# kongzhecn/OMG

Measured on AMD Instinct MI355X. Metric: images/sec @ SDXL 1024^2 50-step, 2-concept mask fusion, higher is better.
Workload: dtype fp16 (storage and MFMA operands; fp32 accumulate; = the reference's own torch_dtype, inference_lora.py:153-159).  Measured tolerance per UNet forward at full size vs the fp32 oracle: rms 1.09e-3, max 4.9e-3 of O(1) outputs — the reference's own fp16 eager execution, emulated op by op in the oracle

## Files before the change

include/omg_hip.h:

```cpp
#ifndef OMG_HIP_H
#define OMG_HIP_H

#include <stdint.h>

#ifdef __cplusplus
extern "C" {
#endif

#define OMG_ABI_VERSION 6

enum { OMG_F16 = 0, OMG_BF16 = 1, OMG_F32 = 2  };

enum {
  OMG_OK = 0,
  OMG_EINVAL = -1,
  OMG_EDTYPE = -2,
  OMG_ELAUNCH = -3
};

enum {
  OMG_ACT_NONE = 0,
  OMG_ACT_SILU = 1,
  OMG_ACT_GEGLU = 2
};

int omg_abi_version(void);
const char* omg_last_error(void);

typedef struct {
  int32_t dtype;
  int32_t M, N, K;
  const void* A;  int64_t lda;
  const void* W;  int64_t ldw;
  const void* A2; int64_t lda2;
  const void* W2; int64_t ldw2;
  int32_t K2;
  int32_t a2_col_block;
  int32_t groups;
  int32_t rows_per_group;
  const int32_t* group_adapter;
  int64_t w_adapter_stride;
  int64_t w2_adapter_stride;
  const void* bias;
  const void* group_bias; int64_t ldgb;
  const void* residual; int64_t ldr;
  int32_t act;
  float out_scale;
  void* C; int64_t ldc;
} omg_gemm_args;

int omg_gemm(const omg_gemm_args* a, void* stream);

int omg_quant_mx8(int32_t dtype, const void* x, int64_t ldx, int32_t M, int32_t K,
                  void* q, int64_t ldq, void* scales, int32_t s_ld, void* stream);

typedef struct {
  int32_t dtype;
  int32_t M, N, K;
  const void* A; int64_t lda;
  const void* a_scale; int32_t sa_ld;
  const void* W; int64_t ldw;
  const void* w_scale; int32_t sw_ld;
  int32_t groups, rows_per_group;
  const int32_t* group_adapter;
  int64_t w_adapter_stride;
  int64_t sw_adapter_stride;
  const void* bias;
  const void* residual; int64_t ldr;
  int32_t act;
  float out_scale;
  void* C; int64_t ldc;
  void* c_scale; int32_t sc_ld;
} omg_gemm_mx8_args;

int omg_gemm_mx8(const omg_gemm_mx8_args* a, void* stream);

typedef struct {
  int32_t dtype;
  int32_t B, H, W, Cin, Cout;
  const void* X; const void* x_scale;
  const void* Wq; const void* w_scale;
  int32_t sw_ld, act;
  const void* bias;
  const void* group_bias; int64_t ldgb;
  const void* residual;
  float out_scale;
  void* Y;
} omg_conv2d_mx8_args;
int omg_conv2d_mx8(const omg_conv2d_mx8_args* a, void* stream);

typedef struct {
  int32_t dtype;
  int32_t B, Hin, Win;
  int32_t C1, C2;
  int32_t Hout, Wout, Cout;
  int32_t ksize;
  int32_t stride;
  int32_t upsample;
  const void* X1; const void* X2;
  const void* W;
  const void* bias;
  const void* group_bias; int64_t ldgb;
  const void* residual;
  float out_scale;
  void* Y;
  int32_t act;
} omg_conv2d_args;

int omg_conv2d(const omg_conv2d_args* a, void* stream);

typedef struct {
  omg_conv2d_args conv;
  const int32_t* group_adapter;
  int64_t w_slot_stride;
  const void* A2; int64_t lda2;
  const void* W2; int64_t ldw2;
  int64_t w2_slot_stride;
  int32_t K2;
} omg_conv2d_slots_args;

int omg_conv2d_slots(const omg_conv2d_slots_args* a, void* stream);

typedef struct {
  int32_t dtype;
  int32_t B, heads, Nq, Nkv;
  const void* Q; int64_t ldq; int64_t q_bstride;
  const void* K; int64_t ldk; int64_t k_bstride;
  const void* Vt;
  int32_t Nkv_pad;
  const int32_t* qk_src;
  float scale;
  int32_t accumulate;
  float out_scale;
  void* O; int64_t ldo; int64_t o_bstride;
  const void* V; int64_t ldv; int64_t v_bstride;
} omg_attn_args;

int omg_attn_fwd(const omg_attn_args* a, void* stream);

int omg_attn_fwd_causal(const omg_attn_args* a, void* stream);

int omg_transpose_v(int dtype, const void* V, int64_t ldv, int64_t v_bstride,
                    int B, int heads, int Nkv, int Nkv_pad, void* Vt, int mfma_key_order, void* stream);

typedef struct {
  int32_t dtype;
  int32_t B, heads, Nkv, Nkv_pad;
  const void* V; int64_t ldv; int64_t v_bstride;
  const int32_t* edit_of;
  int32_t E, steps;
  const float* mapper; int64_t ld_mapper; int64_t mapper_estride;
  const float* alpha; int64_t alpha_step_stride; int64_t alpha_estride;
  const int32_t* step_idx;
  void* Vt_mapped; void* Vt_own;
} omg_vmap_args;

int omg_transpose_v_mapped(const omg_vmap_args* a, void* stream);

int64_t omg_groupnorm_ws_floats(int B, int groups, int HW);
int omg_groupnorm(int dtype, const void* X1, int C1, const void* X2, int C2,
                  int B, int HW, int groups, float eps,
                  const void* gamma, const void* beta, int silu,
                  float* workspace, void* Y, void* stream);
int omg_layernorm(int dtype, const void* X, int64_t ldx, int M, int C, float eps,
                  const void* gamma, const void* beta, void* Y, int64_t ldy, void* stream);
int omg_layernorm_mx8(int dtype, const void* X, int64_t ldx, int M, int C, float eps,
                      const void* gamma, const void* beta, void* Q, int64_t ldq,
                      void* scales, int s_ld, void* stream);

int omg_groupnorm_mx8(int dtype, const void* X1, int C1, const void* X2, int C2,
                      int B, int HW, int groups, float eps,
                      const void* gamma, const void* beta, int silu,
                      float* workspace, void* Q, void* scales, void* stream);

typedef struct {
  int32_t B, Hin, Win, Cin;
  int32_t Hout, Wout, Cout;
  int32_t ksize, upsample;
  const void* X; const void* W; const void* bias; const void* residual;
  void* Y;
} omg_conv2d_f32_args;

int omg_conv2d_f32(const omg_conv2d_f32_args* a, void* stream);

typedef struct {
  int32_t B, Hin, Win, Cin;
  int32_t Hout, Wout, Cout;
  int32_t upsample;
  const void* X; const void* U; const void* bias; const void* residual;
  void* Y;
} omg_conv2d_f32_wino_args;

int64_t omg_conv2d_f32_wino_weight_floats(int Cout, int Cin);
int omg_conv2d_f32_wino(const omg_conv2d_f32_wino_args* a, void* stream);
int omg_cast_f32(int dtype, const void* X, float* Y, int64_t n, void* stream);

int omg_conv_in(int dtype, const void* X_nchw, int x_is_f32, int B, int Cin, int H, int W,
                const void* Wt , const void* bias, int Cout,
                void* workspace ,
                void* Y_nhwc, void* stream);
int omg_conv_out(int dtype, const void* X_nhwc, int B, int H, int W, int Cin,
// ... 62 lines not shown
```

omg_amd/_lib.py:

```python
from __future__ import annotations

import ctypes as C
import os

_HERE = os.path.dirname(os.path.abspath(__file__))
LIB_PATH = os.environ.get("OMG_HIP_LIB") or os.path.join(_HERE, "csrc", "libomg_hip.so")

OMG_F16, OMG_BF16, OMG_F32 = 0, 1, 2
ACT_NONE, ACT_SILU, ACT_GEGLU = 0, 1, 2
MAX_CONCEPTS = 8

c_i32, c_i64, c_f32, c_vp = C.c_int32, C.c_int64, C.c_float, C.c_void_p


class GemmArgs(C.Structure):
    _fields_ = [
        ("dtype", c_i32), ("M", c_i32), ("N", c_i32), ("K", c_i32),
        ("A", c_vp), ("lda", c_i64), ("W", c_vp), ("ldw", c_i64),
        ("A2", c_vp), ("lda2", c_i64), ("W2", c_vp), ("ldw2", c_i64),
        ("K2", c_i32), ("a2_col_block", c_i32),
        ("groups", c_i32), ("rows_per_group", c_i32),
        ("group_adapter", c_vp), ("w_adapter_stride", c_i64), ("w2_adapter_stride", c_i64),
        ("bias", c_vp), ("group_bias", c_vp), ("ldgb", c_i64),
        ("residual", c_vp), ("ldr", c_i64),
        ("act", c_i32), ("out_scale", c_f32),
        ("C", c_vp), ("ldc", c_i64),
    ]


class GemmMx8Args(C.Structure):
    _fields_ = [
        ("dtype", c_i32), ("M", c_i32), ("N", c_i32), ("K", c_i32),
        ("A", c_vp), ("lda", c_i64), ("a_scale", c_vp), ("sa_ld", c_i32),
        ("W", c_vp), ("ldw", c_i64), ("w_scale", c_vp), ("sw_ld", c_i32),
        ("groups", c_i32), ("rows_per_group", c_i32), ("group_adapter", c_vp),
        ("w_adapter_stride", c_i64), ("sw_adapter_stride", c_i64),
        ("bias", c_vp), ("residual", c_vp), ("ldr", c_i64),
        ("act", c_i32), ("out_scale", c_f32),
        ("C", c_vp), ("ldc", c_i64),
        ("c_scale", c_vp), ("sc_ld", c_i32),
    ]


class Conv2dMx8Args(C.Structure):
    _fields_ = [
        ("dtype", c_i32), ("B", c_i32), ("H", c_i32), ("W", c_i32), ("Cin", c_i32), ("Cout", c_i32),
        ("X", c_vp), ("x_scale", c_vp), ("Wq", c_vp), ("w_scale", c_vp),
        ("sw_ld", c_i32), ("act", c_i32),
        ("bias", c_vp), ("group_bias", c_vp), ("ldgb", c_i64), ("residual", c_vp),
        ("out_scale", c_f32), ("Y", c_vp),
    ]


class Conv2dArgs(C.Structure):
    _fields_ = [
        ("dtype", c_i32), ("B", c_i32), ("Hin", c_i32), ("Win", c_i32),
        ("C1", c_i32), ("C2", c_i32), ("Hout", c_i32), ("Wout", c_i32), ("Cout", c_i32),
        ("ksize", c_i32), ("stride", c_i32), ("upsample", c_i32),
        ("X1", c_vp), ("X2", c_vp), ("W", c_vp), ("bias", c_vp),
        ("group_bias", c_vp), ("ldgb", c_i64), ("residual", c_vp),
        ("out_scale", c_f32), ("Y", c_vp), ("act", c_i32),
    ]


class Conv2dSlotsArgs(C.Structure):
    _fields_ = [
        ("conv", Conv2dArgs), ("group_adapter", c_vp), ("w_slot_stride", c_i64),
        ("A2", c_vp), ("lda2", c_i64), ("W2", c_vp), ("ldw2", c_i64),
        ("w2_slot_stride", c_i64), ("K2", c_i32),
    ]


class Conv2dF32Args(C.Structure):
    _fields_ = [
        ("B", c_i32), ("Hin", c_i32), ("Win", c_i32), ("Cin", c_i32),
        ("Hout", c_i32), ("Wout", c_i32), ("Cout", c_i32), ("ksize", c_i32), ("upsample", c_i32),
        ("X", c_vp), ("W", c_vp), ("bias", c_vp), ("residual", c_vp), ("Y", c_vp),
    ]


class Conv2dF32WinoArgs(C.Structure):
    _fields_ = [
        ("B", c_i32), ("Hin", c_i32), ("Win", c_i32), ("Cin", c_i32),
        ("Hout", c_i32), ("Wout", c_i32), ("Cout", c_i32), ("upsample", c_i32),
        ("X", c_vp), ("U", c_vp), ("bias", c_vp), ("residual", c_vp), ("Y", c_vp),
    ]


class AttnArgs(C.Structure):
    _fields_ = [
        ("dtype", c_i32), ("B", c_i32), ("heads", c_i32), ("Nq", c_i32), ("Nkv", c_i32),
        ("Q", c_vp), ("ldq", c_i64), ("q_bstride", c_i64),
        ("K", c_vp), ("ldk", c_i64), ("k_bstride", c_i64),
        ("Vt", c_vp), ("Nkv_pad", c_i32),
        ("qk_src", c_vp), ("scale", c_f32), ("accumulate", c_i32), ("out_scale", c_f32),
        ("O", c_vp), ("ldo", c_i64), ("o_bstride", c_i64),
        ("V", c_vp), ("ldv", c_i64), ("v_bstride", c_i64),
    ]


class VMapArgs(C.Structure):
    _fields_ = [
        ("dtype", c_i32), ("B", c_i32), ("heads", c_i32), ("Nkv", c_i32), ("Nkv_pad", c_i32),
        ("V", c_vp), ("ldv", c_i64), ("v_bstride", c_i64),
        ("edit_of", c_vp), ("E", c_i32), ("steps", c_i32),
        ("mapper", c_vp), ("ld_mapper", c_i64), ("mapper_estride", c_i64),
        ("alpha", c_vp), ("alpha_step_stride", c_i64), ("alpha_estride", c_i64),
        ("step_idx", c_vp), ("Vt_mapped", c_vp), ("Vt_own", c_vp),
    ]


class StepArgs(C.Structure):
    _fields_ = [
        ("C", c_i32), ("H", c_i32), ("W", c_i32), ("Hm", c_i32), ("Wm", c_i32),
        ("n_concepts", c_i32), ("fuse", c_i32), ("guidance_scale", c_f32),
        ("noise_pred", c_vp), ("region_pred", c_vp * MAX_CONCEPTS), ("masks", c_vp * MAX_CONCEPTS),
        ("coef", c_vp), ("step_idx", c_vp), ("advance", c_i32),
        ("latents", c_vp), ("out_dtype", c_i32), ("model_input_next", c_vp), ("fused_noise_out", c_vp),
    ]


SYMBOLS = {
    "omg_abi_version": (c_i32, []),
    "omg_last_error": (C.c_char_p, []),
    "omg_gemm": (c_i32, [C.POINTER(GemmArgs), c_vp]),
    "omg_quant_mx8": (c_i32, [c_i32, c_vp, c_i64, c_i32, c_i32, c_vp, c_i64, c_vp, c_i32, c_vp]),
    "omg_gemm_mx8": (c_i32, [C.POINTER(GemmMx8Args), c_vp]),
    "omg_conv2d_mx8": (c_i32, [C.POINTER(Conv2dMx8Args), c_vp]),
    "omg_groupnorm_mx8": (c_i32, [c_i32, c_vp, c_i32, c_vp, c_i32, c_i32, c_i32, c_i32, c_f32, c_vp, c_vp, c_i32, c_vp, c_vp, c_vp, c_vp]),
    "omg_conv2d": (c_i32, [C.POINTER(Conv2dArgs), c_vp]),
    "omg_conv2d_slots": (c_i32, [C.POINTER(Conv2dSlotsArgs), c_vp]),
    "omg_conv2d_f32": (c_i32, [C.POINTER(Conv2dF32Args), c_vp]),
    "omg_conv2d_f32_wino_weight_floats": (c_i64, [c_i32, c_i32]),
    "omg_conv2d_f32_wino": (c_i32, [C.POINTER(Conv2dF32WinoArgs), c_vp]),
    "omg_cast_f32": (c_i32, [c_i32, c_vp, c_vp, c_i64, c_vp]),
    "omg_attn_fwd": (c_i32, [C.POINTER(AttnArgs), c_vp]),
    "omg_attn_fwd_causal": (c_i32, [C.POINTER(AttnArgs), c_vp]),
    "omg_transpose_v": (c_i32, [c_i32, c_vp, c_i64, c_i64, c_i32, c_i32, c_i32, c_i32, c_vp, c_i32, c_vp]),
    "omg_transpose_v_mapped": (c_i32, [C.POINTER(VMapArgs), c_vp]),
    "omg_groupnorm_ws_floats": (c_i64, [c_i32, c_i32, c_i32]),
    "omg_groupnorm": (c_i32, [c_i32, c_vp, c_i32, c_vp, c_i32, c_i32, c_i32, c_i32, c_f32, c_vp, c_vp, c_i32, c_vp, c_vp, c_vp]),
    "omg_layernorm": (c_i32, [c_i32, c_vp, c_i64, c_i32, c_i32, c_f32, c_vp, c_vp, c_vp, c_i64, c_vp]),
    "omg_layernorm_mx8": (c_i32, [c_i32, c_vp, c_i64, c_i32, c_i32, c_f32, c_vp, c_vp, c_vp, c_i64, c_vp, c_i32, c_vp]),
    "omg_conv_in": (c_i32, [c_i32, c_vp, c_i32, c_i32, c_i32, c_i32, c_i32, c_vp, c_vp, c_i32, c_vp, c_vp, c_vp]),
    "omg_conv_out": (c_i32, [c_i32, c_vp, c_i32, c_i32, c_i32, c_i32, c_vp, c_vp, c_i32, c_vp, c_vp]),
    "omg_timestep_embedding": (c_i32, [c_i32, c_vp, c_i32, c_i32, c_vp, c_i64, c_vp]),
    "omg_silu": (c_i32, [c_i32, c_vp, c_vp, c_i64, c_vp]),
    "omg_softmax_rows": (c_i32, [c_i32, c_vp, c_i64, c_i64, c_i64, C.c_float, c_vp]),
    "omg_channel_mix": (c_i32, [c_vp, c_vp, c_vp, c_i32, c_i32, c_i32, c_i64, c_vp, c_vp]),
    "omg_add_inplace": (c_i32, [c_i32, c_vp, c_vp, c_i64, c_vp]),
    "omg_copy2d": (c_i32, [c_i32, c_vp, c_i64, c_vp, c_i64, c_i64, c_i64, c_vp]),
    "omg_fuse_cfg_step": (c_i32, [C.POINTER(StepArgs), c_vp]),
    "omg_fuse_cfg_step_ms": (c_i32, [C.POINTER(StepArgs), c_vp, c_vp, c_vp]),
    "omg_fuse_cfg_step_noise": (c_i32, [C.POINTER(StepArgs), c_vp, c_i64, c_vp]),
    "omg_scale_model_input": (c_i32, [c_i32, c_vp, c_vp, c_i32, c_vp, c_vp]),
    "omg_gather_step": (c_i32, [c_i32, c_vp, c_vp, c_vp, c_i64, c_vp]),
    "omg_attn_probs": (c_i32, [C.POINTER(AttnArgs), c_vp, c_vp]),
    "omg_attn_apply_probs": (c_i32, [c_i32, c_vp, c_vp, c_i64, c_i64, c_i32, c_i32, c_i32, c_i32, c_vp, c_i64, c_i64, c_vp]),
    "omg_dwconv2d": (c_i32, [c_i32, c_vp, c_i64, c_i32, c_i32, c_i32, c_i32, c_i32, c_vp, c_vp, c_vp, c_i64, c_vp]),
    "omg_relu_linear_att_ws_floats": (c_i64, [c_i32, c_i32, c_i32, c_i32]),
    "omg_relu_linear_att": (c_i32, [c_i32, c_vp, c_i64, c_i32, c_i32, c_i32, c_i32, c_f32, c_vp, c_vp, c_i64, c_vp]),
    "omg_conv3x3_nhwc_act": (c_i32, [c_i32, c_vp, c_i32, c_i32, c_i32, c_i32, c_i32, c_i32, c_vp, c_vp, c_i32, c_vp, c_vp, c_vp]),
    "omg_dwconv3x3_act": (c_i32, [c_i32, c_vp, c_i64, c_i32, c_i32, c_i32, c_i32, c_i32, c_vp, c_vp, c_i32, c_vp, c_i64, c_vp]),
    "omg_upsample_add_nhwc": (c_i32, [c_i32, c_vp, c_i32, c_i32, c_i32, c_i32, c_i32, c_i32, c_i32, c_vp, c_vp]),
    "omg_debug_set_glds": (None, [c_i32]),
    "omg_debug_set_gemm_variant": (None, [c_i32]),
    "omg_debug_choose_variant": (c_i32, [c_i32, c_i32, c_i32, c_i32]),
    "omg_debug_set_mx8_split": (None, [c_i32]),
    "omg_debug_set_attn_variant": (None, [c_i32]),
}

_lib = None


class OmgHipError(RuntimeError):
    pass


def lib() -> C.CDLL:
# ... 36 lines not shown
```

omg_amd/attention.py:

```python
from __future__ import annotations

from typing import Optional

import torch
from torch import nn

from . import _lib as L
from . import ops
from .modules import Dropout, Linear, LoraState, bump_pointer_epoch, pointer_epoch


class Attention(nn.Module):

    def __init__(self, query_dim: int, cross_attention_dim: Optional[int], heads: int, dim_head: int = 64,
                 dtype=torch.float16, device=None):
        super().__init__()
        if dim_head != 64:
            raise L.OmgHipError("the gfx950 attention kernel is specialised for head_dim 64 (all SDXL layers)")
        inner = heads * dim_head
        self.heads, self.scale, self.inner_dim = heads, dim_head ** -0.5, inner
        self.is_cross = cross_attention_dim is not None
        kv_dim = cross_attention_dim if self.is_cross else query_dim
        self.to_q = Linear(query_dim, inner, bias=False, dtype=dtype, device=device)
        self.to_k = Linear(kv_dim, inner, bias=False, dtype=dtype, device=device)
        self.to_v = Linear(kv_dim, inner, bias=False, dtype=dtype, device=device)
        self.to_out = nn.ModuleList([Linear(inner, query_dim, bias=True, dtype=dtype, device=device), Dropout()])
        self.spatial_norm = None
        self.group_norm = None
        self.norm_cross = None
        self.residual_connection = False
        self.rescale_output_factor = 1.0
        self.processor = FusedAttnProcessor()
        self._qkv = None
        self._kv = None
        self._qkv_slots = None
        self._kv_slots = None
        self._kv_cache = {}
        self.ip_kv_weight: Optional[torch.Tensor] = None
        self.ip_scale, self.ip_tokens = 1.0, 16
        self._ip_cache = None
        self._mx8 = {}

    def set_processor(self, processor) -> None:
        self.processor = processor

    def get_processor(self):
        return self.processor

    def forward(self, hidden_states, encoder_hidden_states=None, attention_mask=None, **cross_attention_kwargs):
        return self.processor(self, hidden_states, encoder_hidden_states=encoder_hidden_states,
                              attention_mask=attention_mask, **cross_attention_kwargs)

    def prepare_attention_mask(self, attention_mask, target_length, batch_size, out_dim=3):
        if attention_mask is not None:
            raise L.OmgHipError("attention masks are not used on OMG's path (always None) and are not supported")
        return None

    def head_to_batch_dim(self, t: torch.Tensor) -> torch.Tensor:
        B, N, _ = t.shape
        return t.reshape(B, N, self.heads, 64).permute(0, 2, 1, 3).reshape(B * self.heads, N, 64)

    def batch_to_head_dim(self, t: torch.Tensor) -> torch.Tensor:
        BH, N, d = t.shape
        return t.reshape(BH // self.heads, self.heads, N, d).permute(0, 2, 1, 3).reshape(BH // self.heads, N, self.heads * d)

    def get_attention_scores(self, query: torch.Tensor, key: torch.Tensor, attention_mask=None) -> torch.Tensor:
        if attention_mask is not None:
            raise L.OmgHipError("attention masks are not supported")
        q, k = query.contiguous(), key.contiguous()
        return ops.attn_probs(q, k, 1, self.scale)

    def _apply(self, fn, *a, **k):
        self.invalidate_packed()
        return super()._apply(fn, *a, **k)

    def invalidate_packed(self):
        self._qkv = self._kv = self._qkv_slots = self._kv_slots = None
        self._kv_cache = {}
        self._mx8 = {}
        self._ip_cache = None
        bump_pointer_epoch()

    def qkv_weight(self) -> torch.Tensor:
        if self._qkv is None:
            self._qkv = torch.cat([self.to_q.weight.data, self.to_k.weight.data, self.to_v.weight.data], dim=0).contiguous()
        return self._qkv

    def kv_weight(self) -> torch.Tensor:
        if self._kv is None:
            self._kv = torch.cat([self.to_k.weight.data, self.to_v.weight.data], dim=0).contiguous()
        return self._kv

    def _has_lora(self) -> bool:
        st = self.to_q.lora_state
        return st is not None and not st.merged and any(l.lora_down is not None for l in (self.to_q, self.to_k, self.to_v))

    def _merged(self) -> Optional[LoraState]:
        st = self.to_q.lora_state
        if st is None or not st.merged:
            return None
        have = [l.w_slots is not None for l in (self.to_q, self.to_k, self.to_v)]
        if any(have) and not all(have):
            raise L.OmgHipError("merged LoRA slots cover only part of to_q/to_k/to_v; rebuild the LoraBank")
        return st if all(have) else None

    def qkv_slots(self) -> torch.Tensor:
        if self._qkv_slots is None:
            self._qkv_slots = torch.cat([self.to_q.w_slots, self.to_k.w_slots, self.to_v.w_slots], dim=1).contiguous()
        return self._qkv_slots

    def kv_slots(self) -> torch.Tensor:
        if self._kv_slots is None:
            self._kv_slots = torch.cat([self.to_k.w_slots, self.to_v.w_slots], dim=1).contiguous()
        return self._kv_slots

    def project_self(self, x):
        B, N, C = x.shape
        inner = self.inner_dim
        if isinstance(x, ops.Mx8Tensor) or (self.to_q.mx8 and C % 128 == 0 and not self._has_lora()):
            if self._has_lora():
                raise L.OmgHipError("MX-fp8 activations cannot feed a segment-mode LoRA projection")
            xq = x if isinstance(x, ops.Mx8Tensor) else ops.quant_mx8(x)
            st = self._merged()
            if st is not None:
                if "qkv_slots" not in self._mx8:
                    self._mx8["qkv_slots"] = ops.quant_mx8(self.qkv_slots().reshape(-1, C))
                qkv = ops.gemm_mx8(xq, self._mx8["qkv_slots"], out_dtype=self.to_q.weight.dtype, groups=st.groups,
                                   w_group_adapter=st.group_adapter, n_per_adapter=3 * inner)
            else:
                if "qkv" not in self._mx8:
                    self._mx8["qkv"] = ops.quant_mx8(self.qkv_weight())
                qkv = ops.gemm_mx8(xq, self._mx8["qkv"], out_dtype=self.to_q.weight.dtype)
            qkv = qkv.view(B, N, 3 * inner)
            return qkv[:, :, :inner], qkv[:, :, inner:2 * inner], ops.value_operand(qkv[:, :, 2 * inner:], self.heads)
        if self._has_lora():
            q = self.to_q(x); k = self.to_k(x); v = self.to_v(x)
        else:
            st = self._merged()
            if st is not None:
                qkv = ops.gemm(x.reshape(B * N, C), self.qkv_slots(), groups=st.groups, w_group_adapter=st.group_adapter)
            else:
                qkv = ops.gemm(x.reshape(B * N, C), self.qkv_weight())
            qkv = qkv.view(B, N, 3 * inner)
            q, k, v = qkv[:, :, :inner], qkv[:, :, inner:2 * inner], qkv[:, :, 2 * inner:]
        return q, k, ops.value_operand(v, self.heads)

    def project_cross(self, ctx: torch.Tensor, with_v: bool = False):
        st = self.to_k.lora_state
        skey = (tuple(ctx.shape), None if st is None else (st.group_adapter.data_ptr(), st.merged))
        stamp = (ctx.data_ptr(), ctx._version)
        hit = self._kv_cache.get(skey)
        if hit is not None:
            self._kv_cache[skey] = self._kv_cache.pop(skey)
        if hit is not None and hit[0] == stamp:
            return (hit[1], hit[2], hit[5], hit[6]) if with_v else (hit[1], hit[2])
        B, Nk, Cx = ctx.shape
        inner = self.inner_dim
        kv_out = hit[4] if hit is not None else None
        vt_out = hit[2] if hit is not None else None
        if self._has_lora():
            k = self.to_k(ctx); v = self.to_v(ctx)
            kv_out = None
        else:
            ms = self._merged()
            x2 = ctx.reshape(B * Nk, Cx)
            if ms is not None:
                kv = ops.gemm(x2, self.kv_slots(), groups=ms.groups, w_group_adapter=ms.group_adapter, out=kv_out)
            else:
                kv = ops.gemm(x2, self.kv_weight(), out=kv_out)
            kv_out = kv
            kv = kv.view(B, Nk, 2 * inner)
            k, v = kv[:, :, :inner], kv[:, :, inner:]
        vt = ops.transpose_v(v, self.heads, out=vt_out)
        if hit is None and len(self._kv_cache) >= 4:
            self._kv_cache.pop(next(iter(self._kv_cache)))
            bump_pointer_epoch()
        images = hit[6] if hit is not None else [None, None]
        self._kv_cache[skey] = (stamp, k, vt, ctx, kv_out, v, images)
        return (k, vt, v, images) if with_v else (k, vt)


def _ip_kv(attn: Attention, ip_ctx: torch.Tensor):
    shape = tuple(ip_ctx.shape)
    stamp = (ip_ctx.data_ptr(), ip_ctx._version)
    cache = attn._ip_cache
    if cache is None:
        cache = attn._ip_cache = {}
    c = cache.get(shape)
    if c is not None:
        cache[shape] = cache.pop(shape)
    if c is None or c[0] != stamp:
        Bc, Ni, Cx = shape
        kv_out = c[3] if c is not None else None
        vt_out = c[2] if c is not None else None
        kv = ops.gemm(ip_ctx.reshape(Bc * Ni, Cx), attn.ip_kv_weight, out=kv_out)
        kv3 = kv.view(Bc, Ni, 2 * attn.inner_dim)
        vt = ops.transpose_v(kv3[:, :, attn.inner_dim:], attn.heads, out=vt_out)
        if c is None and len(cache) >= 4:
            cache.pop(next(iter(cache)))
            bump_pointer_epoch()
        c = (stamp, kv3[:, :, :attn.inner_dim], vt, kv, shape, ip_ctx)
        cache[shape] = c
    return c


def _ip_branch(attn: Attention, q: torch.Tensor, o: torch.Tensor, ip_ctx: torch.Tensor, row0: int) -> None:
    c = _ip_kv(attn, ip_ctx)
    ops.attention(q[row0:], c[1], c[2], attn.heads, attn.scale, out=o[row0:], accumulate=True, out_scale=attn.ip_scale)


def _to_tokens(attn, hidden_states):
    if isinstance(hidden_states, ops.Mx8Tensor):
        return hidden_states
    if hidden_states.dim() == 4:
        raise L.OmgHipError("4-D (NCHW) hidden_states are not produced by the SDXL transformer blocks; pass (B, N, C)")
    return hidden_states


class FusedAttnProcessor:

    supports_fused_residual = True

    def _qk_src(self, attn, is_cross: bool, n_tokens: int, batch: int, device, main_batch=None, images=1):
        return None

    def _skip_layer(self) -> None:
        return None

    def __call__(self, attn: Attention, hidden_states, encoder_hidden_states=None, attention_mask=None, temb=None,
                 scale: float = 1.0, residual: Optional[torch.Tensor] = None, **cross_attention_kwargs):
        if attention_mask is not None:
            raise L.OmgHipError("attention_mask is not supported")
        x = _to_tokens(attn, hidden_states)
        B, N, _ = x.shape
        is_cross = encoder_hidden_states is not None
        if is_cross:
            q = attn.to_q(x)
            k, vt = attn.project_cross(encoder_hidden_states)
        else:
            q, k, vt = attn.project_self(x)
        bypass = cross_attention_kwargs.pop("omg_bypass_controller", False)
        main_b = cross_attention_kwargs.pop("omg_main_batch", None)
        n_img = cross_attention_kwargs.pop("omg_images", 1)
        twin = cross_attention_kwargs.pop("omg_twin", False)
        if twin and not bypass:
            self._skip_layer()
        src = None if (bypass or twin) else self._qk_src(attn, is_cross, N, B, x.device, main_b, n_img)
        ip_ctx = cross_attention_kwargs.pop("omg_ip_tokens", None)
        ip_row0 = cross_attention_kwargs.pop("omg_ip_rows", 0)
        o = ops.attention(q, k, vt, attn.heads, attn.scale, qk_src=src)
        if is_cross and ip_ctx is not None and attn.ip_kv_weight is not None:
            _ip_branch(attn, q, o, ip_ctx, ip_row0)
        out = attn.to_out[0](o, residual=residual)
        return out


class RegionControlNet_AttnProcessor(FusedAttnProcessor):

    force_protocol = False

    def __init__(self, attention_op=None, controller=None, place_in_unet=None):
        self.attention_op = attention_op
        self.controller = controller
        self.place_in_unet = place_in_unet

    def _fusable(self) -> bool:
        return self.controller is None or getattr(self.controller, "is_pure_replacement", False)

    def _general(self) -> bool:
        c = self.controller
        return hasattr(c, "fused_edit") and hasattr(c, "edit_tables") and getattr(c, "local_blend", None) is None

    def _general_call(self, attn: Attention, hidden_states, encoder_hidden_states, residual, kw):
        ctl = self.controller
        x = _to_tokens(attn, hidden_states)
        B, N, _ = x.shape
        is_cross = encoder_hidden_states is not None
        main_b = kw.pop("omg_main_batch", None)
        n_img = kw.pop("omg_images", 1)
        if kw.pop("omg_twin", False):
            raise L.OmgHipError("omg_twin (dedup) needs a pure-replacement controller")
        ip_ctx = kw.pop("omg_ip_tokens", None)
        ip_row0 = kw.pop("omg_ip_rows", 0)
        v = images = None
        if is_cross:
            q = attn.to_q(x)
            if ctl.cross_kind() == "mixed":
                k, vt, v, images = attn.project_cross(encoder_hidden_states, with_v=True)
            else:
                k, vt = attn.project_cross(encoder_hidden_states)
        else:
            q, k, vt = attn.project_self(x)
        kind, src, edit_of = ctl.fused_edit(is_cross, N, main_b or B, self.place_in_unet, device=x.device, total_batch=B, images=n_img)
        if kind == "mixed":
            mapper, alpha, step = ctl.edit_tables(x.device)
            if images[0] is None:
                images[0], images[1] = torch.empty_like(vt), torch.empty_like(vt)
            vm, vo = ops.transpose_v_mapped(v, attn.heads, edit_of, mapper, alpha, step, nkv_pad=vt.shape[3], out=(images[0], images[1]))
            o = ops.attention(q, k, vm, attn.heads, attn.scale, qk_src=src)
            ops.attention(q, k, vo, attn.heads, attn.scale, out=o, accumulate=True)
        else:
            o = ops.attention(q, k, vt, attn.heads, attn.scale, qk_src=src)
        if is_cross and ip_ctx is not None and attn.ip_kv_weight is not None:
            _ip_branch(attn, q, o, ip_ctx, ip_row0)
        return attn.to_out[0](o, residual=residual)

    def _qk_src(self, attn, is_cross, n_tokens, batch, device, main_batch=None, images=1):
        if self.controller is None:
            return None
        return self.controller.fused_qk_src(is_cross, n_tokens, main_batch or batch, self.place_in_unet, device=device,
                                            total_batch=batch, images=images)

    def _skip_layer(self) -> None:
        if self.controller is not None:
            self.controller.skip_layer()

    def __call__(self, attn: Attention, hidden_states, encoder_hidden_states=None, attention_mask=None, temb=None,
                 scale: float = 1.0, residual: Optional[torch.Tensor] = None, **cross_attention_kwargs):
        bypass = cross_attention_kwargs.get("omg_bypass_controller", False)
        if bypass or self.controller is None or (self._fusable() and not self.force_protocol):
            return super().__call__(attn, hidden_states, encoder_hidden_states, attention_mask, temb, scale,
                                    residual=residual, **cross_attention_kwargs)
        if self._general() and not self.force_protocol:
            if attention_mask is not None:
                raise L.OmgHipError("attention_mask is not supported")
            return self._general_call(attn, hidden_states, encoder_hidden_states, residual, cross_attention_kwargs)
        if cross_attention_kwargs.get("omg_images", 1) != 1:
            raise L.OmgHipError("protocol mode (non-identity mapper) runs one request at a time")
        x = _to_tokens(attn, hidden_states)
        is_cross = encoder_hidden_states is not None
        src = encoder_hidden_states if is_cross else x
        query = attn.head_to_batch_dim(attn.to_q(x))
        key = attn.head_to_batch_dim(attn.to_k(src))
        value = attn.to_v(src)
        probs = attn.get_attention_scores(query, key, None)
        probs = self.controller(probs, is_cross, self.place_in_unet)
        o = ops.attn_apply_probs(probs.contiguous(), value, attn.heads)
        return attn.to_out[0](o, residual=residual)


class IPAttnProcessor2_0(nn.Module):

    supports_fused_residual = True

    def __init__(self, hidden_size: int, cross_attention_dim: Optional[int] = None, scale: float = 1.0, num_tokens: int = 4,
                 dtype=torch.float16, device=None):
        super().__init__()
        self.hidden_size, self.cross_attention_dim, self.scale, self.num_tokens = hidden_size, cross_attention_dim, scale, num_tokens
        self.to_k_ip = Linear(cross_attention_dim or hidden_size, hidden_size, bias=False, dtype=dtype, device=device)
        self.to_v_ip = Linear(cross_attention_dim or hidden_size, hidden_size, bias=False, dtype=dtype, device=device)

    def __call__(self, attn: Attention, hidden_states, encoder_hidden_states=None, attention_mask=None, temb=None,
                 residual: Optional[torch.Tensor] = None, **kw):
        if attention_mask is not None:
            raise L.OmgHipError("attention_mask is not supported")
        x = _to_tokens(attn, hidden_states)
        if encoder_hidden_states is None:
            q, k, vt = attn.project_self(x)
            o = ops.attention(q, k, vt, attn.heads, attn.scale)
            return attn.to_out[0](o, residual=residual)
        end = encoder_hidden_states.shape[1] - self.num_tokens
        text, ip = encoder_hidden_states[:, :end], encoder_hidden_states[:, end:]
        q = attn.to_q(x)
        B, Nt, Cx = text.shape
        k = attn.to_k(text.reshape(B * Nt, Cx)).view(B, Nt, -1)
        v = attn.to_v(text.reshape(B * Nt, Cx)).view(B, Nt, -1)
        o = ops.attention(q, k, ops.transpose_v(v, attn.heads), attn.heads, attn.scale)
        Ni = ip.shape[1]
        ipc = ip.reshape(B * Ni, Cx)
        k_ip = self.to_k_ip(ipc).view(B, Ni, -1)
        v_ip = self.to_v_ip(ipc).view(B, Ni, -1)
        ops.attention(q, k_ip, ops.transpose_v(v_ip, attn.heads), attn.heads, attn.scale, out=o, accumulate=True,
                      out_scale=self.scale)
        return attn.to_out[0](o, residual=residual)
```

omg_amd/controller.py:

```python
from __future__ import annotations

from typing import Dict, List, Optional, Sequence, Tuple

import numpy as np
import torch

MAX_NUM_WORDS = 77


def _word_of_token(text: str, tokenizer) -> Tuple[List[str], np.ndarray]:
    words = text.split(" ")
    pieces = [tokenizer.decode([tok]).strip("#") for tok in tokenizer.encode(text)][1:-1]
    cum = np.cumsum([len(pc_) for pc_ in pieces], dtype=np.int64) if pieces else np.zeros(0, np.int64)
    owner = np.full(len(pieces), len(words), dtype=np.int64)
    first, base = 0, 0
    for k, word in enumerate(words):
        if first >= len(pieces):
            break
        last = int(np.searchsorted(cum, base + len(word), side="left"))
        last = max(last, first)
        last = min(last, len(pieces) - 1)
        owner[first:last + 1] = k
        first, base = last + 1, int(cum[last])
    return words, owner


def get_word_inds(text: str, word_place, tokenizer) -> np.ndarray:
    words = text.split(" ")
    if isinstance(word_place, str):
        wanted = [i for i, w in enumerate(words) if w == word_place]
    elif isinstance(word_place, int):
        wanted = [word_place]
    else:
        wanted = list(word_place)
    if not wanted:
        return np.array([])
    _, owner = _word_of_token(text, tokenizer)
    return np.flatnonzero(np.isin(owner, wanted)) + 1


def _alignment_matrix(src_spans: Sequence[np.ndarray], tgt_spans: Sequence[np.ndarray], max_len: int) -> np.ndarray:
    m = np.zeros((max_len, max_len))
    i = j = 0
    for s, t in zip(src_spans, tgt_spans):
        s, t = np.asarray(s, dtype=np.int64), np.asarray(t, dtype=np.int64)
        run = min(int(s[0]) - i, max_len - i, max_len - j)
        if run < int(s[0]) - i:
            r = np.arange(max(run, 0))
            m[i + r, j + r] = 1
            return m
        r = np.arange(run)
        m[i + r, j + r] = 1
        i, j = i + run, j + run
        if i >= max_len or j >= max_len:
            return m
        if len(s) == len(t):
            m[s, t] = 1
        else:
            m[np.ix_(s, t)] = 1.0 / len(t)
        i, j = i + len(s), j + len(t)
    tail = np.arange(max(0, min(max_len - i, max_len - j)))
    if src_spans:
        m[j + tail, j + tail] = 1
    else:
        m[i + tail, j + tail] = 1
    return m


def get_replacement_mapper(prompts: Sequence[str], tokenizer, max_len: int = MAX_NUM_WORDS) -> torch.Tensor:
    out = []
    words0 = prompts[0].split(" ")
    for other in prompts[1:]:
        words = other.split(" ")
        if len(words0) != len(words):
            raise ValueError("attention replacement edit can only be applied on prompts with the same length"
                             f" but prompt A has {len(words0)} words and prompt B has {len(words)} words.")
        changed = [k for k, (a, b) in enumerate(zip(words0, words)) if a != b]
        if not changed:
            out.append(torch.eye(max_len, dtype=torch.float32))
            continue
        if tokenizer is None:
            raise ValueError("a tokenizer is required to align prompts that differ")
        _, own0 = _word_of_token(prompts[0], tokenizer)
        _, own1 = _word_of_token(other, tokenizer)
        src = [np.flatnonzero(own0 == k) + 1 for k in changed]
        tgt = [np.flatnonzero(own1 == k) + 1 for k in changed]
        out.append(torch.from_numpy(_alignment_matrix(src, tgt, max_len)).float())
    return torch.stack(out)


def get_time_words_attention_alpha(prompts, num_steps, cross_replace_steps, tokenizer, max_num_words=MAX_NUM_WORDS):
    spec = dict(cross_replace_steps) if isinstance(cross_replace_steps, dict) else {"default_": cross_replace_steps}
    spec.setdefault("default_", (0.0, 1.0))
    if isinstance(cross_replace_steps, dict):
        cross_replace_steps.setdefault("default_", (0.0, 1.0))
    n_rows, n_edit = num_steps + 1, len(prompts) - 1
    steps = torch.arange(n_rows).view(n_rows, 1)

    def inside(bounds) -> torch.Tensor:
        lo, hi = (0, bounds) if isinstance(bounds, float) else bounds
        return ((steps >= int(lo * n_rows)) & (steps < int(hi * n_rows))).to(torch.float32)

    alpha = inside(spec["default_"]).view(n_rows, 1, 1).repeat(1, n_edit, max_num_words)
    for word, bounds in spec.items():
        if word == "default_":
            continue
        col = inside(bounds)
        for k in range(n_edit):
            pos = get_word_inds(prompts[k + 1], word, tokenizer)
            if len(pos) > 0:
                alpha[:, k, torch.as_tensor(pos, dtype=torch.long)] = col
    return alpha.reshape(n_rows, n_edit, 1, 1, max_num_words)


class AttentionReplace:
    def __init__(self, prompts, num_steps: int, cross_replace_steps, self_replace_steps, width, height,
                 local_blend=None, tokenizer=None, device=None, dtype=None):
        self.low_resource = False
        self.width, self.height = width, height
        self.batch_size = len(prompts)
        self.local_blend = local_blend
        self.device, self.dtype = device, dtype
        alpha = get_time_words_attention_alpha(prompts, num_steps, cross_replace_steps, tokenizer)
        self.cross_replace_alpha = alpha.to(device)
        if isinstance(self_replace_steps, float):
            self_replace_steps = (0, self_replace_steps)
        self.num_self_replace = (int(num_steps * self_replace_steps[0]), int(num_steps * self_replace_steps[1]))
        mapper = get_replacement_mapper(prompts, tokenizer)
        self._alpha_host = alpha.reshape(alpha.shape[0], alpha.shape[1], MAX_NUM_WORDS).float().contiguous()
        self._mapper_host = mapper.float().contiguous()
        self._tables: Dict[str, Tuple[torch.Tensor, torch.Tensor]] = {}
        self._edit_cache: Dict[Tuple, torch.Tensor] = {}
        self._step_dev: Dict[str, torch.Tensor] = {}
        self._step_dev_val: Dict[str, int] = {}
        self._bound_step: Optional[Tuple[torch.Tensor, int]] = None
        self.mapper = mapper.to(dtype=dtype, device=device)
        self.num_att_layers = -1
        self.cur_step = 0
        self.cur_att_layer = 0
        eye = torch.eye(MAX_NUM_WORDS)
        self._identity_mapper = all(torch.equal(m.float().cpu(), eye) for m in self.mapper)
        self.is_pure_replacement = bool(local_blend is None and self._identity_mapper and bool((self.cross_replace_alpha == 1).all()))
        self._src_cache: Dict[Tuple, torch.Tensor] = {}
        ident = bool(all(torch.equal(m, eye) for m in self._mapper_host))
        self._cross_kinds = ["borrow" if ident and bool((a == 1).all()) else "own" if bool((a == 0).all()) else "mixed"
                             for a in self._alpha_host]

    @property
    def num_uncond_att_layers(self):
        return 0

    def reset(self):
        self.cur_step = 0
        self.cur_att_layer = 0

    def between_steps(self):
        return

    def step_callback(self, x_t):
        return x_t

    def _tick(self):
        self.cur_att_layer += 1
        if self.cur_att_layer == self.num_att_layers + self.num_uncond_att_layers:
            self.cur_att_layer = 0
            self.cur_step += 1
            self.between_steps()

    def _self_window(self) -> bool:
        return self.num_self_replace[0] <= self.cur_step < self.num_self_replace[1]

    def forward(self, attn, is_cross: bool, place_in_unet: str):
        if not (is_cross or self._self_window()):
            return attn
        v = attn.reshape(self.batch_size, attn.shape[0] // self.batch_size, *attn.shape[1:])
        base, edits = v[0], v[1:]
        if is_cross:
            a = self.cross_replace_alpha[self.cur_step].to(device=v.device, dtype=v.dtype)
            mapped = base.unsqueeze(0).expand(edits.shape[0], *base.shape) if self._identity_mapper \
                else torch.matmul(base.unsqueeze(0), self.mapper.to(device=v.device, dtype=v.dtype).unsqueeze(1))
            edits.copy_(mapped * a + (1 - a) * edits)
        elif edits.shape[2] <= self.width * self.height:
            edits.copy_(base.unsqueeze(0).expand_as(edits))
        return v.reshape(attn.shape)

    def __call__(self, attn, is_cross: bool, place_in_unet: str):
        cond = attn[attn.shape[0] // 2:]
        out = self.forward(cond, is_cross, place_in_unet)
        if out.data_ptr() != cond.data_ptr():
            cond.copy_(out)
        self._tick()
        return attn

    def replaces(self, is_cross: bool, n_tokens: int) -> bool:
        if is_cross:
            return True
        return self._self_window() and n_tokens <= self.width * self.height

    def qk_src_vector(self, batch: int, device, total_batch: Optional[int] = None, images: int = 1) -> torch.Tensor:
        total = total_batch or batch * images
        key = (batch, total, images, str(device))
        t = self._src_cache.get(key)
        if t is None:
            n = batch // 2
            v = []
            for j in range(images):
                v += [j * batch + i for i in range(n)] + [j * batch + n] * (batch - n)
            v += list(range(batch * images, total))
            t = torch.tensor(v, dtype=torch.int32, device=device)
            self._src_cache[key] = t
        return t

    def cross_kind(self, step: Optional[int] = None) -> str:
        step = self.cur_step if step is None else step
        return self._cross_kinds[min(max(step, 0), len(self._cross_kinds) - 1)]

    def edit_of_vector(self, batch: int, device, total_batch: Optional[int] = None, images: int = 1) -> torch.Tensor:
        total = total_batch or batch * images
        key = (batch, total, images, str(device))
        t = self._edit_cache.get(key)
        if t is None:
            n = batch // 2
            t = torch.tensor(([-1] * (n + 1) + list(range(batch - n - 1))) * images + [-1] * (total - batch * images),
                             dtype=torch.int32, device=device)
            self._edit_cache[key] = t
        return t

    def bind_step_counter(self, step_idx: Optional[torch.Tensor], offset: int = 0) -> None:
        self._bound_step = None if step_idx is None else (step_idx, int(offset))

    def _own_step_counter(self, device, refresh: bool = True) -> torch.Tensor:
        key = str(device)
        t = self._step_dev.get(key)
        if t is None:
            t = self._step_dev[key] = torch.zeros(1, dtype=torch.int32, device=device)
            self._step_dev_val[key] = 0
        if refresh and self._step_dev_val[key] != self.cur_step:
            if torch.cuda.is_current_stream_capturing():
                raise RuntimeError("a captured step needs a device step counter: bind_step_counter(step_idx) before capturing")
            t.fill_(self.cur_step)
            self._step_dev_val[key] = self.cur_step
        return t

    def edit_tables(self, device=None) -> Tuple[torch.Tensor, torch.Tensor, torch.Tensor]:
        device = torch.device(device or self.device or "cuda")
        key = str(device)
        tabs = self._tables.get(key)
        if tabs is None:
            tabs = self._tables[key] = (self._mapper_host.to(device), self._alpha_host.to(device))
        mapper, alpha = tabs
        if self._bound_step is not None:
            step, off = self._bound_step
            if not 0 <= off < alpha.shape[0]:
                raise RuntimeError(f"step counter offset {off} outside the {alpha.shape[0]}-row alpha table")
            return mapper, alpha[off:], step
        return mapper, alpha, self._own_step_counter(device, refresh=False)

    def fused_edit(self, is_cross: bool, n_tokens: int, batch: int, place_in_unet: str = "", device=None,
                   total_batch: Optional[int] = None, images: int = 1):
        if self.local_blend is not None:
            raise RuntimeError("fused_edit does not cover local_blend")
        n2 = 2 * self.batch_size
        if batch != n2 and not (batch == n2 - 1 and self.is_pure_replacement):
            raise ValueError(f"controller built for {self.batch_size} prompts expects a batch of {n2} ([unc..., cond...]), got {batch}")
        dev = device or self.device or "cuda"
        kind = self.cross_kind() if is_cross else ("borrow" if self.replaces(False, n_tokens) else "own")
        src = edit_of = None
        if kind != "own":
            src = self.qk_src_vector(batch, dev, total_batch, images)
        if kind == "mixed":
            edit_of = self.edit_of_vector(batch, dev, total_batch, images)
            if self._bound_step is None:
                self._own_step_counter(torch.device(dev))
        self._tick()
        return kind, src, edit_of

    def skip_layer(self) -> None:
        if not self.is_pure_replacement:
            raise RuntimeError("skip_layer needs a pure-replacement controller")
        self._tick()

    def fused_qk_src(self, is_cross: bool, n_tokens: int, batch: int, place_in_unet: str = "",
                     device=None, total_batch: Optional[int] = None, images: int = 1) -> Optional[torch.Tensor]:
        if not self.is_pure_replacement:
            raise RuntimeError("fused_qk_src needs a pure-replacement controller (identity mapper, alpha == 1)")
        if batch not in (2 * self.batch_size, 2 * self.batch_size - 1):
            raise ValueError(f"controller built for {self.batch_size} prompts expects a batch of {2 * self.batch_size} "
                             f"([unc..., cond...]), got {batch}")
        src = self.qk_src_vector(batch, device or self.device or "cuda", total_batch, images) if self.replaces(is_cross, n_tokens) else None
        self._tick()
        return src
```

omg_amd/csrc/gemm.hip:

```cpp
#include "common.h"
#include "gemm_epilogue.h"

__device__ __attribute__((aligned(256))) unsigned char omg_zero_page[256];

__device__ long long omg_dbg_ts[8192][6];

namespace {

constexpr int BM = 128, BN = 128, BK = 64;
constexpr int TILE_BYTES = BM * BK * 2;
constexpr int STAGE_LD = 68;
constexpr int LDS_BYTES_MAIN = 4 * TILE_BYTES;
constexpr int LDS_BYTES_EPI = 4 * 64 * STAGE_LD * 4;
constexpr int LDS_BYTES = LDS_BYTES_EPI > LDS_BYTES_MAIN ? LDS_BYTES_EPI : LDS_BYTES_MAIN;


template <bool GLDS>
OMG_DEV void stage16(const char* src, char* lds_wave_base, int lane, u32x4& hold) {
  if constexpr (GLDS) {
    __builtin_amdgcn_global_load_lds((gbl_ptr_t)src, (lds_ptr_t)lds_wave_base, 16, 0, 0);
  } else {
    hold = *(const u32x4*)src;
  }
}

template <typename T, int MT, int NT>
OMG_DEV void acc_init_cols(const GemmP& p, f32x16 (&acc)[MT][NT], int l31, int col0, int m0) {
  const bool fold = fold_group_bias(p);
  const long grow = fold ? (long)(m0 / p.rows_per_group) * p.ldgb : 0;
#pragma unroll
  for (int j = 0; j < NT; ++j) {
    const int c = col0 + j * 32 + l31;
    float b = 0.f;
    if (c < p.N) {
      float g = 0.f;
      if (p.bias) b = (float)((const T*)p.bias)[c];
      if (fold) g = (float)((const T*)p.group_bias)[grow + c];
      b = b + g;
    }
#pragma unroll
    for (int i = 0; i < MT; ++i)
#pragma unroll
      for (int r = 0; r < 16; ++r) acc[i][j][r] = b;
  }
}

template <typename T>
OMG_DEV void gemm_epilogue(const GemmP& p, f32x16 (&acc)[2][2], char* smem, int w, int lane, int m0, int n0, int m_end) {
  const int hi = lane >> 5, l31 = lane & 31;
  const int wm = w >> 1, wn = w & 1;
  __syncthreads();
  float* stage = (float*)smem + w * (64 * STAGE_LD);
#pragma unroll
  for (int i = 0; i < 2; ++i)
#pragma unroll
    for (int j = 0; j < 2; ++j)
#pragma unroll
      for (int r = 0; r < 16; ++r) {
        const int row = i * 32 + (r & 3) + 8 * (r >> 2) + 4 * hi;
        stage[row * STAGE_LD + j * 32 + l31] = acc[i][j][r];
      }
  __syncthreads();

  const int wm0 = m0 + wm * 64;
  const int wn0 = n0 + wn * 64;
  if (p.act == OMG_ACT_GEGLU) {
    const int ocol0 = (wn0 >> 1);
    const int sub = lane & 3, rsub = lane >> 2;
#pragma unroll
    for (int it = 0; it < 4; ++it) {
      const int row = it * 16 + rsub;
      const int gm = wm0 + row;
      const int gc = wn0 + sub * 8;
      if (gm < m_end && gc < p.N) {
        float v[8], g[8];
        const float* sp = stage + row * STAGE_LD + sub * 8;
#pragma unroll
        for (int e = 0; e < 8; ++e) { v[e] = sp[e]; g[e] = sp[32 + e]; }
        float o[8];
#pragma unroll
        for (int e = 0; e < 8; ++e) o[e] = v[e] * gelu_f(g[e]) * p.out_scale;
        *(u32x4*)(p.C + ((long)gm * p.ldc + ocol0 + sub * 8) * 2) = pack8<T>(o);
      }
    }
    return;
  }
  {
    const int sub = lane & 7, rsub = lane >> 3;
    const int gc = wn0 + sub * 8;
    const bool gb_rows = p.group_bias != nullptr && !fold_group_bias(p);
#pragma unroll
    for (int it = 0; it < 8; ++it) {
      const int row = it * 8 + rsub;
      const int gm = wm0 + row;
      if (gm < m_end && gc < p.N) {
        float v[8];
        const float* sp = stage + row * STAGE_LD + sub * 8;
#pragma unroll
        for (int e = 0; e < 8; ++e) v[e] = sp[e];
        if (gb_rows) {
          float gb[8];
          const int g = gm / p.rows_per_group;
          unpack8<T>(*(const u32x4*)(p.group_bias + ((long)g * p.ldgb + gc) * 2), gb);
#pragma unroll
          for (int e = 0; e < 8; ++e) v[e] += gb[e];
        }
        if (p.act == OMG_ACT_SILU) {
#pragma unroll
          for (int e = 0; e < 8; ++e) v[e] = silu_fast(v[e]);
        }
        if (p.residual) {
          float rv[8];
          unpack8<T>(*(const u32x4*)(p.residual + ((long)gm * p.ldr + gc) * 2), rv);
#pragma unroll
          for (int e = 0; e < 8; ++e) v[e] = __builtin_fmaf(v[e], p.out_scale, rv[e]);
        } else {
#pragma unroll
          for (int e = 0; e < 8; ++e) v[e] *= p.out_scale;
        }
        *(u32x4*)(p.C + ((long)gm * p.ldc + gc) * 2) = pack8<T>(v);
      }
    }
  }
}

template <typename T, bool CONV, bool GLDS, bool CSEG = false>
__global__ __launch_bounds__(256, 2) void gemm_kernel(GemmP p) {
  static_assert(CONV || !CSEG, "CSEG is the segment of the CONV form; the plain form always has it");
  extern __shared__ __attribute__((aligned(16))) char smem[];
  const int tid = threadIdx.x;
  const int lane = tid & 63;
  const int w = __builtin_amdgcn_readfirstlane(tid >> 6);
  const int hi = lane >> 5;
  const int l31 = lane & 31;

  const int nwg = gridDim.x;
  int bid = blockIdx.x;
  {
    const int q = nwg >> 3, r = nwg & 7, xcd = bid & 7, idx = bid >> 3;
    bid = (xcd < r ? xcd * (q + 1) : r * (q + 1) + (xcd - r) * q) + idx;
  }
  const int tiles_per_group = p.tiles_m * p.tiles_n;
  const int grp = bid / tiles_per_group;
  const int t_in = bid - grp * tiles_per_group;
  int tm, tn;
  {
    const int per_group = 8 * p.tiles_n;
    const int gid = t_in / per_group;
    const int first_m = gid * 8;
    const int gsz = (p.tiles_m - first_m) < 8 ? (p.tiles_m - first_m) : 8;
    const int r = t_in - gid * per_group;
    tm = first_m + (r % gsz);
    tn = r / gsz;
  }
  const int m_base = (p.tile_groups > 1) ? grp * p.rows_per_group : 0;
  const int m_end = (p.tile_groups > 1) ? m_base + p.rows_per_group : p.M;
  const int m0 = m_base + tm * BM;
  const int n0 = tn * BN;

  int adapter = 0;
  if (p.group_adapter != nullptr) adapter = p.group_adapter[grp];
  const bool seg2 = (p.K2 > 0) && (adapter >= 0);
  if (p.w_adapter_stride != 0 && adapter < 0) return;
  const char* Wp = p.W + (p.w_adapter_stride != 0 ? (long)adapter * p.w_adapter_stride * 2 : 0);
  const char* W2p = p.W2 + (seg2 ? (long)adapter * p.w2_adapter_stride * 2 : 0);
  const int a2off = (p.a2_col_block > 0) ? (n0 / p.a2_col_block) * p.K2 : 0;

  const int nk1 = (p.K + BK - 1) / BK;
  const int nk2 = seg2 ? (p.K2 + BK - 1) / BK : 0;
  const int nk = nk1 + nk2;

  const int prow = lane >> 3;
  const int ppos = lane & 7;
  int arow[4];
  int wrow[4];
  int cb[4], cy[4], cx[4];
#pragma unroll
  for (int i = 0; i < 4; ++i) {
    const int r = w * 32 + i * 8 + prow;
    int gm = m0 + r; if (gm > m_end - 1) gm = m_end - 1;
    int gn = n0 + r; if (gn > p.N - 1) gn = p.N - 1;
    arow[i] = gm; wrow[i] = gn;
    if constexpr (CONV) {
      const int hw = p.Hout * p.Wout;
      const int b = gm / hw; const int rem = gm - b * hw;
      cb[i] = b; cy[i] = rem / p.Wout; cx[i] = rem - cy[i] * p.Wout;
    }
  }
  const int Ctot = p.C1 + p.C2;
  const int cpt = CONV ? Ctot / BK : 1;
  const int pad = CONV ? (p.ksize == 3 ? 1 : 0) : 0;
  const char* zero = (const char*)omg_zero_page;

  u32x4 hold[8];
  char* ldsA = smem;
  char* ldsB = smem + 2 * TILE_BYTES;

  auto issue = [&](int kt, int buf) {
    const bool s2 = kt >= nk1;
    const int k0 = (s2 ? kt - nk1 : kt) * BK;
    const int Kseg = s2 ? p.K2 : p.K;
    int dy = 0, dx = 0, c0 = k0;
    const char* xsrc = p.A; int xC = p.C1;
    if constexpr (CONV) {
      const int ktc = (CSEG && s2) ? 0 : kt;
      const int tap = ktc / cpt; const int cc = ktc - tap * cpt;
      dy = tap / p.ksize; dx = tap - dy * p.ksize;
      c0 = cc * BK;
      if (c0 >= p.C1) { xsrc = p.X2; xC = p.C2; c0 -= p.C1; }
    }
#pragma unroll
    for (int i = 0; i < 4; ++i) {
      const int r = w * 32 + i * 8 + prow;
      const int c = ppos ^ ((r >> 1) & 7);
      const bool kvalid = (k0 + c * 8) < Kseg;
      const char* asrc;
      if constexpr (CONV) {
        int iy = cy[i] * p.stride + dy - pad;
        int ix = cx[i] * p.stride + dx - pad;
        const int Hl = p.upsample ? p.Hin * 2 : p.Hin;
        const int Wl = p.upsample ? p.Win * 2 : p.Win;
        const bool ok = (iy >= 0) && (iy < Hl) && (ix >= 0) && (ix < Wl);
        if (p.upsample) { iy >>= 1; ix >>= 1; }
        const long pix = ((long)cb[i] * p.Hin + iy) * p.Win + ix;
        asrc = ok ? xsrc + (pix * xC + c0 + c * 8) * 2 : zero;
        if constexpr (CSEG) {
          if (s2) asrc = kvalid ? p.A2 + ((long)arow[i] * p.lda2 + k0 + c * 8) * 2 : zero;
        }
      } else {
        if (!s2) asrc = kvalid ? p.A + ((long)arow[i] * p.lda + k0 + c * 8) * 2 : zero;
        else     asrc = kvalid ? p.A2 + ((long)arow[i] * p.lda2 + a2off + k0 + c * 8) * 2 : zero;
      }
      stage16<GLDS>(asrc, ldsA + buf * TILE_BYTES + (w * 32 + i * 8) * 128, lane, hold[i]);
      const char* wsrc;
      if (!s2) wsrc = kvalid ? Wp + ((long)wrow[i] * p.ldw + (CONV ? kt * BK : k0) + c * 8) * 2 : zero;
      else     wsrc = kvalid ? W2p + ((long)wrow[i] * p.ldw2 + k0 + c * 8) * 2 : zero;
      stage16<GLDS>(wsrc, ldsB + buf * TILE_BYTES + (w * 32 + i * 8) * 128, lane, hold[4 + i]);
    }
  };
  auto commit = [&](int buf) {
    if constexpr (!GLDS) {
#pragma unroll
      for (int i = 0; i < 4; ++i) {
        const int off = (w * 32 + i * 8) * 128 + lane * 16;
        *(u32x4*)(ldsA + buf * TILE_BYTES + off) = hold[i];
        *(u32x4*)(ldsB + buf * TILE_BYTES + off) = hold[4 + i];
      }
    }
  };

  const int wm = w >> 1, wn = w & 1;
  f32x16 acc[2][2];
  acc_init_cols<T, 2, 2>(p, acc, lane & 31, n0 + wn * 64, m0);

  using V8 = typename Vec<T>::v8;

  issue(0, 0);
  commit(0);
  for (int kt = 0; kt < nk; ++kt) {
    const int buf = kt & 1;
    asm volatile("s_waitcnt vmcnt(0)" ::: "memory");
    __syncthreads();
    if (kt + 1 < nk) issue(kt + 1, buf ^ 1);
    const char* a_base = ldsA + buf * TILE_BYTES;
    const char* b_base = ldsB + buf * TILE_BYTES;
#pragma unroll
    for (int ks = 0; ks < 4; ++ks) {
      V8 af[2], bf[2];
      const int kc = ks * 2 + hi;
#pragma unroll
      for (int i = 0; i < 2; ++i) {
        const int ra = wm * 64 + i * 32 + l31;
        af[i] = *(const V8*)(a_base + ra * 128 + ((kc ^ ((ra >> 1) & 7)) << 4));
        const int rb = wn * 64 + i * 32 + l31;
        bf[i] = *(const V8*)(b_base + rb * 128 + ((kc ^ ((rb >> 1) & 7)) << 4));
      }
#pragma unroll
      for (int i = 0; i < 2; ++i)
#pragma unroll
        for (int j = 0; j < 2; ++j) acc[i][j] = Vec<T>::mfma32(af[i], bf[j], acc[i][j]);
    }
    if constexpr (!GLDS) { if (kt + 1 < nk) commit(buf ^ 1); }
  }

  gemm_epilogue<T>(p, acc, smem, w, lane, m0, n0, m_end);
}


OMG_DEV int conv_voff(int b, int oy, int ox, int ch_bytes, int stride, int dy, int dx, int Hl, int Wl, int ups, int Hin, int Win,
                      int pix_bytes, int c0_bytes) {
  int iy = oy * stride + dy, ix = ox * stride + dx;
  const bool ok = ((unsigned)iy < (unsigned)Hl) & ((unsigned)ix < (unsigned)Wl);
  iy >>= ups; ix >>= ups;
  const int pix = (b * Hin + iy) * Win + ix;
  const int off = pix * pix_bytes + c0_bytes + ch_bytes;
  return ok ? off : 0x7ffffff0;
}

template <typename T, bool CONV, int MT>
__global__ __launch_bounds__(512, 2) void gemm_kernel_v6(GemmP p) {
  constexpr int BM_ = 256, BN_ = MT == 4 ? 256 : 128, BKc = 64, NW = 8, NT = 2;
  constexpr int WN_ = MT == 4 ? 4 : 2;
  constexpr int BI = BN_ / 8 / NW;
  constexpr int ND = 4 + BI;
  constexpr int HB = ND / 2;
  constexpr int A_BYTES = BM_ * BKc * 2;
  constexpr int STAGE_BYTES = (BM_ + BN_) * BKc * 2;

  extern __shared__ __attribute__((aligned(16))) char smem[];
  const int tid = threadIdx.x;
  const int lane = tid & 63;
  const int w = __builtin_amdgcn_readfirstlane(tid >> 6);
  const int hi = lane >> 5;
  const int l31 = lane & 31;

  const int nwg = gridDim.x;
  int bid = blockIdx.x;
  {
    const int q = nwg >> 3, r = nwg & 7, xcd = bid & 7, idx = bid >> 3;
    bid = (xcd < r ? xcd * (q + 1) : r * (q + 1) + (xcd - r) * q) + idx;
  }
  const int tiles_per_group = p.tiles_m * p.tiles_n;
  const int grp = bid / tiles_per_group;
  const int t_in = bid - grp * tiles_per_group;
  int tm, tn;
  {
    const int per_group = 8 * p.tiles_n;
    const int gid = t_in / per_group;
    const int first_m = gid * 8;
    const int gsz = (p.tiles_m - first_m) < 8 ? (p.tiles_m - first_m) : 8;
    const int r = t_in - gid * per_group;
    tm = first_m + (r % gsz);
    tn = r / gsz;
  }
  const int m_base = (p.tile_groups > 1) ? grp * p.rows_per_group : 0;
  const int m_end = (p.tile_groups > 1) ? m_base + p.rows_per_group : p.M;
  const int m0 = m_base + tm * BM_;
  const int n0 = tn * BN_;
  int adapter = 0;
  if (p.group_adapter != nullptr) adapter = p.group_adapter[grp];
  if (p.w_adapter_stride != 0 && adapter < 0) return;
  const char* Wp = p.W + (p.w_adapter_stride != 0 ? (long)adapter * p.w_adapter_stride * 2 : 0);
  const int nk = (p.K + BKc - 1) / BKc;

  const int Ctot = p.C1 + p.C2;
  const long a_bytes = CONV ? (long)p.M / (p.Hout * p.Wout) * p.Hin * p.Win * p.C1 * 2 : ((long)(p.M - 1) * p.lda + p.K) * 2;
  const __amdgpu_buffer_rsrc_t rsA = __builtin_amdgcn_make_buffer_rsrc((void*)p.A, 0, (int)(a_bytes < 0x7fffff00 ? a_bytes : 0x7fffff00), 0x00020000);
  const __amdgpu_buffer_rsrc_t rsA2 = __builtin_amdgcn_make_buffer_rsrc((void*)(CONV && p.X2 ? p.X2 : p.A), 0,
      CONV ? (int)((long)p.M / (p.Hout * p.Wout) * p.Hin * p.Win * p.C2 * 2) : 0, 0x00020000);
  const long w_bytes = ((long)(p.N - 1) * p.ldw + p.K) * 2;
  const __amdgpu_buffer_rsrc_t rsW = __builtin_amdgcn_make_buffer_rsrc((void*)Wp, 0, (int)w_bytes, 0x00020000);

  const int prow = lane >> 3, ppos = lane & 7;
  int voffA[4], voffW[BI], ldoA[4], ldoW[BI];
  int cb[4], cy[4], cx[4], cch[4];
#pragma unroll
  for (int i = 0; i < 4; ++i) {
    const int r = (w + i * NW) * 8 + prow;
    const int c = ppos ^ ((r >> 1) & 7);
    int gm = m0 + r; if (gm > m_end - 1) gm = m_end - 1;
    ldoA[i] = (w + i * NW) * 1024;
    if constexpr (CONV) {
      const int hw = p.Hout * p.Wout;
      const int b = gm / hw; const int rem = gm - b * hw;
      cb[i] = b; cy[i] = rem / p.Wout; cx[i] = rem - cy[i] * p.Wout; cch[i] = c * 16;
      voffA[i] = 0;
    } else {
      voffA[i] = (int)(((long)gm * p.lda + c * 8) * 2);
    }
  }
#pragma unroll
  for (int i = 0; i < BI; ++i) {
    const int r = (w + i * NW) * 8 + prow;
    const int c = ppos ^ ((r >> 1) & 7);
    int gn = n0 + r; if (gn > p.N - 1) gn = p.N - 1;
    voffW[i] = (int)(((long)gn * p.ldw + c * 8) * 2);
    ldoW[i] = A_BYTES + (w + i * NW) * 1024;
  }

  const int wm = w / WN_, wn = w % WN_;
  f32x16 acc[MT][NT];
  const bool gb_epi = acc_init_bias<T, MT, NT>(p, acc, lane, m0, n0 + wn * 64);
  using V8 = typename Vec<T>::v8;
  int aro[MT][4], bro[NT][4];
#pragma unroll
  for (int ks = 0; ks < 4; ++ks) {
    const int kc = ks * 2 + hi;
#pragma unroll
    for (int i = 0; i < MT; ++i) {
      const int ra = wm * (MT * 32) + i * 32 + l31;
      aro[i][ks] = ra * 128 + ((kc ^ ((ra >> 1) & 7)) << 4);
    }
#pragma unroll
    for (int j = 0; j < NT; ++j) {
      const int rb = wn * 64 + j * 32 + l31;
      bro[j][ks] = A_BYTES + rb * 128 + ((kc ^ ((rb >> 1) & 7)) << 4);
    }
  }

  int koff = 0;
  int tap_dy = 0, tap_dx = 0, c0b = 0, xCb = 0;
  bool x2 = false;
  const int cpt = CONV ? Ctot / BKc : 1;
  const int pad = CONV ? (p.ksize == 3 ? 1 : 0) : 0;
  const int Hl = CONV ? (p.upsample ? p.Hin * 2 : p.Hin) : 0;
  const int Wl = CONV ? (p.upsample ? p.Win * 2 : p.Win) : 0;
#define OMG_PREP(kt_)                                                                                      \
  do {                                                                                                     \
    koff = (kt_) * (BKc * 2);                                                                              \
    if constexpr (CONV) {                                                                                  \
      const int tap = (kt_) / cpt; const int cc = (kt_) - tap * cpt;                                       \
      tap_dy = tap / p.ksize - pad; tap_dx = tap - (tap / p.ksize) * p.ksize - pad;                        \
      int c0 = cc * BKc;                                                                                   \
      x2 = c0 >= p.C1;                                                                                     \
      if (x2) c0 -= p.C1;                                                                                  \
      c0b = c0 * 2; xCb = (x2 ? p.C2 : p.C1) * 2;                                                          \
    }                                                                                                      \
  } while (0)
#define OMG_AVO(i_) (CONV ? conv_voff(cb[i_], cy[i_], cx[i_], cch[i_], p.stride, tap_dy, tap_dx, Hl, Wl, p.upsample, p.Hin, p.Win, xCb, c0b) : voffA[i_])

  const bool late = w >= 4;
  V8 af[2][MT], bf[2][NT];
#define OMG_ISA(d_) ((d_) < 4)
#define OMG_AI(d_) ((d_) < 4 ? (d_) : 0)
#define OMG_WI(d_) ((d_) >= 4 ? (d_) - 4 : 0)
#define OMG_VO(d_) (OMG_ISA(d_) ? OMG_AVO(OMG_AI(d_)) : voffW[OMG_WI(d_)])
#define OMG_LO(d_) (OMG_ISA(d_) ? ldoA[OMG_AI(d_)] : ldoW[OMG_WI(d_)])
#define OMG_RS(d_) (OMG_ISA(d_) ? ((CONV && x2) ? rsA2 : rsA) : rsW)
#define OMG_SO(d_) ((OMG_ISA(d_) && CONV) ? 0 : koff)
#define OMG_DMA(d_, nb_)                                                                                     \
  dma16(OMG_RS(d_), (nb_) + OMG_LO(d_), OMG_VO(d_), OMG_SO(d_))
#define OMG_DMA2(q_, nb_)                                                                                    \
  dma16(late ? OMG_RS(HB + (q_)) : OMG_RS(q_), (nb_) + (late ? OMG_LO(HB + (q_)) : OMG_LO(q_)),              \
        late ? OMG_VO(HB + (q_)) : OMG_VO(q_), late ? OMG_SO(HB + (q_)) : OMG_SO(q_))
#define OMG_Q(q_)                                                                                            \
  do {                                                                                                       \
    if constexpr (MT == 4) {                                                                                 \
      _Pragma("unroll") for (int i = ((q_) & 1) * 2; i < ((q_) & 1) * 2 + 2; ++i)                            \
        _Pragma("unroll") for (int j = 0; j < NT; ++j)                                                       \
          acc[i][j] = Vec<T>::mfma32(bf[(q_) >> 1][j], af[(q_) >> 1][i], acc[i][j]);                         \
    } else {                                                                                                 \
      _Pragma("unroll") for (int j = 0; j < NT; ++j)                                                         \
        acc[(q_) & 1][j] = Vec<T>::mfma32(bf[(q_) >> 1][j], af[(q_) >> 1][(q_) & 1], acc[(q_) & 1][j]);      \
    }                                                                                                        \
  } while (0)
#define OMG_RD(sb_, half_)                                                                                   \
  do {                                                                                                       \
    _Pragma("unroll") for (int ks = 0; ks < 2; ++ks) {                                                       \
      _Pragma("unroll") for (int j = 0; j < NT; ++j) bf[ks][j] = *(const V8*)((sb_) + bro[j][(half_) * 2 + ks]); \
      _Pragma("unroll") for (int i = 0; i < MT; ++i) af[ks][i] = *(const V8*)((sb_) + aro[i][(half_) * 2 + ks]); \
    }                                                                                                        \
  } while (0)

  OMG_PREP(0);
  OMG_DMA(0, smem); OMG_DMA(1, smem); OMG_DMA(2, smem); OMG_DMA(3, smem);
  OMG_DMA(4, smem); OMG_DMA(5, smem);
  if constexpr (ND == 8) { OMG_DMA(6, smem); OMG_DMA(7, smem); }

  for (int kt = 0; kt < nk; ++kt) {
    wait_vmcnt<0>();
    __builtin_amdgcn_s_barrier();
    const char* sb = smem + (kt & 1) * STAGE_BYTES;
    char* nb = smem + ((kt + 1) & 1) * STAGE_BYTES;
    const bool nxt = kt + 1 < nk;
    OMG_PREP(kt + 1);
    if (late) {
      if (kt > 0) {
        OMG_Q(0); if (nxt) OMG_DMA(0, nb);
        OMG_Q(1); if (nxt) OMG_DMA(1, nb);
        OMG_Q(2); if (nxt) OMG_DMA(2, nb);
        OMG_Q(3); if constexpr (HB == 4) { if (nxt) OMG_DMA(3, nb); }
      } else if (nxt) {
        OMG_DMA(0, nb); OMG_DMA(1, nb); OMG_DMA(2, nb);
        if constexpr (HB == 4) OMG_DMA(3, nb);
      }
    }
    OMG_RD(sb, 0);
    OMG_Q(0); if (nxt) OMG_DMA2(0, nb);
    OMG_Q(1); if (nxt) OMG_DMA2(1, nb);
    OMG_Q(2); if (nxt) OMG_DMA2(2, nb);
    OMG_Q(3); if constexpr (HB == 4) { if (nxt) OMG_DMA2(3, nb); }
    OMG_RD(sb, 1);
    if (!late) {
      OMG_Q(0); if (nxt) OMG_DMA(HB + 0, nb);
      OMG_Q(1); if (nxt) OMG_DMA(HB + 1, nb);
      OMG_Q(2); if (nxt) OMG_DMA(HB + 2, nb);
      OMG_Q(3); if constexpr (HB == 4) { if (nxt) OMG_DMA(HB + 3, nb); }
    }
  }
  if (late) { OMG_Q(0); OMG_Q(1); OMG_Q(2); OMG_Q(3); }
#undef OMG_DMA
#undef OMG_DMA2
#undef OMG_Q
#undef OMG_RD
#undef OMG_ISA
#undef OMG_AI
#undef OMG_WI
#undef OMG_VO
#undef OMG_LO
#undef OMG_RS
#undef OMG_SO
#undef OMG_PREP
#undef OMG_AVO
  if (p.dbg & 32) {
    float sacc = 0.f;
#pragma unroll
    for (int i = 0; i < MT; ++i)
#pragma unroll
      for (int j = 0; j < NT; ++j)
#pragma unroll
        for (int r = 0; r < 16; ++r) sacc += acc[i][j][r];
    if (sacc == 1.2345e-30f) p.C[0] = 1;
    return;
  }
  epilogue_direct<T, MT, NT>(p, acc, lane, m0 + wm * (MT * 32), n0 + wn * 64, m_end, gb_epi);
}

template <typename T, bool CONV, int ABL = 0, int MT = 4, int NT = 4, bool XE = false, int EF = 0>
__global__ __launch_bounds__(256, 1) void gemm_kernel_v7(GemmP p) {
  constexpr int BM_ = MT * 64, BN_ = NT * 64, BKc = 64;
  constexpr int AB = MT * 2, WB = NT * 2;
  constexpr int NMM = MT * NT;
  constexpr int SLOTS = NMM / 2;
  constexpr int NRD = MT + NT;
  static_assert(NMM % 2 == 0, "even number of MFMAs per k-step");
  constexpr int A_BYTES = BM_ * BKc * 2;
  constexpr int STAGE_BYTES = (BM_ + BN_) * BKc * 2;

  const bool ts_on = (p.dbg & 16) && blockIdx.x < 8192 && threadIdx.x == 0;
  long long ts0 = 0, ts1 = 0, ts2 = 0;
  if (((p.dbg >> 16) & 0xff) != 0 && blockIdx.x < 256) {
    const long long wait = (long long)((blockIdx.x * 97) & 255) * ((p.dbg >> 16) & 0xff) * 25 / 256;
    const long long t_end = __builtin_amdgcn_s_memrealtime() + wait;
    while (__builtin_amdgcn_s_memrealtime() < t_end) __builtin_amdgcn_s_sleep(2);
  }
  if (p.dbg & 16) ts0 = __builtin_amdgcn_s_memrealtime();
  extern __shared__ __attribute__((aligned(16))) char smem[];
  const int tid = threadIdx.x;
  const int lane = tid & 63;
  const int w = __builtin_amdgcn_readfirstlane(tid >> 6);
  const int hi = lane >> 5;
  const int l31 = lane & 31;

  const int nwg = gridDim.x;
  int bid = blockIdx.x;
  {
    const int q = nwg >> 3, r = nwg & 7, xcd = bid & 7, idx = bid >> 3;
    bid = (xcd < r ? xcd * (q + 1) : r * (q + 1) + (xcd - r) * q) + idx;
  }
  const int tiles_per_group = p.tiles_m * p.tiles_n;
  const int grp = bid / tiles_per_group;
  const int t_in = bid - grp * tiles_per_group;
  int tm, tn;
  {
    const int per_group = 8 * p.tiles_n;
    const int gid = t_in / per_group;
    const int first_m = gid * 8;
    const int gsz = (p.tiles_m - first_m) < 8 ? (p.tiles_m - first_m) : 8;
    const int r = t_in - gid * per_group;
    tm = first_m + (r % gsz);
    tn = r / gsz;
  }
  const int m_base = (p.tile_groups > 1) ? grp * p.rows_per_group : 0;
  const int m_end = (p.tile_groups > 1) ? m_base + p.rows_per_group : p.M;
  const int m0 = m_base + tm * BM_;
  const int n0 = tn * BN_;
  int adapter = 0;
  if (p.group_adapter != nullptr) adapter = p.group_adapter[grp];
  if (p.w_adapter_stride != 0 && adapter < 0) return;
  const char* Wp = p.W + (p.w_adapter_stride != 0 ? (long)adapter * p.w_adapter_stride * 2 : 0);
  const int nk = (p.K + BKc - 1) / BKc;

  const int Ctot = p.C1 + p.C2;
  const long a_bytes = CONV ? (long)p.M / (p.Hout * p.Wout) * p.Hin * p.Win * p.C1 * 2 : ((long)(p.M - 1) * p.lda + p.K) * 2;
  const __amdgpu_buffer_rsrc_t rsA = __builtin_amdgcn_make_buffer_rsrc((void*)p.A, 0, (int)(a_bytes < 0x7fffff00 ? a_bytes : 0x7fffff00), 0x00020000);
  const __amdgpu_buffer_rsrc_t rsA2 = __builtin_amdgcn_make_buffer_rsrc((void*)(CONV && p.X2 ? p.X2 : p.A), 0,
      CONV ? (int)((long)p.M / (p.Hout * p.Wout) * p.Hin * p.Win * p.C2 * 2) : 0, 0x00020000);
  const long w_bytes = ((long)(p.N - 1) * p.ldw + p.K) * 2;
  const __amdgpu_buffer_rsrc_t rsW = __builtin_amdgcn_make_buffer_rsrc((void*)Wp, 0, (int)w_bytes, 0x00020000);

  const int prow = lane >> 3, ppos = lane & 7;
  int voffA[AB], voffW[WB];
  int cb[AB], cy[AB], cx[AB];
  const int dchunk = (ppos ^ ((w & 1) * 4 + (prow >> 1))) * 16;
#pragma unroll
  for (int i = 0; i < AB; ++i) {
    const int r = (w + i * 4) * 8 + prow;
    int gm = m0 + r; if (gm > m_end - 1) gm = m_end - 1;
    if constexpr (CONV) {
      const int hw = p.Hout * p.Wout;
      const int b = gm / hw; const int rem = gm - b * hw;
      cb[i] = b; cy[i] = rem / p.Wout; cx[i] = rem - cy[i] * p.Wout;
      voffA[i] = 0;
    } else {
      cb[i] = cy[i] = cx[i] = 0;
      voffA[i] = (int)((long)gm * p.lda * 2) + dchunk;
    }
  }
#pragma unroll
  for (int i = 0; i < WB; ++i) {
    const int r = (w + i * 4) * 8 + prow;
    int gn = n0 + r; if (gn > p.N - 1) gn = p.N - 1;
    voffW[i] = (int)((long)gn * p.ldw * 2) + dchunk;
  }
  const int ldo = w * 1024;

  const int wm = w >> 1, wn = w & 1;
  f32x16 acc[MT][NT];
  using V8 = typename Vec<T>::v8;
  int aoff[4], boff[4];
#pragma unroll
  for (int ks = 0; ks < 4; ++ks) {
    const int sw = ((ks * 2 + hi) ^ ((l31 >> 1) & 7)) << 4;
    aoff[ks] = (wm * (MT * 32) + l31) * 128 + sw;
    boff[ks] = A_BYTES + (wn * (NT * 32) + l31) * 128 + sw;
  }

  int koff = 0;
  int tap_dy = 0, tap_dx = 0, c0b = 0, xCb = 0;
  bool x2 = false;
  const int cpt = CONV ? Ctot / BKc : 1;
  const int pad = CONV ? (p.ksize == 3 ? 1 : 0) : 0;
  const int Hl = CONV ? (p.upsample ? p.Hin * 2 : p.Hin) : 0;
  const int Wl = CONV ? (p.upsample ? p.Win * 2 : p.Win) : 0;
#define OMG_PREP(kt_)                                                                                      \
  do {                                                                                                     \
    koff = (kt_) * (BKc * 2);                                                                              \
    if constexpr (CONV) {                                                                                  \
      const int tap = (kt_) / cpt; const int cc = (kt_) - tap * cpt;                                       \
      tap_dy = tap / p.ksize - pad; tap_dx = tap - (tap / p.ksize) * p.ksize - pad;                        \
      int c0 = cc * BKc;                                                                                   \
      x2 = c0 >= p.C1;                                                                                     \
      if (x2) c0 -= p.C1;                                                                                  \
      c0b = c0 * 2; xCb = (x2 ? p.C2 : p.C1) * 2;                                                          \
    }                                                                                                      \
  } while (0)
#define OMG_DMA(d_, nb_)                                                                                   \
  do {                                                                                                     \
    if ((d_) < AB) {                                                                                       \
      const int i_ = (d_) < AB ? (d_) : 0;                                                                 \
      if (CONV) dma16(x2 ? rsA2 : rsA, (nb_) + ldo + i_ * 4096,                                            \
                      conv_voff(cb[i_], cy[i_], cx[i_], dchunk, p.stride, tap_dy, tap_dx, Hl, Wl, p.upsample, p.Hin, p.Win, xCb, c0b), 0); \
      else dma16(rsA, (nb_) + ldo + i_ * 4096, voffA[i_], koff);                                           \
    } else {                                                                                               \
      const int i_ = (d_) - AB < WB ? (d_) - AB : 0;                                                       \
      dma16(rsW, (nb_) + A_BYTES + ldo + i_ * 4096, voffW[i_], koff);                                      \
    }                                                                                                      \
  } while (0)
#define OMG_DMAN(first_, n_, nb_)                                                                          \
  do { _Pragma("unroll") for (int d_ = 0; d_ < (n_); ++d_) OMG_DMA((first_) + d_, nb_); } while (0)
#define OMG_RD(f_, sb_, ks_)                                                                               \
  do {                                                                                                     \
    _Pragma("unroll") for (int j = 0; j < NT; ++j) bf[f_][j] = *(const V8*)((sb_) + boff[ks_] + j * 4096); \
    _Pragma("unroll") for (int i = 0; i < MT; ++i) af[f_][i] = *(const V8*)((sb_) + aoff[ks_] + i * 4096); \
  } while (0)
#define OMG_MM(f_)                                                                                         \
  do {                                                                                                     \
    _Pragma("unroll") for (int i = 0; i < MT; ++i)                                                         \
      _Pragma("unroll") for (int j = 0; j < NT; ++j)                                                       \
        acc[i][j] = Vec<T>::mfma32(af[f_][i], bf[f_][j], acc[i][j]);                                       \
  } while (0)
#define OMG_RD1(f_, sb_, ks_, r_)                                                                          \
  do {                                                                                                     \
     \
    const bool isA_ = (r_) == 1 || (r_) > NT;                                                              \
    const int idx_ = (r_) <= 1 ? 0 : (r_) <= NT ? (r_) - 1 : (r_) - NT;                                    \
    if (!isA_) bf[f_][idx_] = *(const V8*)((sb_) + boff[ks_] + idx_ * 4096);                               \
    else af[f_][idx_] = *(const V8*)((sb_) + aoff[ks_] + idx_ * 4096);                                     \
  } while (0)
#define OMG_MM1(f_, n_) acc[(n_) / NT][(n_) % NT] = Vec<T>::mfma32(bf[f_][(n_) % NT], af[f_][(n_) / NT], acc[(n_) / NT][(n_) % NT])
#define OMG_KSTEP(f_, RD_, rb_, rks_, DMA_, d0_, dn_, db_)                                                 \
  do {                                                                                                     \
    constexpr int RPS_ = (RD_) == 2 ? 2 : (NRD + SLOTS - 1) / SLOTS;                                       \
    constexpr int DPS_ = ((dn_) + SLOTS - 1) / SLOTS;                                                      \
    _Pragma("unroll") for (int s_ = 0; s_ < SLOTS; ++s_) {                                                 \
      OMG_MM1(f_, 2 * s_);                                                                                 \
      __builtin_amdgcn_sched_barrier(0);                                                                   \
      if ((RD_) != 0 && !(ABL & 2)) {                                                                      \
        _Pragma("unroll") for (int q_ = 0; q_ < RPS_; ++q_)                                                \
          if (s_ * RPS_ + q_ < NRD) OMG_RD1(1 - (f_), rb_, rks_, s_ * RPS_ + q_);                          \
      }                                                                                                    \
      __builtin_amdgcn_sched_barrier(0);                                                                   \
      OMG_MM1(f_, 2 * s_ + 1);                                                                             \
      __builtin_amdgcn_sched_barrier(0);                                                                   \
      if ((DMA_) && !(ABL & 1)) {                                                                          \
        _Pragma("unroll") for (int q_ = 0; q_ < DPS_; ++q_)                                                \
          if (s_ * DPS_ + q_ < (dn_)) OMG_DMA((d0_) + s_ * DPS_ + q_, db_);                                \
      }                                                                                                    \
      __builtin_amdgcn_sched_barrier(0);                                                                   \
    }                                                                                                      \
  } while (0)

  V8 af[2][MT], bf[2][NT];
  OMG_PREP(0);
  OMG_DMAN(0, AB + WB, smem);
  const bool gb_epi = acc_init_bias<T, MT, NT>(p, acc, lane, m0, n0 + wn * (NT * 32));
  wait_vmcnt<0>();
  __builtin_amdgcn_s_barrier();
  if (p.dbg & 16) ts1 = __builtin_amdgcn_s_memrealtime();
  OMG_PREP(1);
  if (nk > 1) OMG_DMAN(0, AB, smem + STAGE_BYTES);
  OMG_RD(0, smem, 0);

#define OMG_STAGE(HAS1_, HAS2_)                                                                            \
  do {                                                                                                     \
    const char* cur = smem + (kt & 1) * STAGE_BYTES;                                                       \
    char* nxt = smem + ((kt + 1) & 1) * STAGE_BYTES;                                                       \
                                                  \
    OMG_KSTEP(0, 1, cur, 1, HAS1_, AB, WB, nxt);                                                            \
    OMG_KSTEP(1, 1, cur, 2, false, 0, 0, nxt);                                                             \
    OMG_KSTEP(0, 1, cur, 3, false, 0, 0, nxt);                                                             \
     \
    if (!(ABL & 4)) { asm volatile("s_waitcnt vmcnt(0) lgkmcnt(0)" ::: "memory"); __builtin_amdgcn_s_barrier(); } \
                                                                                                      \
     \
    if (HAS2_) OMG_PREP(kt + 2);                                                                           \
    OMG_KSTEP(1, (HAS1_) ? 2 : 0, nxt, 0, HAS2_, 0, AB, (char*)cur);                                                     \
  } while (0)
  int kt = 0;
// ... 57 lines not shown
  if (grid <= 0) return OMG_OK;
  OMG_LAUNCH((gemm_kernel_v6<T, CONV, MT>), dim3(grid), dim3(512), lds, s, p);
  return omg_check_launch("gemm_v6");
}

template <typename T, bool CONV, int ABL = 0, int MT = 4, int NT = 4, bool XE = false, int EF = 0>
int launch_v7(GemmP p, hipStream_t s, int mrows) {
  constexpr int BM_ = MT * 64, BN_ = NT * 64;
  constexpr int lds = 2 * (BM_ + BN_) * 64 * 2 + (XE ? 4 * 8192 : 0);
  static bool attr = false;
  if (!attr) {
    attr = true;
    (void)hipFuncSetAttribute((const void*)gemm_kernel_v7<T, CONV, ABL, MT, NT, XE, EF>, hipFuncAttributeMaxDynamicSharedMemorySize, lds);
  }
  p.tiles_m = (mrows + BM_ - 1) / BM_;
  p.tiles_n = (p.N + BN_ - 1) / BN_;
  p.dbg = g_dbg;
  const int grid = p.tile_groups * p.tiles_m * p.tiles_n;
  if (grid <= 0) return OMG_OK;
  OMG_LAUNCH((gemm_kernel_v7<T, CONV, ABL, MT, NT, XE, EF>), dim3(grid), dim3(256), lds, s, p);
  return omg_check_launch("gemm_v7");
}

int num_cus();
#include "gemm_v12.h"
#include "gemm_v13.h"

int num_cus() {
  static int n = 0;
  if (n == 0) {
    int dev = 0;
    (void)hipGetDevice(&dev);
    if (hipDeviceGetAttribute(&n, hipDeviceAttributeMultiprocessorCount, dev) != hipSuccess || n <= 0) n = 256;
  }
  return n;
}

int choose_variant(int mrows, int groups, int N, bool conv, bool geglu = false) {
  if (g_variant != 0) return g_variant;
  const long t256 = (long)groups * ((mrows + 255) / 256) * ((N + 255) / 256);
  const long t256x128 = (long)groups * ((mrows + 255) / 256) * ((N + 127) / 128);
  const long t128x320 = (long)groups * ((mrows + 127) / 128) * ((N + 319) / 320);
  const long t256x320 = (long)groups * ((mrows + 255) / 256) * ((N + 319) / 320);
  const double c256 = (N > 128 && t256 >= 120) ? (double)((t256 + 255) / 256) : 1e30;
  const double c128 = t256x128 >= 120 ? (double)((t256x128 + 255) / 256) * 0.58 * 1.06 : 1e30;
  const double c320 = (conv && !geglu && N % 320 == 0 && t128x320 >= 120) ? (double)((t128x320 + 255) / 256) * 0.70 : 1e30;
  const double c13 = (!geglu && N % 320 == 0 && t256x320 >= 120) ? (double)((t256x320 + 255) / 256) * (conv ? 1.20 : 1.28) : 1e30;
  if (c13 < c256 && c13 < c128 && c13 < c320) return 28;
  if (c320 < c256 && c320 < c128) return 24;
  if (c256 <= c128) return c256 < 1e30 ? 25 : 1;
  return 14;
}

template <typename T, bool CONV>
int launch(const GemmP& p, hipStream_t s) {
  const int mrows = p.tile_groups > 1 ? p.rows_per_group : p.M;
  if (g_use_glds) {
    int v = choose_variant(mrows, p.tile_groups, p.N, CONV, p.act == OMG_ACT_GEGLU);
    const long lim = 0x7fff0000L;
    const long a_sz = CONV ? (long)p.M / (p.Hout * p.Wout) * p.Hin * p.Win * (p.C1 > p.C2 ? p.C1 : p.C2) * 2 : (long)p.M * p.lda * 2;
    const long c_sz = (long)p.M * (p.ldc > p.ldr ? p.ldc : p.ldr) * 2;
    const bool v6ok = p.K2 == 0 && p.A2 == nullptr && p.K % 64 == 0 && a_sz < lim && (long)p.N * p.ldw * 2 < lim && c_sz < lim &&
                      (p.group_bias == nullptr || (long)(p.M / (p.rows_per_group > 0 ? p.rows_per_group : 1) + 1) * p.ldgb * 2 < lim);
    if ((v == 24 || v == 28) && p.act == OMG_ACT_GEGLU) v = 25;
    if (v == 24 && v6ok) return launch_v7<T, CONV, 0, 2, 5>(p, s, mrows);
    if (v == 15 && v6ok) return launch_v7<T, CONV>(p, s, mrows);
    if (v == 25 && v6ok) return launch_v12_form<T, CONV>(p, s, mrows);
    if (v == 28 && v6ok) return launch_v13_form<T, CONV>(p, s, mrows);
#ifdef OMG_ABLATION_BUILDS
    if constexpr (!CONV && sizeof(T) == 2 && Vec<T>::is_f16) {
      if (v >= 17 && v <= 23 && v6ok) {
        switch (v - 16) {
          case 1: return launch_v7<T, CONV, 1>(p, s, mrows);
          case 2: return launch_v7<T, CONV, 2>(p, s, mrows);
          case 3: return launch_v7<T, CONV, 3>(p, s, mrows);
          case 4: return launch_v7<T, CONV, 4>(p, s, mrows);
          case 5: return launch_v7<T, CONV, 5>(p, s, mrows);
          case 6: return launch_v7<T, CONV, 6>(p, s, mrows);
          default: return launch_v7<T, CONV, 7>(p, s, mrows);
        }
      }
    }
#endif
    if ((v == 13 || v == 14) && v6ok) return v == 13 ? launch_v6<T, CONV, 4>(p, s, mrows) : launch_v6<T, CONV, 2>(p, s, mrows);
  }
  const int grid = p.tile_groups * p.tiles_m * p.tiles_n;
  if (grid <= 0) return OMG_OK;
  if constexpr (CONV) {
    if (p.K2 > 0) {
      if (g_use_glds) {
        OMG_LAUNCH((gemm_kernel<T, true, true, true>), dim3(grid), dim3(256), LDS_BYTES, s, p);
      } else {
        OMG_LAUNCH((gemm_kernel<T, true, false, true>), dim3(grid), dim3(256), LDS_BYTES, s, p);
      }
      return omg_check_launch("gemm");
    }
  }
  if (g_use_glds) {
    OMG_LAUNCH((gemm_kernel<T, CONV, true>), dim3(grid), dim3(256), LDS_BYTES, s, p);
  } else {
    OMG_LAUNCH((gemm_kernel<T, CONV, false>), dim3(grid), dim3(256), LDS_BYTES, s, p);
  }
  return omg_check_launch("gemm");
}

bool g_attr_set = false;
void ensure_attrs() {
  if (g_attr_set) return;
  g_attr_set = true;
  (void)hipFuncSetAttribute((const void*)gemm_kernel<f16, false, true>, hipFuncAttributeMaxDynamicSharedMemorySize, LDS_BYTES);
  (void)hipFuncSetAttribute((const void*)gemm_kernel<f16, false, false>, hipFuncAttributeMaxDynamicSharedMemorySize, LDS_BYTES);
  (void)hipFuncSetAttribute((const void*)gemm_kernel<f16, true, true>, hipFuncAttributeMaxDynamicSharedMemorySize, LDS_BYTES);
  (void)hipFuncSetAttribute((const void*)gemm_kernel<f16, true, false>, hipFuncAttributeMaxDynamicSharedMemorySize, LDS_BYTES);
  (void)hipFuncSetAttribute((const void*)gemm_kernel<f16, true, true, true>, hipFuncAttributeMaxDynamicSharedMemorySize, LDS_BYTES);
  (void)hipFuncSetAttribute((const void*)gemm_kernel<f16, true, false, true>, hipFuncAttributeMaxDynamicSharedMemorySize, LDS_BYTES);
#ifndef OMG_DEV_F16_ONLY
  (void)hipFuncSetAttribute((const void*)gemm_kernel<bf16, false, true>, hipFuncAttributeMaxDynamicSharedMemorySize, LDS_BYTES);
  (void)hipFuncSetAttribute((const void*)gemm_kernel<bf16, false, false>, hipFuncAttributeMaxDynamicSharedMemorySize, LDS_BYTES);
  (void)hipFuncSetAttribute((const void*)gemm_kernel<bf16, true, true>, hipFuncAttributeMaxDynamicSharedMemorySize, LDS_BYTES);
  (void)hipFuncSetAttribute((const void*)gemm_kernel<bf16, true, false>, hipFuncAttributeMaxDynamicSharedMemorySize, LDS_BYTES);
  (void)hipFuncSetAttribute((const void*)gemm_kernel<bf16, true, true, true>, hipFuncAttributeMaxDynamicSharedMemorySize, LDS_BYTES);
  (void)hipFuncSetAttribute((const void*)gemm_kernel<bf16, true, false, true>, hipFuncAttributeMaxDynamicSharedMemorySize, LDS_BYTES);
#endif
}

}

extern "C" int omg_debug_read_ts(long long* out, int blocks) {
  return (int)hipMemcpyFromSymbol(out, HIP_SYMBOL(omg_dbg_ts), sizeof(long long) * 6 * (blocks < 8192 ? blocks : 8192));
}
extern "C" void omg_debug_set_glds(int on) { g_use_glds = on != 0; }
extern "C" void omg_debug_set_gemm_variant(int v) { g_variant = v & 0xff; g_dbg = v >> 8; }
extern "C" int omg_debug_choose_variant(int mrows, int groups, int N, int conv) {
  const int saved = g_variant;
  g_variant = 0;
  const int v = choose_variant(mrows, groups, N, (conv & 1) != 0, (conv & 2) != 0);
  g_variant = saved;
  return v;
}

extern "C" int omg_gemm(const omg_gemm_args* a, void* stream) {
  OMG_REQUIRE(a != nullptr, "omg_gemm: null args");
  OMG_REQUIRE(a->dtype == OMG_F16 || a->dtype == OMG_BF16, "omg_gemm: dtype");
  OMG_REQUIRE(a->M >= 0 && a->N > 0 && a->K > 0, "omg_gemm: shape");
  if (a->M == 0) return OMG_OK;
  OMG_REQUIRE(a->K % 8 == 0 && a->N % 8 == 0 && a->K2 % 8 == 0, "omg_gemm: K, K2, N must be multiples of 8");
  OMG_REQUIRE(a->lda % 8 == 0 && a->ldw % 8 == 0 && a->ldc % 8 == 0, "omg_gemm: leading dims must be multiples of 8");
  OMG_REQUIRE(a->A && a->W && a->C, "omg_gemm: null operand");
  OMG_REQUIRE(a->groups >= 1 && (long)a->groups * a->rows_per_group == a->M, "omg_gemm: M != groups*rows_per_group");
  if (a->K2 > 0) OMG_REQUIRE(a->A2 && a->W2 && a->lda2 % 8 == 0 && a->ldw2 % 8 == 0, "omg_gemm: LoRA segment operands");
  if (a->act == OMG_ACT_GEGLU) OMG_REQUIRE(a->N % 64 == 0 && !a->residual && !a->group_bias, "omg_gemm: GEGLU needs N % 64 == 0, no residual");
  if (a->residual) OMG_REQUIRE(a->ldr % 8 == 0, "omg_gemm: ldr");
  if (a->group_bias) OMG_REQUIRE(a->ldgb % 8 == 0, "omg_gemm: ldgb");
  ensure_attrs();
  GemmP p{};
  p.M = a->M; p.N = a->N; p.K = a->K;
  p.A = (const char*)a->A; p.lda = a->lda; p.W = (const char*)a->W; p.ldw = a->ldw;
  p.A2 = (const char*)a->A2; p.lda2 = a->lda2; p.W2 = (const char*)a->W2; p.ldw2 = a->ldw2;
  p.K2 = a->K2; p.a2_col_block = a->a2_col_block;
  const bool per_group = (a->group_adapter != nullptr) && a->groups > 1;
  p.tile_groups = per_group ? a->groups : 1;
  p.rows_per_group = a->rows_per_group;
  p.group_adapter = a->group_adapter;
  p.w_adapter_stride = a->w_adapter_stride; p.w2_adapter_stride = a->w2_adapter_stride;
  p.bias = (const char*)a->bias; p.group_bias = (const char*)a->group_bias; p.ldgb = a->ldgb;
  p.residual = (const char*)a->residual; p.ldr = a->ldr;
  p.act = a->act; p.out_scale = a->out_scale; p.C = (char*)a->C; p.ldc = a->ldc;
  const int mrows = per_group ? a->rows_per_group : a->M;
  p.tiles_m = (mrows + BM - 1) / BM;
  p.tiles_n = (a->N + BN - 1) / BN;
  hipStream_t s = (hipStream_t)stream;
#ifdef OMG_DEV_F16_ONLY
  OMG_REQUIRE(a->dtype == OMG_F16, "omg_gemm: this is a DEV=1 build (fp16 kernels only)");
  return launch<f16, false>(p, s);
#else
  return a->dtype == OMG_F16 ? launch<f16, false>(p, s) : launch<bf16, false>(p, s);
#endif
}

static int conv2d_params(const omg_conv2d_args* a, GemmP& p) {
  OMG_REQUIRE(a->dtype == OMG_F16 || a->dtype == OMG_BF16, "omg_conv2d: dtype");
  OMG_REQUIRE(a->ksize == 1 || a->ksize == 3, "omg_conv2d: ksize must be 1 or 3");
  OMG_REQUIRE(a->stride == 1 || a->stride == 2, "omg_conv2d: stride must be 1 or 2");
  OMG_REQUIRE(a->C1 > 0 && a->C1 % 64 == 0 && a->C2 % 64 == 0 && a->C2 >= 0, "omg_conv2d: channels must be multiples of 64");
  OMG_REQUIRE(a->Cout % 8 == 0, "omg_conv2d: Cout % 8");
  OMG_REQUIRE(a->X1 && a->W && a->Y && (a->C2 == 0 || a->X2), "omg_conv2d: null operand");
  OMG_REQUIRE(!(a->upsample && a->stride != 1), "omg_conv2d: upsample with stride");
  const int Hl = a->upsample ? 2 * a->Hin : a->Hin, Wl = a->upsample ? 2 * a->Win : a->Win;
  const int pad = a->ksize == 3 ? 1 : 0;
  OMG_REQUIRE(a->Hout == (Hl + 2 * pad - a->ksize) / a->stride + 1 && a->Wout == (Wl + 2 * pad - a->ksize) / a->stride + 1,
              "omg_conv2d: output size mismatch");
  ensure_attrs();
  const int Ctot = a->C1 + a->C2;
  p.M = a->B * a->Hout * a->Wout; p.N = a->Cout; p.K = a->ksize * a->ksize * Ctot;
  if (p.M == 0) return OMG_OK;
  p.A = (const char*)a->X1; p.X2 = (const char*)a->X2;
  p.W = (const char*)a->W; p.ldw = p.K;
  p.K2 = 0; p.tile_groups = 1; p.rows_per_group = a->Hout * a->Wout;
  p.bias = (const char*)a->bias; p.group_bias = (const char*)a->group_bias; p.ldgb = a->ldgb;
  p.residual = (const char*)a->residual; p.ldr = a->Cout;
  OMG_REQUIRE(a->act == OMG_ACT_NONE || a->act == OMG_ACT_SILU, "omg_conv2d: act");
  p.act = a->act; p.out_scale = a->out_scale; p.C = (char*)a->Y; p.ldc = a->Cout;
  p.Hin = a->Hin; p.Win = a->Win; p.C1 = a->C1; p.C2 = a->C2; p.Hout = a->Hout; p.Wout = a->Wout;
  p.ksize = a->ksize; p.stride = a->stride; p.upsample = a->upsample;
  p.tiles_m = (p.M + BM - 1) / BM; p.tiles_n = (p.N + BN - 1) / BN;
  if (a->group_bias) OMG_REQUIRE(a->ldgb % 8 == 0, "omg_conv2d: ldgb");
#ifdef OMG_DEV_F16_ONLY
  OMG_REQUIRE(a->dtype == OMG_F16, "omg_conv2d: this is a DEV=1 build (fp16 kernels only)");
#endif
  return OMG_OK;
}

static int conv2d_launch(int dtype, const GemmP& p, hipStream_t s) {
#ifdef OMG_DEV_F16_ONLY
  (void)dtype;
  return launch<f16, true>(p, s);
#else
  return dtype == OMG_F16 ? launch<f16, true>(p, s) : launch<bf16, true>(p, s);
#endif
}

extern "C" int omg_conv2d(const omg_conv2d_args* a, void* stream) {
  OMG_REQUIRE(a != nullptr, "omg_conv2d: null args");
  GemmP p{};
  const int rc = conv2d_params(a, p);
  if (rc != OMG_OK || p.M == 0) return rc;
  return conv2d_launch(a->dtype, p, (hipStream_t)stream);
}

extern "C" int omg_conv2d_slots(const omg_conv2d_slots_args* a, void* stream) {
  OMG_REQUIRE(a != nullptr, "omg_conv2d_slots: null args");
  OMG_REQUIRE(a->K2 >= 0 && a->K2 % 8 == 0, "omg_conv2d_slots: K2 must be a non-negative multiple of 8");
  OMG_REQUIRE(a->w_slot_stride >= 0 && a->w_slot_stride % 8 == 0, "omg_conv2d_slots: w_slot_stride must be a non-negative multiple of 8");
  if (a->K2 > 0) {
    OMG_REQUIRE(a->A2 && a->W2, "omg_conv2d_slots: LoRA segment operands");
    OMG_REQUIRE(a->lda2 >= a->K2 && a->lda2 % 8 == 0 && a->ldw2 >= a->K2 && a->ldw2 % 8 == 0,
                "omg_conv2d_slots: lda2 / ldw2 must be multiples of 8 and at least K2");
    OMG_REQUIRE(a->w2_slot_stride >= 0 && a->w2_slot_stride % 8 == 0, "omg_conv2d_slots: w2_slot_stride must be a non-negative multiple of 8");
  }
  GemmP p{};
  const int rc = conv2d_params(&a->conv, p);
  if (rc != OMG_OK) return rc;
  OMG_REQUIRE(a->w_slot_stride == 0 || a->w_slot_stride >= (int64_t)p.N * p.K, "omg_conv2d_slots: w_slot_stride smaller than one weight");
  if (p.M == 0) return OMG_OK;
  const bool per_sample = a->group_adapter != nullptr && a->conv.B > 1;
  if (per_sample) {
    p.tile_groups = a->conv.B;
    p.tiles_m = (p.rows_per_group + BM - 1) / BM;
  }
  p.group_adapter = a->group_adapter;
  p.w_adapter_stride = a->w_slot_stride;
  p.A2 = (const char*)a->A2; p.lda2 = a->lda2; p.W2 = (const char*)a->W2; p.ldw2 = a->ldw2;
  p.K2 = a->K2; p.w2_adapter_stride = a->w2_slot_stride;
  if (p.K2 == 0) { p.A2 = nullptr; p.W2 = nullptr; }
  return conv2d_launch(a->conv.dtype, p, (hipStream_t)stream);
}
```

omg_amd/csrc/gemm_epilogue.h:

```cpp
#pragma once
#include "common.h"

namespace {

struct GemmP {
  int M, N, K;
  const char* A; long lda;
  const char* W; long ldw;
  const char* A2; long lda2;
  const char* W2; long ldw2;
  int K2, a2_col_block;
  int tile_groups, rows_per_group;
  const int* group_adapter;
  long w_adapter_stride, w2_adapter_stride;
  const char* bias;
  const char* group_bias; long ldgb;
  const char* residual; long ldr;
  int act; float out_scale;
  char* C; long ldc;
  int Hin, Win, C1, C2, Hout, Wout, ksize, stride, upsample;
  const char* X2;
  int tiles_m, tiles_n;
  int dbg;
  const char* SA; const char* SW;
  int sa_ld, sw_ld;
  long sw_adapter_stride;
  char* QS; int qs_ld;
};

typedef __attribute__((address_space(3))) void* lds_ptr_t;
typedef const __attribute__((address_space(1))) void* gbl_ptr_t;
OMG_DEV bool fold_group_bias(const GemmP& p) { return p.group_bias != nullptr && p.rows_per_group % 256 == 0; }

template <int N> OMG_DEV void wait_vmcnt() {
  static_assert(N >= 0 && N <= 63, "vmcnt range");
  asm volatile("s_waitcnt vmcnt(%0)" ::"n"(N) : "memory");
}


template <typename T>
OMG_DEV void swap_runs(unsigned (&q)[4]) {
  asm volatile("s_nop 4\n\tv_permlane32_swap_b32 %0, %2\n\tv_permlane32_swap_b32 %1, %3\n\ts_nop 4"
               : "+v"(q[0]), "+v"(q[1]), "+v"(q[2]), "+v"(q[3]));
}
constexpr int EPI_OOB = 0x7f000000;
OMG_DEV __amdgpu_buffer_rsrc_t epi_rsrc(const char* base, long bytes) {
  const unsigned long long a = (unsigned long long)base;
  const unsigned lo = __builtin_amdgcn_readfirstlane((unsigned)a), hi = __builtin_amdgcn_readfirstlane((unsigned)(a >> 32));
  const int n = __builtin_amdgcn_readfirstlane(base != nullptr ? (int)(bytes < 0x7effff00L ? bytes : 0x7effff00L) : 0);
  return __builtin_amdgcn_make_buffer_rsrc((void*)(((unsigned long long)hi << 32) | lo), 0, n, 0x00020000);
}
template <typename T>
OMG_DEV void decode_runs(const u32x4 raw, float (&f)[8]) {
  unsigned q[4] = {raw[0], raw[1], raw[2], raw[3]};
  swap_runs<T>(q);
  u32x4 sw = {q[0], q[1], q[2], q[3]};
  unpack8<T>(sw, f);
}
template <typename T>
OMG_DEV void load_runs(__amdgpu_buffer_rsrc_t rs, int off, int soff, float (&f)[8]) {
  decode_runs<T>(__builtin_amdgcn_raw_buffer_load_b128(rs, off, soff, 0), f);
}
template <typename T>
OMG_DEV void store_runs(__amdgpu_buffer_rsrc_t rs, int off, int soff, const float (&f)[8]) {
  u32x4 pk = pack8<T>(f);
  unsigned q[4] = {pk[0], pk[1], pk[2], pk[3]};
  swap_runs<T>(q);
  u32x4 sw = {q[0], q[1], q[2], q[3]};
  __builtin_amdgcn_raw_buffer_store_b128(sw, rs, off + soff, 0, 0);
}
template <typename T>
OMG_DEV void store_runs_dbg(__amdgpu_buffer_rsrc_t rs, int off, const float (&f)[8], bool nt, int pol) {
  u32x4 pk = pack8<T>(f);
  switch (pol) {
    case 1: __builtin_amdgcn_raw_buffer_store_b128(pk, rs, off, 0, 1); break;
    case 2: __builtin_amdgcn_raw_buffer_store_b128(pk, rs, off, 0, 16); break;
    case 3: __builtin_amdgcn_raw_buffer_store_b128(pk, rs, off, 0, 17); break;
    case 4: __builtin_amdgcn_raw_buffer_store_b128(pk, rs, off, 0, 3); break;
    case 5: __builtin_amdgcn_raw_buffer_store_b128(pk, rs, off, 0, 18); break;
    case 6: __builtin_amdgcn_raw_buffer_store_b128(pk, rs, off, 0, 19); break;
    default:
      if (nt) __builtin_amdgcn_raw_buffer_store_b128(pk, rs, off, 0, 2);
      else __builtin_amdgcn_raw_buffer_store_b128(pk, rs, off, 0, 0);
  }
}

template <typename T, int MT, int NT>
OMG_DEV bool acc_init_bias(const GemmP& p, f32x16 (&acc)[MT][NT], int lane, int m0, int wn0) {
  const int hi = lane >> 5;
  const bool fold_gb = fold_group_bias(p);
  const __amdgpu_buffer_rsrc_t rsB = epi_rsrc(p.bias, (long)p.N * 2);
  const __amdgpu_buffer_rsrc_t rsG = epi_rsrc(fold_gb ? p.group_bias + (long)(m0 / p.rows_per_group) * p.ldgb * 2 : nullptr, (long)p.N * 2);
  u32x4 rb[NT][2], rg[NT][2];
#pragma unroll
  for (int j = 0; j < NT; ++j)
#pragma unroll
    for (int pr = 0; pr < 2; ++pr) {
      const int c = wn0 + j * 32 + pr * 16 + hi * 8;
      rb[j][pr] = __builtin_amdgcn_raw_buffer_load_b128(rsB, c * 2, 0, 0);
      rg[j][pr] = __builtin_amdgcn_raw_buffer_load_b128(rsG, c * 2, 0, 0);
    }
#pragma unroll
  for (int j = 0; j < NT; ++j)
#pragma unroll
    for (int pr = 0; pr < 2; ++pr) {
      float f[8], g[8];
      decode_runs<T>(rb[j][pr], f);
      decode_runs<T>(rg[j][pr], g);
#pragma unroll
      for (int i = 0; i < MT; ++i)
#pragma unroll
        for (int e = 0; e < 8; ++e) acc[i][j][pr * 8 + e] = f[e] + g[e];
    }
  return p.group_bias != nullptr && !fold_gb;
}

template <int NT>
struct EpiCtx {
  __amdgpu_buffer_rsrc_t rsC, rsR, rsG;
  int hi, l31, wm0, m_end;
  int lane_col;
  int wn0, n_out;
  char* xl;
  const char* rl;
  int voob[NT][2];
};


template <typename T, int ROWB>
OMG_DEV void xe_put(const EpiCtx<4>& cx, int piece, const float (&v)[8]) {
  const u32x4 pk = pack8<T>(v);
  const int sw = ROWB == 256 ? (cx.l31 & 15) : ((cx.l31 >> 1) & 7);
  char* b = cx.xl + cx.l31 * ROWB + ((cx.hi ^ (cx.l31 >> 4)) << 3);
  const int c0 = piece ^ sw;
  const u32x2 r0 = {pk[0], pk[1]}, r1 = {pk[2], pk[3]};
  *(u32x2*)(b + (c0 << 4)) = r0;
  *(u32x2*)(b + ((c0 ^ 1) << 4)) = r1;
}
template <typename T, int ROWB>
OMG_DEV void xe_flush(const GemmP& p, const EpiCtx<4>& cx, int i, int col0) {
  constexpr int LPR = ROWB / 16;
  constexpr int RPI = 64 / LPR;
  constexpr int NU = 32 / RPI;
  asm volatile("s_waitcnt lgkmcnt(0)" ::: "memory");
  const int lane = cx.hi * 32 + cx.l31;
  const int rq = lane / LPR, c = lane % LPR;
  const bool col_ok = col0 + 8 * c < cx.n_out && !(p.dbg & 1024);
  const int colb = (col0 + 8 * c) * 2;
  u32x4 d[NU];
#pragma unroll
  for (int u = 0; u < NU; ++u) {
    const int rr = u * RPI + rq;
    const int sw = ROWB == 256 ? (rr & 15) : ((rr >> 1) & 7);
    const u32x4 x = *(const u32x4*)(cx.xl + rr * ROWB + ((c ^ sw) << 4));
    if (u * RPI >= 16) d[u] = u32x4{x[2], x[3], x[0], x[1]}; else d[u] = x;
  }
  if constexpr (ROWB == 128) {
    if (p.QS != nullptr) {
      const __amdgpu_buffer_rsrc_t rsQ = epi_rsrc(p.QS, (long)(cx.n_out >> 7) * p.qs_ld * 4);
      const int sbase = ((col0 >> 7) * p.qs_ld) * 4 + ((col0 >> 5) & 3);
#pragma unroll
      for (int u = 0; u < NU; ++u) {
        const int gm = cx.wm0 + i * 32 + u * RPI + rq;
        float f[8];
        unpack8<T>(d[u], f);
        float amax = 0.f;
#pragma unroll
        for (int e = 0; e < 8; ++e) amax = __builtin_fmaxf(amax, __builtin_fabsf(f[e]));
        amax = __builtin_fmaxf(amax, __shfl_xor(amax, 1));
        amax = __builtin_fmaxf(amax, __shfl_xor(amax, 2));
        const unsigned be = mx8_scale_exp(amax);
        const float inv = mx8_inv_scale(be);
        const u32x2 o = {mx8_pack4(f[0] * inv, f[1] * inv, f[2] * inv, f[3] * inv), mx8_pack4(f[4] * inv, f[5] * inv, f[6] * inv, f[7] * inv)};
        const bool ok = gm < cx.m_end && col_ok;
        __builtin_amdgcn_raw_buffer_store_b64(o, cx.rsC, ok ? gm * (int)p.ldc + col0 + 8 * c : EPI_OOB, 0, 0);
        const unsigned both = be | (__shfl_down(be, 4) << 8);
        __builtin_amdgcn_raw_buffer_store_b16((unsigned short)both, rsQ, (ok && c == 0) ? sbase + gm * 4 : EPI_OOB, 0, 0);
      }
      asm volatile("" ::: "memory");
      return;
    }
  }
#pragma unroll
  for (int u = 0; u < NU; ++u) {
    const int gm = cx.wm0 + i * 32 + u * RPI + rq;
// ... 167 lines not shown
```

omg_amd/csrc/gemm_v12.h:

```cpp
#include "gemm_v12_sched.inc"

template <typename T, int NT>
OMG_DEV void bias_issue(const GemmP& p, int lane, int m0, int wn0, u32x4 (&rb)[NT][2], u32x4 (&rg)[NT][2]) {
  const int hi = lane >> 5;
  const bool fold_gb = fold_group_bias(p);
  const __amdgpu_buffer_rsrc_t rsB = epi_rsrc(p.bias, (long)p.N * 2);
  const __amdgpu_buffer_rsrc_t rsG = epi_rsrc(fold_gb ? p.group_bias + (long)(m0 / p.rows_per_group) * p.ldgb * 2 : nullptr, (long)p.N * 2);
#pragma unroll
  for (int j = 0; j < NT; ++j)
#pragma unroll
    for (int pr = 0; pr < 2; ++pr) {
      const int c = wn0 + j * 32 + pr * 16 + hi * 8;
      rb[j][pr] = __builtin_amdgcn_raw_buffer_load_b128(rsB, c * 2, 0, 0);
      rg[j][pr] = __builtin_amdgcn_raw_buffer_load_b128(rsG, c * 2, 0, 0);
    }
}
template <typename T, int MT, int NT>
OMG_DEV void bias_apply(const u32x4 (&rb)[NT][2], const u32x4 (&rg)[NT][2], f32x16 (&acc)[MT][NT]) {
#pragma unroll
  for (int j = 0; j < NT; ++j)
#pragma unroll
    for (int pr = 0; pr < 2; ++pr) {
      float f[8], g[8];
      decode_runs<T>(rb[j][pr], f);
      decode_runs<T>(rg[j][pr], g);
#pragma unroll
      for (int i = 0; i < MT; ++i)
#pragma unroll
        for (int e = 0; e < 8; ++e) acc[i][j][pr * 8 + e] = f[e] + g[e];
    }
}

constexpr bool omg_is_next(unsigned tag) { return tag == 1u; }
OMG_DEV int fresh_lane() {
  int l = (int)__builtin_amdgcn_mbcnt_hi(~0u, __builtin_amdgcn_mbcnt_lo(~0u, 0u));
  asm volatile("" : "+v"(l));
  return l;
}
struct TileV12 { int m0, n0, m_end, grp; };
OMG_DEV TileV12 decode_tile_v12(const GemmP& p, int vb, int ntiles) {
  int bid = vb;
  {
    const int q = ntiles >> 3, r = ntiles & 7, xcd = bid & 7, idx = bid >> 3;
    bid = (xcd < r ? xcd * (q + 1) : r * (q + 1) + (xcd - r) * q) + idx;
  }
  const int tiles_per_group = p.tiles_m * p.tiles_n;
  const int grp = bid / tiles_per_group;
  const int t_in = bid - grp * tiles_per_group;
  constexpr int G = 8;
  const int per_group = G * p.tiles_n;
  const int gid = t_in / per_group;
  const int first_m = gid * G;
  const int gsz = (p.tiles_m - first_m) < G ? (p.tiles_m - first_m) : G;
  const int r = t_in - gid * per_group;
  const int tm = first_m + (r % gsz);
  const int tn = r / gsz;
  const int m_base = (p.tile_groups > 1) ? grp * p.rows_per_group : 0;
  TileV12 t;
  t.m_end = (p.tile_groups > 1) ? m_base + p.rows_per_group : p.M;
  t.m0 = m_base + tm * 256;
  t.n0 = tn * 256;
  t.grp = grp;
  return t;
}
OMG_DEV int next_tile_v12(const GemmP& p, int vb, int step, int ntiles) {
  if (p.w_adapter_stride == 0 || p.group_adapter == nullptr) return vb;
  while (vb < ntiles) {
    const TileV12 t = decode_tile_v12(p, vb, ntiles);
    if (p.group_adapter[t.grp] >= 0) break;
    vb += step;
  }
  return vb;
}

template <typename T, bool CONV, int EF>
__global__ __launch_bounds__(256, 1) void gemm_kernel_v12(GemmP p) {
  constexpr int MT = 4, NT = 4;
  constexpr bool XE = true;
  constexpr int BM_ = MT * 64, BN_ = NT * 64, BKc = 64;
  constexpr int AB = MT * 2, WB = NT * 2;
  constexpr int A_BYTES = BM_ * BKc * 2;
  constexpr int STAGE_BYTES = (BM_ + BN_) * BKc * 2;
  constexpr int HALF = 32768;
  static_assert(A_BYTES == HALF && STAGE_BYTES == 2 * HALF, "the ring's canonical roles are the two-stage layout");
  constexpr bool EARLY_RES = EF == 2;
  constexpr bool PERSIST = EF != 2;
  constexpr bool PREFETCH = PERSIST;
  static_assert(OMG_KS_LAST_TAILS >= 32, "32 prefetch DMAs / 32 residual DMAs");

  extern __shared__ __attribute__((aligned(16))) char smem[];
  const int tid = threadIdx.x;
  const int lane = tid & 63;
  const int w = __builtin_amdgcn_readfirstlane(tid >> 6);
  const int ntiles = p.tile_groups * p.tiles_m * p.tiles_n;
  const int step = PERSIST ? (int)gridDim.x : ntiles;
  const int nk = (p.K + BKc - 1) / BKc;

  const int Ctot = p.C1 + p.C2;
  const long a_bytes = CONV ? (long)p.M / (p.Hout * p.Wout) * p.Hin * p.Win * p.C1 * 2 : ((long)(p.M - 1) * p.lda + p.K) * 2;
  const __amdgpu_buffer_rsrc_t rsA = __builtin_amdgcn_make_buffer_rsrc((void*)p.A, 0, (int)(a_bytes < 0x7fffff00 ? a_bytes : 0x7fffff00), 0x00020000);
  const __amdgpu_buffer_rsrc_t rsA2 = __builtin_amdgcn_make_buffer_rsrc((void*)(CONV && p.X2 ? p.X2 : p.A), 0,
      CONV ? (int)((long)p.M / (p.Hout * p.Wout) * p.Hin * p.Win * p.C2 * 2) : 0, 0x00020000);
  const long w_bytes = ((long)(p.N - 1) * p.ldw + p.K) * 2;
  __amdgpu_buffer_rsrc_t rsW;

  const int prow = lane >> 3, ppos = lane & 7;
  int voffA[AB], voffW[WB];
  int cb[AB], cy[AB], cx[AB];
  const int dchunk = (ppos ^ ((w & 1) * 4 + (prow >> 1))) * 16;
  const int ldo = w * 1024;
  const int wm = w >> 1, wn = w & 1;
  f32x16 acc[MT][NT];
  using V8 = typename Vec<T>::v8;

  int vb = next_tile_v12(p, (int)blockIdx.x, step, ntiles);
  if (vb >= ntiles) return;
  int m0, n0, m_end;
#define OMG_TILE_SCALARS(t_)                                                                               \
  do {                                                                                                     \
    m0 = (t_).m0; n0 = (t_).n0; m_end = (t_).m_end;                                                        \
    int adapter_ = 0;                                                                                      \
    if (p.group_adapter != nullptr) adapter_ = p.group_adapter[(t_).grp];                                  \
    const char* Wp_ = p.W + (p.w_adapter_stride != 0 ? (long)adapter_ * p.w_adapter_stride * 2 : 0);       \
    rsW = __builtin_amdgcn_make_buffer_rsrc((void*)Wp_, 0, (int)w_bytes, 0x00020000);                      \
  } while (0)
#define OMG_ADDR_A(i_)                                                                                     \
  do {                                                                                                     \
    const int r_ = (w + (i_) * 4) * 8 + prow;                                                              \
    int gm_ = m0 + r_; if (gm_ > m_end - 1) gm_ = m_end - 1;                                               \
    if constexpr (CONV) {                                                                                  \
      const int hw_ = p.Hout * p.Wout;                                                                     \
      const int b_ = gm_ / hw_; const int rem_ = gm_ - b_ * hw_;                                           \
      cb[i_] = b_; cy[i_] = rem_ / p.Wout; cx[i_] = rem_ - cy[i_] * p.Wout;                                \
      voffA[i_] = 0;                                                                                       \
    } else {                                                                                               \
      cb[i_] = cy[i_] = cx[i_] = 0;                                                                        \
      voffA[i_] = (int)((long)gm_ * p.lda * 2) + dchunk;                                                   \
    }                                                                                                      \
  } while (0)
#define OMG_ADDR_W(i_)                                                                                     \
  do {                                                                                                     \
    const int r_ = (w + (i_) * 4) * 8 + prow;                                                              \
    int gn_ = n0 + r_; if (gn_ > p.N - 1) gn_ = p.N - 1;                                                   \
    voffW[i_] = (int)((long)gn_ * p.ldw * 2) + dchunk;                                                     \
  } while (0)
  {
    const TileV12 t = decode_tile_v12(p, vb, ntiles);
    OMG_TILE_SCALARS(t);
  }
#pragma unroll
  for (int i = 0; i < AB; ++i) OMG_ADDR_A(i);
#pragma unroll
  for (int i = 0; i < WB; ++i) OMG_ADDR_W(i);

  int koff = 0;
  int tap_dy = 0, tap_dx = 0, c0b = 0, xCb = 0;
  bool x2 = false;
  const int cpt = CONV ? Ctot / BKc : 1;
  const int pad = CONV ? (p.ksize == 3 ? 1 : 0) : 0;
  const int Hl = CONV ? (p.upsample ? p.Hin * 2 : p.Hin) : 0;
  const int Wl = CONV ? (p.upsample ? p.Win * 2 : p.Win) : 0;
#define OMG_PREP(kt_)                                                                                      \
  do {                                                                                                     \
    koff = (kt_) * (BKc * 2);                                                                              \
    if constexpr (CONV) {                                                                                  \
      const int tap = (kt_) / cpt; const int cc = (kt_) - tap * cpt;                                       \
      tap_dy = tap / p.ksize - pad; tap_dx = tap - (tap / p.ksize) * p.ksize - pad;                        \
      int c0 = cc * BKc;                                                                                   \
      x2 = c0 >= p.C1;                                                                                     \
      if (x2) c0 -= p.C1;                                                                                  \
      c0b = c0 * 2; xCb = (x2 ? p.C2 : p.C1) * 2;                                                          \
    }                                                                                                      \
  } while (0)
#define OMG_DMA(d_, nb_)                                                                                   \
  do {                                                                                                     \
    if ((d_) < AB) {                                                                                       \
      const int i_ = (d_) < AB ? (d_) : 0;                                                                 \
      if (CONV) dma16(x2 ? rsA2 : rsA, (nb_) + ldo + i_ * 4096,                                            \
                      conv_voff(cb[i_], cy[i_], cx[i_], dchunk, p.stride, tap_dy, tap_dx, Hl, Wl, p.upsample, p.Hin, p.Win, xCb, c0b), 0); \
      else dma16(rsA, (nb_) + ldo + i_ * 4096, voffA[i_], koff);                                           \
    } else {                                                                                               \
      const int i_ = (d_) >= AB ? (d_) - AB : 0;                                                           \
      dma16(rsW, (nb_) + A_BYTES + ldo + i_ * 4096, voffW[i_], koff);                                      \
    }                                                                                                      \
  } while (0)
#define OMG_DMAN(first_, n_, nb_)                                                                          \
  do { _Pragma("unroll") for (int d_ = 0; d_ < (n_); ++d_) OMG_DMA((first_) + d_, nb_); } while (0)
  V8 fw[4][NT], fa[4][MT];
  unsigned la[4], lw[4];
#define OMG_LA_LW(lane_)                                                                                   \
  do {                                                                                                     \
    const unsigned lds0_ = (unsigned)(unsigned long)(lds_ptr_t)smem;                                       \
    const int hi_ = (lane_) >> 5, l31_ = (lane_) & 31;                                                     \
    _Pragma("unroll") for (int ks = 0; ks < 4; ++ks) {                                                     \
      const unsigned sw_ = (unsigned)(((ks * 2 + hi_) ^ ((l31_ >> 1) & 7)) << 4);                          \
      la[ks] = lds0_ + (unsigned)((wm * (MT * 32) + l31_) * 128) + sw_;                                    \
      lw[ks] = lds0_ + (unsigned)((wn * (NT * 32) + l31_) * 128) + sw_;                                    \
    }                                                                                                      \
  } while (0)
  OMG_LA_LW(lane);
  int sa_cur, sw_cur, sa_nxt, sw_nxt, s_sp;
#define OMG_DMAR(d_)                                                                                       \
  do {                                                                                                     \
    if ((d_) < AB) {                                                                                       \
      const int i_ = (d_) < AB ? (d_) : 0;                                                                 \
      if (CONV) dma16(x2 ? rsA2 : rsA, smem + s_sp + ldo + i_ * 4096,                                      \
                      conv_voff(cb[i_], cy[i_], cx[i_], dchunk, p.stride, tap_dy, tap_dx, Hl, Wl, p.upsample, p.Hin, p.Win, xCb, c0b), 0); \
      else dma16(rsA, smem + s_sp + ldo + i_ * 4096, voffA[i_], koff);                                     \
    } else {                                                                                               \
      const int i_ = (d_) >= AB ? (d_) - AB : 0;                                                           \
      dma16(rsW, smem + sw_cur + ldo + i_ * 4096, voffW[i_], koff);                                        \
    }                                                                                                      \
  } while (0)
#define OMG_SB __builtin_amdgcn_sched_barrier(0)
#define OMG_XRD1(ks_, r_, tog_)                                                                            \
  do {                                                                                                     \
    constexpr bool isA_ = (r_) == 1 || (r_) > NT;                                                          \
    constexpr int idx_ = (r_) <= 1 ? 0 : (r_) <= NT ? (r_) - 1 : (r_) - NT;                                \
    const unsigned ad_ = (isA_ ? la[ks_] : lw[ks_]) + (unsigned)(omg_is_next(tog_) ? (isA_ ? sa_nxt : sw_nxt) : (isA_ ? sa_cur : sw_cur)); \
    if constexpr (isA_) asm volatile("ds_read_b128 %0, %1 offset:%2" : "=v"(fa[ks_][idx_]) : "v"(ad_), "n"(idx_ * 4096)); \
    else asm volatile("ds_read_b128 %0, %1 offset:%2" : "=v"(fw[ks_][idx_]) : "v"(ad_), "n"(idx_ * 4096));  \
  } while (0)
#define OMG_XMM1(ks_, n_) acc[(n_) / NT][(n_) % NT] = Vec<T>::mfma32(fw[ks_][(n_) % NT], fa[ks_][(n_) / NT], acc[(n_) / NT][(n_) % NT])
#define OMG_XMML(ks_, n_) do { OMG_XMM1(ks_, n_); asm volatile("" : "+a"(acc[(n_) / NT][(n_) % NT])); } while (0)
#define OMG_XWAIT(ks_, left_)                                                                              \
  asm volatile("s_waitcnt lgkmcnt(" #left_ ")"                                                             \
               : "+v"(fw[ks_][0]), "+v"(fw[ks_][1]), "+v"(fw[ks_][2]), "+v"(fw[ks_][3]),                   \
                 "+v"(fa[ks_][0]), "+v"(fa[ks_][1]), "+v"(fa[ks_][2]), "+v"(fa[ks_][3]))

  int e_m0 = 0, e_n0 = 0, e_mend = 0;
  int vbn = 0;
  int lane_l = 0; (void)lane_l;
  bool has_next = false;
  u32x4 rb[NT][2], rg[NT][2];
#define OMG_HEAD(n_)                                                                                       \
  do {                                                                                                     \
    if constexpr (PREFETCH) {       \
      if constexpr ((n_) == 0) {              \
        const TileV12 t_ = decode_tile_v12(p, has_next ? vbn : vb, ntiles);                                \
        OMG_TILE_SCALARS(t_);                                                                              \
      } else if constexpr ((n_) >= 1 && (n_) <= AB) {                                                      \
        OMG_ADDR_A((n_) >= 1 && (n_) <= AB ? (n_) - 1 : 0);                                                \
      } else if constexpr ((n_) > AB && (n_) <= AB + WB) {                                                 \
        OMG_ADDR_W((n_) > AB && (n_) <= AB + WB ? (n_) - 1 - AB : 0);                                      \
      }                                                                                                    \
    }                                                                                                      \
  } while (0)
#define OMG_TAIL(n_)                                                                                       \
  do {                                                                                                     \
    if constexpr (EARLY_RES) {                                                                             \
      if constexpr ((n_) == 0) lane_l = fresh_lane();                                 \
      if constexpr ((n_) < 32) {                                                      \
        constexpr int i_ = (n_) >> 3, u_ = (n_) & 7;                                                       \
        const int rr_ = u_ * 4 + (lane_l >> 4);                                                            \
        const int gm_ = e_m0 + wm * 128 + i_ * 32 + rr_;                                                   \
        const int col_ = e_n0 + wn * 128 + (((lane_l & 15) ^ (rr_ & 15)) << 3);                            \
        const int off_ = (gm_ < e_mend && col_ < p.N) ? (gm_ * (int)p.ldr + col_) * 2 : EPI_OOB;           \
        __builtin_amdgcn_raw_ptr_buffer_load_lds(rsRes, (lds_ptr_t)(smem + w * 32768 + i_ * 8192 + u_ * 1024), 16, off_, 0, 0, 0); \
      }                                                                                                    \
    }                                                                                                      \
    if constexpr (PREFETCH) {                                                                              \
      if constexpr ((n_) == 0) OMG_PREP(0);                                                                \
      if constexpr ((n_) == AB + WB) OMG_PREP(1);                                                          \
      if constexpr ((n_) < AB + WB) {                                                                      \
        if (has_next) OMG_DMA((n_) < AB + WB ? (n_) : 0, smem);                                            \
      } else if constexpr ((n_) < 2 * (AB + WB)) {                                                         \
        if (has_next && nk > 1) OMG_DMA((n_) >= AB + WB && (n_) < 2 * (AB + WB) ? (n_) - (AB + WB) : 0, smem + STAGE_BYTES); \
      }                                                                                                    \
    }                                                                                                      \
  } while (0)
  const __amdgpu_buffer_rsrc_t rsRes = epi_rsrc(EARLY_RES ? p.residual : nullptr, ((long)(p.M - 1) * p.ldr + p.N) * 2);
  const bool fold_gb = fold_group_bias(p);
  const bool gb_epi = p.group_bias != nullptr && !fold_gb;
  (void)rsRes;

  OMG_PREP(0);
  OMG_DMAN(0, AB + WB, smem);
  bias_issue<T, NT>(p, lane, m0, n0 + wn * (NT * 32), rb, rg);
  bias_apply<T, MT, NT>(rb, rg, acc);
  bool first = true;
  for (;;) {
    wait_vmcnt<0>();
    __builtin_amdgcn_s_barrier();
    if (!PREFETCH || first) {
      OMG_PREP(1);
      if (nk > 1) OMG_DMAN(0, AB + WB, smem + STAGE_BYTES);
    }
    sa_cur = 0; sw_cur = HALF; sa_nxt = 2 * HALF; sw_nxt = 3 * HALF; s_sp = 4 * HALF;
    { const unsigned tnxt = 1u; (void)tnxt; OMG_KS_PROLOGUE_5(); }
    e_m0 = m0; e_n0 = n0; e_mend = m_end;
    if constexpr (PERSIST) { vbn = next_tile_v12(p, vb + step, step, ntiles); has_next = vbn < ntiles; }

    int kt = 0;
#define OMG_KS_VARS const unsigned tcur = 0u; const unsigned tnxt = 1u; (void)tnxt; (void)tcur
#define OMG_KS_ROT do { const int t_ = sa_cur; sa_cur = sa_nxt; sa_nxt = s_sp; s_sp = t_; const int u_ = sw_cur; sw_cur = sw_nxt; sw_nxt = u_; } while (0)
    for (; kt < nk - 2; ++kt) { OMG_KS_VARS; OMG_KS_STAGE_5(true, true); OMG_KS_ROT; }
    if (kt < nk - 1) { OMG_KS_VARS; OMG_KS_STAGE_5(true, false); OMG_KS_ROT; ++kt; }
    { OMG_KS_VARS; OMG_KS_LAST_5(); }

    const int lane_e = PERSIST ? fresh_lane() : lane;
    if constexpr (EF == 2) {
      if constexpr (!EARLY_RES) res_stage_dma(p, smem + w * 32768, lane_e, e_m0 + wm * 128, e_n0 + wn * 128, e_mend);
      epilogue_direct<T, MT, NT, XE, EF>(p, acc, lane_e, e_m0 + wm * (MT * 32), e_n0 + wn * (NT * 32), e_mend, gb_epi, smem + 2 * STAGE_BYTES + w * 8192,
                                         smem + w * 32768);
    } else
    epilogue_direct<T, MT, NT, XE, EF>(p, acc, lane_e, e_m0 + wm * (MT * 32), e_n0 + wn * (NT * 32), e_mend, gb_epi, smem + 2 * STAGE_BYTES + w * 8192);
    if (!PERSIST || !has_next) break;
    vb = vbn;
    first = false;
    { const int lane_n = fresh_lane(); OMG_LA_LW(lane_n); }
    if constexpr (!PREFETCH) {
      const TileV12 t = decode_tile_v12(p, vb, ntiles);
      OMG_TILE_SCALARS(t);
#pragma unroll
      for (int i = 0; i < AB; ++i) OMG_ADDR_A(i);
#pragma unroll
      for (int i = 0; i < WB; ++i) OMG_ADDR_W(i);
      OMG_PREP(0);
      OMG_DMAN(0, AB + WB, smem);
    }
    bias_issue<T, NT>(p, lane, m0, n0 + wn * (NT * 32), rb, rg);
    bias_apply<T, MT, NT>(rb, rg, acc);
  }
#undef OMG_KS_VARS
#undef OMG_KS_ROT
#undef OMG_HEAD
#undef OMG_TAIL
#undef OMG_DMAR
#undef OMG_XWAIT
#undef OMG_XMM1
#undef OMG_XMML
#undef OMG_XRD1
#undef OMG_SB
#undef OMG_PREP
#undef OMG_DMA
#undef OMG_DMAN
#undef OMG_ADDR_A
#undef OMG_LA_LW
#undef OMG_ADDR_W
#undef OMG_TILE_SCALARS
}

template <typename T, bool CONV, int EF>
int launch_v12(GemmP p, hipStream_t s, int mrows) {
  constexpr int lds = 2 * (256 + 256) * 64 * 2 + 4 * 8192;
  static bool attr = false;
  if (!attr) {
    attr = true;
    (void)hipFuncSetAttribute((const void*)gemm_kernel_v12<T, CONV, EF>, hipFuncAttributeMaxDynamicSharedMemorySize, lds);
  }
  p.tiles_m = (mrows + 255) / 256;
  p.tiles_n = (p.N + 255) / 256;
  p.dbg = g_dbg;
  const int ntiles = p.tile_groups * p.tiles_m * p.tiles_n;
  if (ntiles <= 0) return OMG_OK;
  int grid = ntiles;
  if (EF != 2) {
    int cus = num_cus() & ~7;
    if (g_dbg & 0x10000) cus = 8;
    if (grid > cus && cus > 0) grid = cus;
  }
  OMG_LAUNCH((gemm_kernel_v12<T, CONV, EF>), dim3(grid), dim3(256), lds, s, p);
  return omg_check_launch("gemm_v12");
}
template <typename T, bool CONV>
int launch_v12_form(const GemmP& p, hipStream_t s, int mrows) {
  const bool gb_rows = p.group_bias != nullptr && p.rows_per_group % 256 != 0;
  if (p.act == OMG_ACT_GEGLU) return launch_v12<T, CONV, 3>(p, s, mrows);
  if (gb_rows || p.act == OMG_ACT_SILU) return launch_v12<T, CONV, 4>(p, s, mrows);
  if (p.residual != nullptr) return launch_v12<T, CONV, 2>(p, s, mrows);
  return launch_v12<T, CONV, 1>(p, s, mrows);
}
```

omg_amd/csrc/gemm_v13.h:

```cpp

template <typename T> struct MfmaAsm;
template <> struct MfmaAsm<f16> {
  static OMG_DEV void a(f32x16& c, f16x8 x, f16x8 y) { asm volatile("v_mfma_f32_32x32x16_f16 %0, %1, %2, %0" : "+a"(c) : "v"(x), "v"(y)); }
  static OMG_DEV void v(f32x16& c, f16x8 x, f16x8 y) { asm volatile("v_mfma_f32_32x32x16_f16 %0, %1, %2, %0" : "+v"(c) : "v"(x), "v"(y)); }
};
template <> struct MfmaAsm<bf16> {
  static OMG_DEV void a(f32x16& c, bf16x8 x, bf16x8 y) { asm volatile("v_mfma_f32_32x32x16_bf16 %0, %1, %2, %0" : "+a"(c) : "v"(x), "v"(y)); }
  static OMG_DEV void v(f32x16& c, bf16x8 x, bf16x8 y) { asm volatile("v_mfma_f32_32x32x16_bf16 %0, %1, %2, %0" : "+v"(c) : "v"(x), "v"(y)); }
};
OMG_DEV void acc_fence(f32x16 (&acc)[4][5]) {
  asm volatile("s_nop 15\n\ts_nop 15" : "+a"(acc[0][0]), "+a"(acc[0][1]), "+a"(acc[0][2]), "+a"(acc[0][3]), "+v"(acc[0][4]));
  asm volatile("" : "+a"(acc[1][0]), "+a"(acc[1][1]), "+a"(acc[1][2]), "+a"(acc[1][3]), "+v"(acc[1][4]));
  asm volatile("" : "+a"(acc[2][0]), "+a"(acc[2][1]), "+a"(acc[2][2]), "+a"(acc[2][3]), "+v"(acc[2][4]));
  asm volatile("" : "+a"(acc[3][0]), "+a"(acc[3][1]), "+a"(acc[3][2]), "+a"(acc[3][3]), "+v"(acc[3][4]));
}

#define OMG_V13_COL(j_, wn0_, wn4_) ((j_) < 4 ? (wn0_) + (j_) * 32 : (wn4_))

template <typename T>
OMG_DEV bool acc_init_bias13(const GemmP& p, f32x16 (&acc)[4][5], int lane, int m0, int wn0, int wn4) {
  const int hi = lane >> 5;
  const bool fold_gb = fold_group_bias(p);
  const __amdgpu_buffer_rsrc_t rsB = epi_rsrc(p.bias, (long)p.N * 2);
  const __amdgpu_buffer_rsrc_t rsG = epi_rsrc(fold_gb ? p.group_bias + (long)(m0 / p.rows_per_group) * p.ldgb * 2 : nullptr, (long)p.N * 2);
// ... 9 lines not shown
#pragma unroll
  for (int j = 0; j < 5; ++j)
#pragma unroll
    for (int pr = 0; pr < 2; ++pr) {
      float f[8], g[8];
      decode_runs<T>(rb[j][pr], f);
      decode_runs<T>(rg[j][pr], g);
#pragma unroll
      for (int i = 0; i < 4; ++i)
#pragma unroll
        for (int e = 0; e < 8; ++e) acc[i][j][pr * 8 + e] = f[e] + g[e];
    }
  return p.group_bias != nullptr && !fold_gb;
}

template <typename T, bool RS, bool GENERIC>
OMG_DEV void epilogue_rows13(const GemmP& p, f32x16 (&acc)[4][5], const EpiCtx<5>& cx, const EpiCtx<4>& cx4, int lane_col4, bool has_gb) {
  const float osc = p.out_scale;
  const bool has_rs = GENERIC ? p.residual != nullptr : RS;
  u32x4 rraw[2][5][2];
#define OMG_V13_LCOL(j_) ((j_) < 4 ? cx.lane_col : lane_col4)
#define OMG_V13_SOFF(j_, pr_) ((((j_) < 4 ? (j_) * 32 : 0) + (pr_) * 16) * 2)
#define OMG_FETCH_RES13(i_, buf_)                                                                          \
  do {                                                                                                     \
    const int gm_ = cx.wm0 + (i_) * 32 + cx.l31;                                                           \
    const int rrow_ = gm_ < cx.m_end ? gm_ * (int)p.ldr * 2 : EPI_OOB;                                     \
    _Pragma("unroll") for (int j = 0; j < 5; ++j)                                                          \
      _Pragma("unroll") for (int pr = 0; pr < 2; ++pr)                                                     \
        rraw[buf_][j][pr] = __builtin_amdgcn_raw_buffer_load_b128(cx.rsR, (rrow_ + OMG_V13_LCOL(j)) | cx.voob[j][pr], OMG_V13_SOFF(j, pr), 0); \
  } while (0)
  if (has_rs) OMG_FETCH_RES13(0, 0);
#pragma unroll
  for (int i = 0; i < 4; ++i) {
    const int gm = cx.wm0 + i * 32 + cx.l31;
    const bool row_ok = gm < cx.m_end;
    if (has_rs && i + 1 < 4) OMG_FETCH_RES13(i + 1, (i + 1) & 1);
    const int crow = row_ok ? gm * (int)p.ldc * 2 : EPI_OOB;
    const int grow = GENERIC && has_gb && row_ok ? ((gm / p.rows_per_group) * (int)p.ldgb) * 2 : EPI_OOB;
#pragma unroll
    for (int j = 0; j < 5; ++j)
#pragma unroll
      for (int pr = 0; pr < 2; ++pr) {
        float v[8];
#pragma unroll
        for (int e = 0; e < 8; ++e) v[e] = acc[i][j][pr * 8 + e];
        if constexpr (GENERIC) {
          if (has_gb) {
            float f[8];
            load_runs<T>(cx.rsG, (grow + OMG_V13_LCOL(j)) | cx.voob[j][pr], OMG_V13_SOFF(j, pr), f);
#pragma unroll
            for (int e = 0; e < 8; ++e) v[e] += f[e];
          }
          if (p.act == OMG_ACT_SILU) {
#pragma unroll
            for (int e = 0; e < 8; ++e) v[e] = silu_fast(v[e]);
          }
        }
        if (has_rs) {
          const u32x4 rr = rraw[i & 1][j][pr];
          unsigned q[4] = {rr[0], rr[1], rr[2], rr[3]};
          swap_runs<T>(q);
          u32x4 sw = {q[0], q[1], q[2], q[3]};
          float rf[8];
          unpack8<T>(sw, rf);
#pragma unroll
          for (int e = 0; e < 8; ++e) v[e] = __builtin_fmaf(v[e], osc, rf[e]);
        } else {
#pragma unroll
          for (int e = 0; e < 8; ++e) v[e] *= osc;
        }
        if (j < 4) xe_put<T, 256>(cx4, 4 * j + 2 * pr, v);
        else store_runs<T>(cx.rsC, (crow + OMG_V13_LCOL(j)) | cx.voob[j][pr], OMG_V13_SOFF(j, pr), v);
        __builtin_amdgcn_sched_barrier(0);
      }
    xe_flush<T, 256>(p, cx4, i, cx4.wn0);
  }
#undef OMG_FETCH_RES13
#undef OMG_V13_SOFF
#undef OMG_V13_LCOL
}

template <typename T, int EF>
OMG_DEV void epilogue13(const GemmP& p, f32x16 (&acc)[4][5], int lane, int wm0, int wn0, int wn4, int m_end, bool has_gb, char* xl) {
  static_assert(EF == 1 || EF == 4 || EF == 5, "forms of the 256 x 320 tile: bias only, generic, residual");
  EpiCtx<5> cx;
  cx.hi = lane >> 5; cx.l31 = lane & 31; cx.wm0 = wm0; cx.m_end = m_end;
  cx.rsC = epi_rsrc(p.C, ((long)(p.M - 1) * p.ldc + p.N) * 2);
  cx.rsR = epi_rsrc(p.residual, ((long)(p.M - 1) * p.ldr + p.N) * 2);
  cx.rsG = epi_rsrc(has_gb ? p.group_bias : nullptr, 0x7effff00L);
#pragma unroll
  for (int j = 0; j < 5; ++j)
#pragma unroll
    for (int pr = 0; pr < 2; ++pr) cx.voob[j][pr] = (OMG_V13_COL(j, wn0, wn4) + pr * 16 + cx.hi * 8 < p.N && !(p.dbg & 1024)) ? 0 : EPI_OOB;
  cx.lane_col = (wn0 + cx.hi * 8) * 2;
  cx.wn0 = wn0; cx.n_out = p.N; cx.xl = xl; cx.rl = nullptr;
  const int lane_col4 = (wn4 + cx.hi * 8) * 2;
  EpiCtx<4> cx4;
  cx4.rsC = cx.rsC; cx4.rsR = cx.rsR; cx4.rsG = cx.rsG;
  cx4.hi = cx.hi; cx4.l31 = cx.l31; cx4.wm0 = wm0; cx4.m_end = m_end; cx4.lane_col = cx.lane_col; cx4.wn0 = wn0; cx4.n_out = p.N; cx4.xl = xl; cx4.rl = nullptr;
#pragma unroll
  for (int j = 0; j < 4; ++j)
#pragma unroll
    for (int pr = 0; pr < 2; ++pr) cx4.voob[j][pr] = cx.voob[j][pr];
  if constexpr (EF == 1) epilogue_rows13<T, false, false>(p, acc, cx, cx4, lane_col4, false);
  else if constexpr (EF == 5) epilogue_rows13<T, true, false>(p, acc, cx, cx4, lane_col4, false);
  else epilogue_rows13<T, false, true>(p, acc, cx, cx4, lane_col4, has_gb);
}

template <typename T, bool CONV, int EF>
__global__ __launch_bounds__(256, 1) void gemm_kernel_v13(GemmP p) {
  constexpr int MT = 4, NT = 5;
  constexpr int BM_ = MT * 64, BN_ = NT * 64, BKc = 64;
  constexpr int AB = MT * 2, WB = NT * 2;
  constexpr int NMM = MT * NT;
  constexpr int SLOTS = NMM / 2;
  constexpr int NRD = MT + NT;
  constexpr int A_BYTES = BM_ * BKc * 2;
  constexpr int STAGE_BYTES = (BM_ + BN_) * BKc * 2;
  static_assert(2 * STAGE_BYTES <= 160 * 1024, "two stages in LDS");

  const bool ts_on = (p.dbg & 16) && blockIdx.x < 8192 && threadIdx.x == 0;
  long long ts0 = 0, ts1 = 0, ts2 = 0;
  if (p.dbg & 16) ts0 = __builtin_amdgcn_s_memrealtime();
  extern __shared__ __attribute__((aligned(16))) char smem[];
  const int tid = threadIdx.x;
  const int lane = tid & 63;
  const int w = __builtin_amdgcn_readfirstlane(tid >> 6);
  const int hi = lane >> 5;
  const int l31 = lane & 31;

  const int nwg = gridDim.x;
  int bid = blockIdx.x;
  {
    const int q = nwg >> 3, r = nwg & 7, xcd = bid & 7, idx = bid >> 3;
    bid = (xcd < r ? xcd * (q + 1) : r * (q + 1) + (xcd - r) * q) + idx;
  }
  const int tiles_per_group = p.tiles_m * p.tiles_n;
  const int grp = bid / tiles_per_group;
  const int t_in = bid - grp * tiles_per_group;
  int tm, tn;
  {
    const int per_group = 8 * p.tiles_n;
    const int gid = t_in / per_group;
    const int first_m = gid * 8;
    const int gsz = (p.tiles_m - first_m) < 8 ? (p.tiles_m - first_m) : 8;
    const int r = t_in - gid * per_group;
    tm = first_m + (r % gsz);
    tn = r / gsz;
  }
  const int m_base = (p.tile_groups > 1) ? grp * p.rows_per_group : 0;
  const int m_end = (p.tile_groups > 1) ? m_base + p.rows_per_group : p.M;
  const int m0 = m_base + tm * BM_;
  const int n0 = tn * BN_;
  int adapter = 0;
  if (p.group_adapter != nullptr) adapter = p.group_adapter[grp];
  if (p.w_adapter_stride != 0 && adapter < 0) return;
  const char* Wp = p.W + (p.w_adapter_stride != 0 ? (long)adapter * p.w_adapter_stride * 2 : 0);
  const int nk = (p.K + BKc - 1) / BKc;

  const int Ctot = p.C1 + p.C2;
  const long a_bytes = CONV ? (long)p.M / (p.Hout * p.Wout) * p.Hin * p.Win * p.C1 * 2 : ((long)(p.M - 1) * p.lda + p.K) * 2;
  const __amdgpu_buffer_rsrc_t rsA = __builtin_amdgcn_make_buffer_rsrc((void*)p.A, 0, (int)(a_bytes < 0x7fffff00 ? a_bytes : 0x7fffff00), 0x00020000);
  const __amdgpu_buffer_rsrc_t rsA2 = __builtin_amdgcn_make_buffer_rsrc((void*)(CONV && p.X2 ? p.X2 : p.A), 0,
      CONV ? (int)((long)p.M / (p.Hout * p.Wout) * p.Hin * p.Win * p.C2 * 2) : 0, 0x00020000);
  const long w_bytes = ((long)(p.N - 1) * p.ldw + p.K) * 2;
  const __amdgpu_buffer_rsrc_t rsW = __builtin_amdgcn_make_buffer_rsrc((void*)Wp, 0, (int)w_bytes, 0x00020000);

  const int prow = lane >> 3, ppos = lane & 7;
  int voffA[AB], voffW[WB];
  int cb[AB], cy[AB], cx[AB];
  const int dchunk = (ppos ^ ((w & 1) * 4 + (prow >> 1))) * 16;
#pragma unroll
  for (int i = 0; i < AB; ++i) {
    const int r = (w + i * 4) * 8 + prow;
    int gm = m0 + r; if (gm > m_end - 1) gm = m_end - 1;
    if constexpr (CONV) {
      const int hw = p.Hout * p.Wout;
      const int b = gm / hw; const int rem = gm - b * hw;
      cb[i] = b; cy[i] = rem / p.Wout; cx[i] = rem - cy[i] * p.Wout;
      voffA[i] = 0;
    } else {
      cb[i] = cy[i] = cx[i] = 0;
      voffA[i] = (int)((long)gm * p.lda * 2) + dchunk;
    }
  }
#pragma unroll
  for (int i = 0; i < WB; ++i) {
    const int r = (w + i * 4) * 8 + prow;
    int gn = n0 + r; if (gn > p.N - 1) gn = p.N - 1;
    voffW[i] = (int)((long)gn * p.ldw * 2) + dchunk;
  }
  const int ldo = w * 1024;

  const int wm = w >> 1, wn = w & 1;
  const int wn0 = n0 + wn * 128, wn4 = n0 + 256 + wn * 32;
  f32x16 acc[MT][NT];
  using V8 = typename Vec<T>::v8;
  int aoff[4], boff[4], boff4[4];
#pragma unroll
  for (int ks = 0; ks < 4; ++ks) {
    const int sw = ((ks * 2 + hi) ^ ((l31 >> 1) & 7)) << 4;
    aoff[ks] = (wm * (MT * 32) + l31) * 128 + sw;
    boff[ks] = A_BYTES + (wn * 128 + l31) * 128 + sw;
    boff4[ks] = A_BYTES + (256 + wn * 32 + l31) * 128 + sw;
  }

  int koff = 0;
  int tap_dy = 0, tap_dx = 0, c0b = 0, xCb = 0;
  bool x2 = false;
  const int cpt = CONV ? Ctot / BKc : 1;
  const int pad = CONV ? (p.ksize == 3 ? 1 : 0) : 0;
  const int Hl = CONV ? (p.upsample ? p.Hin * 2 : p.Hin) : 0;
  const int Wl = CONV ? (p.upsample ? p.Win * 2 : p.Win) : 0;
#define OMG_PREP(kt_)                                                                                      \
  do {                                                                                                     \
    koff = (kt_) * (BKc * 2);                                                                              \
    if constexpr (CONV) {                                                                                  \
      const int tap = (kt_) / cpt; const int cc = (kt_) - tap * cpt;                                       \
      tap_dy = tap / p.ksize - pad; tap_dx = tap - (tap / p.ksize) * p.ksize - pad;                        \
      int c0 = cc * BKc;                                                                                   \
      x2 = c0 >= p.C1;                                                                                     \
      if (x2) c0 -= p.C1;                                                                                  \
      c0b = c0 * 2; xCb = (x2 ? p.C2 : p.C1) * 2;                                                          \
    }                                                                                                      \
  } while (0)
#define OMG_DMA(d_, nb_)                                                                                   \
  do {                                                                                                     \
    if ((d_) < AB) {                                                                                       \
      const int i_ = (d_) < AB ? (d_) : 0;                                                                 \
      if (CONV) dma16(x2 ? rsA2 : rsA, (nb_) + ldo + i_ * 4096,                                            \
                      conv_voff(cb[i_], cy[i_], cx[i_], dchunk, p.stride, tap_dy, tap_dx, Hl, Wl, p.upsample, p.Hin, p.Win, xCb, c0b), 0); \
      else dma16(rsA, (nb_) + ldo + i_ * 4096, voffA[i_], koff);                                           \
    } else {                                                                                               \
      const int i_ = (d_) - AB < WB ? (d_) - AB : 0;                                                       \
      dma16(rsW, (nb_) + A_BYTES + ldo + i_ * 4096, voffW[i_], koff);                                      \
    }                                                                                                      \
  } while (0)
#define OMG_DMAN(first_, n_, nb_)                                                                          \
  do { _Pragma("unroll") for (int d_ = 0; d_ < (n_); ++d_) OMG_DMA((first_) + d_, nb_); } while (0)
#define OMG_WFRAG(sb_, ks_, j_) (*(const V8*)((sb_) + ((j_) < 4 ? boff[ks_] + (j_) * 4096 : boff4[ks_])))
#define OMG_RD(f_, sb_, ks_)                                                                               \
  do {                                                                                                     \
    _Pragma("unroll") for (int j = 0; j < NT; ++j) bf[f_][j] = OMG_WFRAG(sb_, ks_, j);                     \
    _Pragma("unroll") for (int i = 0; i < MT; ++i) af[f_][i] = *(const V8*)((sb_) + aoff[ks_] + i * 4096); \
  } while (0)
#define OMG_RD1(f_, sb_, ks_, r_)                                                                          \
  do {                                                                                                     \
    const bool isA_ = (r_) == 1 || (r_) > NT;                                                              \
    const int idx_ = (r_) <= 1 ? 0 : (r_) <= NT ? (r_) - 1 : (r_) - NT;                                    \
    if (!isA_) bf[f_][idx_] = OMG_WFRAG(sb_, ks_, idx_);                                                   \
    else af[f_][idx_] = *(const V8*)((sb_) + aoff[ks_] + idx_ * 4096);                                     \
  } while (0)
#define OMG_MM1(f_, n_)                                                                                    \
  do {                                                                                                     \
    if ((n_) % NT == 4) MfmaAsm<T>::v(acc[(n_) / NT][4], bf[f_][4], af[f_][(n_) / NT]);                    \
    else MfmaAsm<T>::a(acc[(n_) / NT][(n_) % NT], bf[f_][(n_) % NT], af[f_][(n_) / NT]);                   \
  } while (0)
#define OMG_KSTEP(f_, RD_, rb_, rks_, DMA_, d0_, dn_, db_)                                                 \
  do {                                                                                                     \
    constexpr int RPS_ = (RD_) == 2 ? 2 : (NRD + SLOTS - 1) / SLOTS;                                       \
    constexpr int DPS_ = ((dn_) + SLOTS - 1) / SLOTS;                                                      \
    _Pragma("unroll") for (int s_ = 0; s_ < SLOTS; ++s_) {                                                 \
      OMG_MM1(f_, 2 * s_);                                                                                 \
      __builtin_amdgcn_sched_barrier(0);                                                                   \
      if ((RD_) != 0) {                                                                                    \
        _Pragma("unroll") for (int q_ = 0; q_ < RPS_; ++q_)                                                \
          if (s_ * RPS_ + q_ < NRD) OMG_RD1(1 - (f_), rb_, rks_, s_ * RPS_ + q_);                          \
      }                                                                                                    \
      __builtin_amdgcn_sched_barrier(0);                                                                   \
      OMG_MM1(f_, 2 * s_ + 1);                                                                             \
      __builtin_amdgcn_sched_barrier(0);                                                                   \
      if (DMA_) {                                                                                          \
        _Pragma("unroll") for (int q_ = 0; q_ < DPS_; ++q_)                                                \
          if (s_ * DPS_ + q_ < (dn_)) OMG_DMA((d0_) + s_ * DPS_ + q_, db_);                                \
      }                                                                                                    \
      __builtin_amdgcn_sched_barrier(0);                                                                   \
    }                                                                                                      \
  } while (0)

  V8 af[2][MT], bf[2][NT];
  OMG_PREP(0);
  OMG_DMAN(0, AB + WB, smem);
  const bool gb_epi = acc_init_bias13<T>(p, acc, lane, m0, wn0, wn4);
  wait_vmcnt<0>();
  __builtin_amdgcn_s_barrier();
  if (p.dbg & 16) ts1 = __builtin_amdgcn_s_memrealtime();
  OMG_PREP(1);
  if (nk > 1) OMG_DMAN(0, AB, smem + STAGE_BYTES);
  OMG_RD(0, smem, 0);
  acc_fence(acc);

#define OMG_STAGE(HAS1_, HAS2_)                                                                            \
  do {                                                                                                     \
    const char* cur = smem + (kt & 1) * STAGE_BYTES;                                                       \
    char* nxt = smem + ((kt + 1) & 1) * STAGE_BYTES;                                                       \
    OMG_KSTEP(0, 1, cur, 1, HAS1_, AB, WB, nxt);                                                           \
    OMG_KSTEP(1, 1, cur, 2, false, 0, 0, nxt);                                                             \
    OMG_KSTEP(0, 1, cur, 3, false, 0, 0, nxt);                                                             \
     \
    asm volatile("s_waitcnt vmcnt(0) lgkmcnt(0)" ::: "memory"); __builtin_amdgcn_s_barrier();              \
    if (HAS2_) OMG_PREP(kt + 2);                                                                           \
    OMG_KSTEP(1, (HAS1_) ? 2 : 0, nxt, 0, HAS2_, 0, AB, (char*)cur);                                       \
  } while (0)
  int kt = 0;
  for (; kt < nk - 2; ++kt) OMG_STAGE(true, true);
  if (kt < nk - 1) { OMG_STAGE(true, false); ++kt; }
// ... 57 lines not shown
```

omg_amd/modules.py:

```python
from __future__ import annotations

from typing import Optional

import torch
from torch import nn

from . import _lib as L
from . import ops


class LoraState:

    __slots__ = ("group_adapter", "groups", "merged")

    def __init__(self, group_adapter: torch.Tensor, groups: int, merged: bool = False):
        self.group_adapter = group_adapter
        self.groups = groups
        self.merged = merged


_POINTER_EPOCH = [0]


def pointer_epoch() -> int:
    return _POINTER_EPOCH[0]


def bump_weights_version(net) -> None:
    net.weights_version = getattr(net, "weights_version", 0) + 1


def bump_pointer_epoch() -> None:
    _POINTER_EPOCH[0] += 1


class _Packed(nn.Module):
    def __init__(self):
        super().__init__()
        self._packed = {}

    def invalidate_packed(self):
        if self._packed:
            bump_pointer_epoch()
        self._packed = {}

    def _load_from_state_dict(self, *a, **k):
        self.invalidate_packed()
        return super()._load_from_state_dict(*a, **k)

    def _apply(self, fn, *a, **k):
        self.invalidate_packed()
        return super()._apply(fn, *a, **k)


class Linear(_Packed):

    def __init__(self, in_features: int, out_features: int, bias: bool = True, dtype=torch.float16, device=None):
        super().__init__()
        self.in_features, self.out_features = in_features, out_features
        self.weight = nn.Parameter(torch.empty(out_features, in_features, dtype=dtype, device=device), requires_grad=False)
        self.bias = nn.Parameter(torch.empty(out_features, dtype=dtype, device=device), requires_grad=False) if bias else None
        self.lora_down: Optional[torch.Tensor] = None
        self.lora_up: Optional[torch.Tensor] = None
        self.w_slots: Optional[torch.Tensor] = None
        self.lora_state: Optional[LoraState] = None
        self.mx8 = False

    def invalidate_mx8_slots(self) -> None:
        if self._packed.pop("mx8_slots", None) is not None:
            bump_pointer_epoch()

    def _mx8_ok(self) -> bool:
        st = self.lora_state
        return self.in_features % 128 == 0 and not (st is not None and not st.merged and self.lora_down is not None)

    def _forward_mx8(self, x, residual, act):
        xq = x if isinstance(x, ops.Mx8Tensor) else ops.quant_mx8(x)
        shp = xq.shape
        r2 = residual.reshape(-1, self.out_features) if residual is not None else None
        st = self.lora_state
        dt = self.weight.dtype
        if st is not None and st.merged and self.w_slots is not None:
            if "mx8_slots" not in self._packed:
                self._packed["mx8_slots"] = ops.quant_mx8(self.w_slots.reshape(-1, self.in_features))
            y = ops.gemm_mx8(xq, self._packed["mx8_slots"], out_dtype=dt, bias=self.bias, residual=r2, act=act, groups=st.groups,
                             w_group_adapter=st.group_adapter, n_per_adapter=self.out_features)
        else:
            if "mx8_w" not in self._packed:
                self._packed["mx8_w"] = ops.quant_mx8(self.weight.data)
            y = ops.gemm_mx8(xq, self._packed["mx8_w"], out_dtype=dt, bias=self.bias, residual=r2, act=act)
        return y.view(*shp[:-1], y.shape[-1])

    def _lora(self, x2: torch.Tensor) -> Optional[ops.LoraSpec]:
        st = self.lora_state
        if st is None or st.merged or self.lora_down is None:
            return None
        t = ops.gemm(x2, self.lora_down, groups=st.groups, w_group_adapter=st.group_adapter)
        return ops.LoraSpec(t, self.lora_up, st.group_adapter)

    def forward(self, x: torch.Tensor, scale=None, *, residual: Optional[torch.Tensor] = None, act: int = L.ACT_NONE,
                group_bias: Optional[torch.Tensor] = None, groups: int = 1) -> torch.Tensor:
        if isinstance(x, ops.Mx8Tensor) or (self.mx8 and group_bias is None and self._mx8_ok()):
            if group_bias is not None or not self._mx8_ok():
                raise L.OmgHipError("an MX-fp8 activation reached a Linear layer that cannot run in MX-fp8")
            return self._forward_mx8(x, residual, act)
        shp = x.shape
        x2 = x.reshape(-1, shp[-1])
        r2 = residual.reshape(-1, self.out_features) if residual is not None else None
        st = self.lora_state
        if st is not None and st.merged and self.w_slots is not None:
            y = ops.gemm(x2, self.w_slots, bias=self.bias, residual=r2, act=act, groups=st.groups, w_group_adapter=st.group_adapter)
            return y.view(*shp[:-1], y.shape[-1])
        lora = self._lora(x2)
        if lora is not None:
            groups = self.lora_state.groups
            if x2.shape[0] % groups != 0:
                raise L.OmgHipError("LoRA groups do not divide the row count")
        y = ops.gemm(x2, self.weight, bias=self.bias, residual=r2, act=act, group_bias=group_bias, groups=groups, lora=lora)
        return y.view(*shp[:-1], y.shape[-1])


class GEGLU(_Packed):

    def __init__(self, dim_in: int, dim_out: int, dtype=torch.float16, device=None):
        super().__init__()
        self.proj = Linear(dim_in, dim_out * 2, dtype=dtype, device=device)

    def _packed_w(self):
        if "w" not in self._packed:
            perm = ops.geglu_row_perm(self.proj.out_features).to(self.proj.weight.device)
            self._packed["w"] = self.proj.weight.data[perm].contiguous()
            self._packed["b"] = self.proj.bias.data[perm].contiguous()
            if self.proj.lora_up is not None:
                self._packed["up"] = self.proj.lora_up[:, perm].contiguous()
            if self.proj.w_slots is not None:
                self._packed["w_slots"] = self.proj.w_slots[:, perm].contiguous()
        return self._packed

    def invalidate_packed(self):
        super().invalidate_packed()

    def _forward_mx8(self, x, out_mx8: bool = False):
        xq = x if isinstance(x, ops.Mx8Tensor) else ops.quant_mx8(x)
        shp = xq.shape
        pk = self._packed_w()
        st = self.proj.lora_state
        dt = self.proj.weight.dtype
        out_mx8 = out_mx8 and self.proj.out_features % 256 == 0
        if st is not None and st.merged and "w_slots" in pk:
            if "mx8_slots" not in pk:
                pk["mx8_slots"] = ops.quant_mx8(pk["w_slots"].reshape(-1, self.proj.in_features))
            y = ops.gemm_mx8(xq, pk["mx8_slots"], out_dtype=dt, bias=pk["b"], act=L.ACT_GEGLU, groups=st.groups,
                             w_group_adapter=st.group_adapter, n_per_adapter=self.proj.out_features, out_mx8=out_mx8)
        else:
            if "mx8_w" not in pk:
                pk["mx8_w"] = ops.quant_mx8(pk["w"])
            y = ops.gemm_mx8(xq, pk["mx8_w"], out_dtype=dt, bias=pk["b"], act=L.ACT_GEGLU, out_mx8=out_mx8)
        if isinstance(y, ops.Mx8Tensor):
            return y
        return y.view(*shp[:-1], y.shape[-1])

    def forward(self, x, out_mx8: bool = False):
        if isinstance(x, ops.Mx8Tensor) or (self.proj.mx8 and self.proj._mx8_ok()):
            return self._forward_mx8(x, out_mx8)
        shp = x.shape
        x2 = x.reshape(-1, shp[-1])
        pk = self._packed_w()
        lora = None
        groups = 1
        st = self.proj.lora_state
        if st is not None and st.merged and "w_slots" in pk:
            y = ops.gemm(x2, pk["w_slots"], bias=pk["b"], act=L.ACT_GEGLU, groups=st.groups, w_group_adapter=st.group_adapter)
            return y.view(*shp[:-1], y.shape[-1])
        if st is not None and not st.merged and self.proj.lora_down is not None:
            t = ops.gemm(x2, self.proj.lora_down, groups=st.groups, w_group_adapter=st.group_adapter)
            lora = ops.LoraSpec(t, pk["up"], st.group_adapter)
            groups = st.groups
        y = ops.gemm(x2, pk["w"], bias=pk["b"], act=L.ACT_GEGLU, groups=groups, lora=lora)
        return y.view(*shp[:-1], y.shape[-1])


class Conv2d(_Packed):

    def __init__(self, cin: int, cout: int, ksize: int, stride: int = 1, dtype=torch.float16, device=None):
        super().__init__()
        self.cin, self.cout, self.ksize, self.stride = cin, cout, ksize, stride
        self.weight = nn.Parameter(torch.empty(cout, cin, ksize, ksize, dtype=dtype, device=device), requires_grad=False)
        self.bias = nn.Parameter(torch.empty(cout, dtype=dtype, device=device), requires_grad=False)
        self.mx8 = False
        self.lora_down: Optional[torch.Tensor] = None
        self.lora_up: Optional[torch.Tensor] = None
        self.w_slots: Optional[torch.Tensor] = None
        self.lora_state: Optional[LoraState] = None

    def lora_eligible(self) -> bool:
        return self.weight.dtype != torch.float32 and self.cin % 64 == 0 and self.cout % 8 == 0

    def has_lora_slots(self) -> bool:
        return self.w_slots is not None or self.lora_down is not None

    def packed_weight(self) -> torch.Tensor:
        if "w" not in self._packed:
            self._packed["w"] = ops.pack_conv_weight(self.weight.data)
        return self._packed["w"]

    def wino_weight(self) -> Optional[torch.Tensor]:
        if self.ksize != 3 or self.stride != 1 or self.cin % 8 != 0 or self.weight.dtype != torch.float32:
            return None
        if "wu" not in self._packed:
            self._packed["wu"] = ops.pack_conv_weight_wino(self.weight.data)
        return self._packed["wu"]

    def mx8_ok(self) -> bool:
        return not self.has_lora_slots() and self.mx8 and self.ksize == 3 and self.stride == 1 and self.cin % 32 == 0 and self.weight.dtype != torch.float32

    def mx8_weight(self) -> "ops.Mx8Tensor":
        if "wq" not in self._packed:
            w = self.packed_weight()
            cq = (self.cin + 127) // 128 * 128
            if cq != self.cin:
                wp = torch.zeros((self.cout, 9, cq), dtype=w.dtype, device=w.device)
                wp[:, :, :self.cin] = w.view(self.cout, 9, self.cin)
                w = wp.view(self.cout, 9 * cq)
            self._packed["wq"] = ops.quant_mx8(w)
        return self._packed["wq"]

    def forward(self, x: torch.Tensor, *, x2: Optional[torch.Tensor] = None, upsample: bool = False,
                group_bias: Optional[torch.Tensor] = None, residual: Optional[torch.Tensor] = None) -> torch.Tensor:
        if isinstance(x, ops.Mx8Map):
            if not self.mx8_ok() or x2 is not None or upsample:
                raise L.OmgHipError("an MX-fp8 feature map can only feed a 3x3 / stride 1 convolution in MX-fp8 mode")
            return ops.conv2d_mx8(x, self.mx8_weight(), bias=self.bias, group_bias=group_bias, residual=residual)
        if self.weight.dtype == torch.float32:
            if x2 is not None or group_bias is not None or self.stride != 1:
                raise L.OmgHipError("the fp32 convolution supports stride 1 without concat / per-sample bias (all the VAE decoder needs)")
            return ops.conv2d_f32(x, self.packed_weight(), self.ksize, upsample=upsample, bias=self.bias, residual=residual,
                                  wu=self.wino_weight())
        st = self.lora_state
        if st is not None and self.has_lora_slots():
            if x.shape[0] != st.groups:
                raise L.OmgHipError("LoRA groups do not match the batch of the convolution")
            if st.merged and self.w_slots is not None:
                return ops.conv2d(x, self.w_slots, self.ksize, stride=self.stride, upsample=upsample, x2=x2, bias=self.bias,
                                  group_bias=group_bias, residual=residual, w_group_adapter=st.group_adapter)
            if not st.merged and self.lora_down is not None:
                t = ops.conv2d(x, self.lora_down, self.ksize, stride=self.stride, upsample=upsample, x2=x2, w_group_adapter=st.group_adapter)
                return ops.conv2d(x, self.packed_weight(), self.ksize, stride=self.stride, upsample=upsample, x2=x2, bias=self.bias,
                                  group_bias=group_bias, residual=residual, lora=ops.LoraSpec(t, self.lora_up, st.group_adapter))
        return ops.conv2d(x, self.packed_weight(), self.ksize, stride=self.stride, upsample=upsample, x2=x2, bias=self.bias,
                          group_bias=group_bias, residual=residual)


def lora_conv_targets(net) -> dict:
    return {n: m for n, m in net.named_modules() if isinstance(m, Conv2d) and n not in ("conv_in", "conv_out") and m.lora_eligible()}


class GroupNorm(nn.Module):
    def __init__(self, groups: int, channels: int, eps: float, dtype=torch.float16, device=None):
        super().__init__()
        self.groups, self.eps = groups, eps
        self.weight = nn.Parameter(torch.empty(channels, dtype=dtype, device=device), requires_grad=False)
        self.bias = nn.Parameter(torch.empty(channels, dtype=dtype, device=device), requires_grad=False)

    def forward(self, x: torch.Tensor, *, x2: Optional[torch.Tensor] = None, silu: bool = False, mx8: bool = False):
        if mx8:
            return ops.groupnorm_mx8(x, self.weight, self.bias, self.groups, self.eps, silu=silu, x2=x2)
        return ops.groupnorm(x, self.weight, self.bias, self.groups, self.eps, silu=silu, x2=x2)


class LayerNorm(nn.Module):
    def __init__(self, channels: int, eps: float = 1e-5, dtype=torch.float16, device=None):
# ... 16 lines not shown
```

omg_amd/ops.py:

```python
from __future__ import annotations

import ctypes as C
import os
from typing import Optional, Sequence, Tuple

import torch

from . import _lib as L

_DT = {torch.float16: L.OMG_F16, torch.bfloat16: L.OMG_BF16}


def _dt(t: torch.Tensor, allow_f32: bool = False) -> int:
    if allow_f32 and t.dtype == torch.float32:
        return L.OMG_F32
    try:
        return _DT[t.dtype]
    except KeyError:
        raise L.OmgHipError(f"unsupported dtype {t.dtype}; use float16 or bfloat16") from None


def _dev(t: torch.Tensor) -> None:
    if not t.is_cuda:
        raise L.OmgHipError("omg_amd ops need tensors on the MI355X (cuda/hip device); there is no CPU fallback")


def _stream() -> int:
    return torch.cuda.current_stream().cuda_stream


def _p(t: Optional[torch.Tensor]) -> Optional[int]:
    return None if t is None else t.data_ptr()


class KernelProfiler:

    def __init__(self):
        self.records = []

    def begin(self):
        e = torch.cuda.Event(enable_timing=True)
        e.record(torch.cuda.current_stream())
        return e

    def end(self, kind: str, flops: float, start, tag=None) -> None:
        e = torch.cuda.Event(enable_timing=True)
        e.record(torch.cuda.current_stream())
        self.records.append((kind, flops, start, e, tag))

    def summary(self):
        out = {}
        for kind, fl, s, e, _ in self.records:
            d = out.setdefault(kind, dict(launches=0, ms=0.0, flops=0.0))
            d["launches"] += 1
            d["ms"] += s.elapsed_time(e)
            d["flops"] += fl
        return out

    def by_tag(self):
        out = {}
        for kind, fl, s, e, tag in self.records:
            d = out.setdefault((kind, tag), dict(launches=0, ms=0.0, flops=0.0))
            d["launches"] += 1
            d["ms"] += s.elapsed_time(e)
            d["flops"] += fl
        return sorted(out.items(), key=lambda kv: -kv[1]["ms"])


_PROF: Optional[KernelProfiler] = None


def set_profiler(p: Optional[KernelProfiler]) -> None:
    global _PROF
    _PROF = p


class LoraSpec:

    __slots__ = ("a2", "w2", "group_adapter", "a2_col_block")

    def __init__(self, a2: torch.Tensor, w2: torch.Tensor, group_adapter: Optional[torch.Tensor] = None,
                 a2_col_block: int = 0):
        self.a2, self.w2, self.group_adapter, self.a2_col_block = a2, w2, group_adapter, a2_col_block


def gemm(a: torch.Tensor, w: torch.Tensor, *, bias: Optional[torch.Tensor] = None,
         residual: Optional[torch.Tensor] = None, act: int = L.ACT_NONE, out: Optional[torch.Tensor] = None,
         out_scale: float = 1.0, group_bias: Optional[torch.Tensor] = None, groups: int = 1,
         lora: Optional[LoraSpec] = None, w_group_adapter: Optional[torch.Tensor] = None) -> torch.Tensor:
    _dev(a)
    M, K = a.shape
    assert a.stride(1) == 1
    if w.dim() == 3:
        N = w.shape[1]
        w_stride = w.stride(0)
        ldw = w.stride(1)
    else:
        N = w.shape[0]
        w_stride = 0
        ldw = w.stride(0)
    assert w.shape[-1] == K and w.stride(-1) == 1
    n_out = N // 2 if act == L.ACT_GEGLU else N
    if out is None:
        out = torch.empty((M, n_out), dtype=a.dtype, device=a.device)
    assert out.stride(1) == 1 and out.shape[0] == M and out.shape[1] == n_out
    args = L.GemmArgs()
    args.dtype = _dt(a)
    args.M, args.N, args.K = M, N, K
    args.A, args.lda = a.data_ptr(), a.stride(0)
    args.W, args.ldw = w.data_ptr(), ldw
    args.groups = groups
    args.rows_per_group = M // groups
    adapter = w_group_adapter
    if lora is not None:
        a2, w2 = lora.a2, lora.w2
        args.A2, args.lda2 = a2.data_ptr(), a2.stride(0)
        args.K2 = w2.shape[-1]
        args.W2 = w2.data_ptr()
        if w2.dim() == 3:
            args.ldw2, args.w2_adapter_stride = w2.stride(1), w2.stride(0)
        else:
            args.ldw2, args.w2_adapter_stride = w2.stride(0), 0
        args.a2_col_block = lora.a2_col_block
        if lora.group_adapter is not None:
            adapter = lora.group_adapter
    args.group_adapter = _p(adapter)
    args.w_adapter_stride = w_stride
    args.bias = _p(bias)
    if group_bias is not None:
        args.group_bias, args.ldgb = group_bias.data_ptr(), group_bias.stride(0)
    if residual is not None:
        assert residual.stride(1) == 1
        args.residual, args.ldr = residual.data_ptr(), residual.stride(0)
    args.act = act
    args.out_scale = out_scale
    args.C, args.ldc = out.data_ptr(), out.stride(0)
    if _PROF is not None:
        t0 = _PROF.begin()
        L.check(L.lib().omg_gemm(C.byref(args), _stream()), "omg_gemm")
        _PROF.end("gemm", 2.0 * M * N * (K + args.K2), t0, ("lin", M, N, K, args.K2, groups if adapter is not None else 1, act))
        return out
    L.check(L.lib().omg_gemm(C.byref(args), _stream()), "omg_gemm")
    return out


class Mx8Tensor:

    __slots__ = ("q", "scales", "rows", "K", "shape")

    def __init__(self, q: torch.Tensor, scales: torch.Tensor, shape=None):
        self.q, self.scales, self.rows, self.K = q, scales, q.shape[0], q.shape[1]
        self.shape = tuple(shape) if shape is not None else (q.shape[0], q.shape[1])

    @property
    def device(self):
        return self.q.device


def quant_mx8(x: torch.Tensor, out: Optional[Mx8Tensor] = None) -> Mx8Tensor:
    _dev(x)
    shape = x.shape
    x = x.reshape(-1, shape[-1])
    assert x.stride(1) == 1
    M, K = x.shape
    if K % 128 != 0:
        raise L.OmgHipError("MX-fp8 operands need K % 128 == 0")
    if out is None:
        s_ld = (M + 3) // 4 * 4
        out = Mx8Tensor(torch.empty((M, K), dtype=torch.uint8, device=x.device),
                        torch.zeros((K // 128, s_ld), dtype=torch.int32, device=x.device), shape)
    assert out.q.shape == (M, K) and out.q.stride(1) == 1 and out.scales.shape[0] == K // 128
    L.check(L.lib().omg_quant_mx8(_dt(x), x.data_ptr(), x.stride(0), M, K, out.q.data_ptr(), out.q.stride(0),
                                  out.scales.data_ptr(), out.scales.stride(0), _stream()), "omg_quant_mx8")
    return out


def gemm_mx8(a: Mx8Tensor, w: Mx8Tensor, *, out_dtype: torch.dtype = torch.float16, bias: Optional[torch.Tensor] = None,
             residual: Optional[torch.Tensor] = None, act: int = L.ACT_NONE, out: Optional[torch.Tensor] = None,
             out_scale: float = 1.0, groups: int = 1, w_group_adapter: Optional[torch.Tensor] = None,
             n_per_adapter: Optional[int] = None, out_mx8: bool = False):
    M, K = a.rows, a.K
    assert w.K == K
    N = n_per_adapter if w_group_adapter is not None else w.rows
    n_out = N // 2 if act == L.ACT_GEGLU else N
    oq = None
    if out_mx8:
        assert out is None and act == L.ACT_GEGLU and N % 256 == 0
        oq = Mx8Tensor(torch.empty((M, n_out), dtype=torch.uint8, device=a.q.device),
                       torch.empty((n_out // 128, (M + 3) // 4 * 4), dtype=torch.int32, device=a.q.device), tuple(a.shape[:-1]) + (n_out,))
        out = oq.q
    elif out is None:
        out = torch.empty((M, n_out), dtype=out_dtype, device=a.q.device)
    assert out.stride(1) == 1 and out.shape == (M, n_out)
    g = L.GemmMx8Args()
    g.dtype = _DT[out_dtype] if out_mx8 else _dt(out)
    g.M, g.N, g.K = M, N, K
    g.A, g.lda, g.a_scale, g.sa_ld = a.q.data_ptr(), a.q.stride(0), a.scales.data_ptr(), a.scales.stride(0)
    g.W, g.ldw, g.w_scale, g.sw_ld = w.q.data_ptr(), w.q.stride(0), w.scales.data_ptr(), w.scales.stride(0)
    g.groups, g.rows_per_group = groups, M // groups
    if w_group_adapter is not None:
        g.group_adapter = w_group_adapter.data_ptr()
        g.w_adapter_stride, g.sw_adapter_stride = N * w.q.stride(0), N
    g.bias = _p(bias)
    if residual is not None:
        assert residual.stride(1) == 1
        g.residual, g.ldr = residual.data_ptr(), residual.stride(0)
    g.act, g.out_scale = act, out_scale
    g.C, g.ldc = out.data_ptr(), out.stride(0)
    if oq is not None:
        g.c_scale, g.sc_ld = oq.scales.data_ptr(), oq.scales.stride(0)
    if _PROF is not None:
        t0 = _PROF.begin()
        L.check(L.lib().omg_gemm_mx8(C.byref(g), _stream()), "omg_gemm_mx8")
        _PROF.end("gemm_mx8", 2.0 * M * N * K, t0, ("mx8", M, N, K, 0, groups if w_group_adapter is not None else 1, act))
        return oq if oq is not None else out
    L.check(L.lib().omg_gemm_mx8(C.byref(g), _stream()), "omg_gemm_mx8")
    return oq if oq is not None else out


def conv2d(x1: torch.Tensor, w: torch.Tensor, ksize: int, *, stride: int = 1, upsample: bool = False,
           x2: Optional[torch.Tensor] = None, bias: Optional[torch.Tensor] = None,
           group_bias: Optional[torch.Tensor] = None, residual: Optional[torch.Tensor] = None,
           out_scale: float = 1.0, act: int = L.ACT_NONE, w_group_adapter: Optional[torch.Tensor] = None,
           lora: Optional[LoraSpec] = None, out: Optional[torch.Tensor] = None) -> torch.Tensor:
    _dev(x1)
    B, Hin, Win, C1 = x1.shape
    assert x1.is_contiguous()
    C2 = 0
    if x2 is not None:
        assert x2.is_contiguous() and x2.shape[:3] == x1.shape[:3]
        C2 = x2.shape[3]
    slots = w.dim() == 3 or w_group_adapter is not None or lora is not None
    Cout = w.shape[-2]
    assert w.is_contiguous() and w.shape[-1] == ksize * ksize * (C1 + C2)
    Hl, Wl = (2 * Hin, 2 * Win) if upsample else (Hin, Win)
    pad = 1 if ksize == 3 else 0
    Hout = (Hl + 2 * pad - ksize) // stride + 1
    Wout = (Wl + 2 * pad - ksize) // stride + 1
    if out is None:
        y = torch.empty((B, Hout, Wout, Cout), dtype=x1.dtype, device=x1.device)
    else:
        y = out
        assert y.is_contiguous() and tuple(y.shape) == (B, Hout, Wout, Cout) and y.dtype == x1.dtype
    sa = L.Conv2dSlotsArgs() if slots else None
    a = sa.conv if slots else L.Conv2dArgs()
    a.dtype = _dt(x1)
    a.B, a.Hin, a.Win, a.C1, a.C2 = B, Hin, Win, C1, C2
    a.Hout, a.Wout, a.Cout = Hout, Wout, Cout
    a.ksize, a.stride, a.upsample = ksize, stride, int(upsample)
    a.X1, a.X2, a.W, a.bias = x1.data_ptr(), _p(x2), w.data_ptr(), _p(bias)
    if group_bias is not None:
        a.group_bias, a.ldgb = group_bias.data_ptr(), group_bias.stride(0)
    if residual is not None:
        assert residual.is_contiguous() and residual.shape == y.shape
        a.residual = residual.data_ptr()
    a.out_scale = out_scale
    a.act = act
    a.Y = y.data_ptr()
    k2 = 0
    if slots:
        adapter = w_group_adapter
        sa.w_slot_stride = w.stride(0) if w.dim() == 3 else 0
        if lora is not None:
            a2, w2 = lora.a2, lora.w2
            a2 = a2.reshape(-1, a2.shape[-1])
            assert a2.stride(1) == 1 and a2.shape[0] == B * Hout * Wout and w2.stride(-1) == 1 and w2.shape[-2] == Cout and lora.a2_col_block == 0
            k2 = w2.shape[-1]
            sa.A2, sa.lda2, sa.W2, sa.K2 = a2.data_ptr(), a2.stride(0), w2.data_ptr(), k2
            if w2.dim() == 3:
                sa.ldw2, sa.w2_slot_stride = w2.stride(1), w2.stride(0)
            else:
                sa.ldw2, sa.w2_slot_stride = w2.stride(0), 0
            if lora.group_adapter is not None:
                adapter = lora.group_adapter
        if adapter is not None:
            assert adapter.dtype == torch.int32 and adapter.is_cuda and adapter.numel() == B
        sa.group_adapter = _p(adapter)
        fn, what, arg = L.lib().omg_conv2d_slots, "omg_conv2d_slots", sa
    else:
        fn, what, arg = L.lib().omg_conv2d, "omg_conv2d", a
    if _PROF is not None:
        t0 = _PROF.begin()
        L.check(fn(C.byref(arg), _stream()), what)
        K = ksize * ksize * (C1 + C2)
        _PROF.end("gemm", 2.0 * B * Hout * Wout * Cout * (K + k2), t0, ("conv", B * Hout * Wout, Cout, K, k2, B if slots else 1, 0))
        return y
    L.check(fn(C.byref(arg), _stream()), what)
    return y


class Mx8Map:

    __slots__ = ("q", "scales", "shape", "dtype")

    def __init__(self, q: torch.Tensor, scales: torch.Tensor, dtype: torch.dtype):
        self.q, self.scales, self.shape, self.dtype = q, scales, tuple(q.shape), dtype

    @property
    def device(self):
        return self.q.device


def groupnorm_mx8(x1: torch.Tensor, gamma: torch.Tensor, beta: torch.Tensor, groups: int, eps: float, *,
                  silu: bool = False, x2: Optional[torch.Tensor] = None) -> Mx8Map:
    _dev(x1)
    assert x1.is_contiguous() and x1.dim() == 4
    B, H, W, C1 = x1.shape
    C2 = 0
    if x2 is not None:
        assert x2.is_contiguous() and x2.shape[:3] == x1.shape[:3]
        C2 = x2.shape[-1]
    Cc = C1 + C2
    if Cc % 32 != 0:
        raise L.OmgHipError("MX-fp8 feature maps need C % 32 == 0")
    Cq = (Cc + 127) // 128 * 128
    out = Mx8Map(torch.empty((B, H, W, Cq), dtype=torch.uint8, device=x1.device),
                 torch.empty((Cq // 128, B * H * W), dtype=torch.int32, device=x1.device), x1.dtype)
    ws = _gn_workspace(x1.device, B, groups, H * W)
    assert gamma.dtype == x1.dtype and beta.dtype == x1.dtype
    L.check(L.lib().omg_groupnorm_mx8(_dt(x1), x1.data_ptr(), C1, _p(x2), C2, B, H * W, groups, eps, gamma.data_ptr(), beta.data_ptr(),
                                      int(silu), ws.data_ptr(), out.q.data_ptr(), out.scales.data_ptr(), _stream()), "omg_groupnorm_mx8")
    return out


def conv2d_mx8(x: Mx8Map, w: "Mx8Tensor", *, bias: Optional[torch.Tensor] = None, group_bias: Optional[torch.Tensor] = None,
               residual: Optional[torch.Tensor] = None, out_scale: float = 1.0, act: int = L.ACT_NONE) -> torch.Tensor:
    _dev(x.q)
    B, H, W, Cin = x.shape
    Cout = w.rows
    assert w.K == 9 * Cin
    y = torch.empty((B, H, W, Cout), dtype=x.dtype, device=x.device)
    a = L.Conv2dMx8Args()
    a.dtype = _DT[x.dtype]
# ... 512 lines not shown
```

Baseline: 0.4176.

## Skip Q/K projection tiles for batch rows whose attention scores are borrowed

Adds a per-group skip table to the fp16 GEMM so tiles whose rows belong to batch entries whose QK scores come from another row (via the controller's qk_src mapping), and whose columns lie in the Q/K part, exit early. A persistent-tile v12 variant and the per-tile kernels check the table. This cuts redundant projection FLOPs in the concept-fusion branches. It leaves those Q/K outputs uninitialised, adds kernel template variants, and sends SiLU or row-group-bias cases to an older kernel.

```diff
diff --git a/include/omg_hip.h b/include/omg_hip.h
--- a/include/omg_hip.h
+++ b/include/omg_hip.h
@@ -47,6 +47,8 @@
   int32_t act;
   float out_scale;
   void* C; int64_t ldc;
+  const int32_t* group_skip;
+  int32_t skip_n_end;
 } omg_gemm_args;
 
 int omg_gemm(const omg_gemm_args* a, void* stream);
diff --git a/omg_amd/_lib.py b/omg_amd/_lib.py
--- a/omg_amd/_lib.py
+++ b/omg_amd/_lib.py
@@ -25,6 +25,7 @@
         ("residual", c_vp), ("ldr", c_i64),
         ("act", c_i32), ("out_scale", c_f32),
         ("C", c_vp), ("ldc", c_i64),
+        ("group_skip", c_vp), ("skip_n_end", c_i32),
     ]
 
 
diff --git a/omg_amd/attention.py b/omg_amd/attention.py
--- a/omg_amd/attention.py
+++ b/omg_amd/attention.py
@@ -8,6 +8,9 @@
 from . import _lib as L
 from . import ops
 from .modules import Dropout, Linear, LoraState, bump_pointer_epoch, pointer_epoch
+
+
+DEAD_ROW_SKIP = True
 
 
 class Attention(nn.Module):
@@ -114,7 +117,7 @@
             self._kv_slots = torch.cat([self.to_k.w_slots, self.to_v.w_slots], dim=1).contiguous()
         return self._kv_slots
 
-    def project_self(self, x):
+    def project_self(self, x, group_skip: Optional[ops.GroupSkip] = None):
         B, N, C = x.shape
         inner = self.inner_dim
         if isinstance(x, ops.Mx8Tensor) or (self.to_q.mx8 and C % 128 == 0 and not self._has_lora()):
@@ -134,13 +137,14 @@
             qkv = qkv.view(B, N, 3 * inner)
             return qkv[:, :, :inner], qkv[:, :, inner:2 * inner], ops.value_operand(qkv[:, :, 2 * inner:], self.heads)
         if self._has_lora():
-            q = self.to_q(x); k = self.to_k(x); v = self.to_v(x)
+            q = self.to_q(x, group_skip=group_skip, skip_n_end=inner); k = self.to_k(x, group_skip=group_skip, skip_n_end=inner); v = self.to_v(x)
         else:
             st = self._merged()
             if st is not None:
-                qkv = ops.gemm(x.reshape(B * N, C), self.qkv_slots(), groups=st.groups, w_group_adapter=st.group_adapter)
+                qkv = ops.gemm(x.reshape(B * N, C), self.qkv_slots(), groups=st.groups, w_group_adapter=st.group_adapter,
+                               group_skip=group_skip, skip_n_end=2 * inner)
             else:
-                qkv = ops.gemm(x.reshape(B * N, C), self.qkv_weight())
+                qkv = ops.gemm(x.reshape(B * N, C), self.qkv_weight(), group_skip=group_skip, skip_n_end=2 * inner)
             qkv = qkv.view(B, N, 3 * inner)
             q, k, v = qkv[:, :, :inner], qkv[:, :, inner:2 * inner], qkv[:, :, 2 * inner:]
         return q, k, ops.value_operand(v, self.heads)
@@ -227,6 +231,9 @@
     def _skip_layer(self) -> None:
         return None
 
+    def _qk_skip(self, batch: int, device, main_batch=None, images=1):
+        return None
+
     def __call__(self, attn: Attention, hidden_states, encoder_hidden_states=None, attention_mask=None, temb=None,
                  scale: float = 1.0, residual: Optional[torch.Tensor] = None, **cross_attention_kwargs):
         if attention_mask is not None:
@@ -234,11 +241,6 @@
         x = _to_tokens(attn, hidden_states)
         B, N, _ = x.shape
         is_cross = encoder_hidden_states is not None
-        if is_cross:
-            q = attn.to_q(x)
-            k, vt = attn.project_cross(encoder_hidden_states)
-        else:
-            q, k, vt = attn.project_self(x)
         bypass = cross_attention_kwargs.pop("omg_bypass_controller", False)
         main_b = cross_attention_kwargs.pop("omg_main_batch", None)
         n_img = cross_attention_kwargs.pop("omg_images", 1)
@@ -248,6 +250,14 @@
         src = None if (bypass or twin) else self._qk_src(attn, is_cross, N, B, x.device, main_b, n_img)
         ip_ctx = cross_attention_kwargs.pop("omg_ip_tokens", None)
         ip_row0 = cross_attention_kwargs.pop("omg_ip_rows", 0)
+        skip = self._qk_skip(B, x.device, main_b, n_img) if (src is not None and DEAD_ROW_SKIP) else None
+        if skip is not None and is_cross and ip_ctx is not None and attn.ip_kv_weight is not None and any(skip.flags[ip_row0:]):
+            skip = None
+        if is_cross:
+            q = attn.to_q(x, group_skip=skip, skip_n_end=attn.inner_dim)
+            k, vt = attn.project_cross(encoder_hidden_states)
+        else:
+            q, k, vt = attn.project_self(x, group_skip=skip)
         o = ops.attention(q, k, vt, attn.heads, attn.scale, qk_src=src)
         if is_cross and ip_ctx is not None and attn.ip_kv_weight is not None:
             _ip_branch(attn, q, o, ip_ctx, ip_row0)
@@ -310,6 +320,9 @@
             return None
         return self.controller.fused_qk_src(is_cross, n_tokens, main_batch or batch, self.place_in_unet, device=device,
                                             total_batch=batch, images=images)
+
+    def _qk_skip(self, batch, device, main_batch=None, images=1):
+        return self.controller.qk_skip_vector(main_batch or batch, device, total_batch=batch, images=images)
 
     def _skip_layer(self) -> None:
         if self.controller is not None:
diff --git a/omg_amd/controller.py b/omg_amd/controller.py
--- a/omg_amd/controller.py
+++ b/omg_amd/controller.py
@@ -142,6 +142,7 @@
         self._identity_mapper = all(torch.equal(m.float().cpu(), eye) for m in self.mapper)
         self.is_pure_replacement = bool(local_blend is None and self._identity_mapper and bool((self.cross_replace_alpha == 1).all()))
         self._src_cache: Dict[Tuple, torch.Tensor] = {}
+        self._skip_cache: Dict[Tuple, object] = {}
         ident = bool(all(torch.equal(m, eye) for m in self._mapper_host))
         self._cross_kinds = ["borrow" if ident and bool((a == 1).all()) else "own" if bool((a == 0).all()) else "mixed"
                              for a in self._alpha_host]
@@ -209,6 +210,17 @@
             v += list(range(batch * images, total))
             t = torch.tensor(v, dtype=torch.int32, device=device)
             self._src_cache[key] = t
+        return t
+
+    def qk_skip_vector(self, batch: int, device, total_batch: Optional[int] = None, images: int = 1):
+        from . import ops
+        total = total_batch or batch * images
+        key = (batch, total, images, str(device))
+        t = self._skip_cache.get(key)
+        if t is None:
+            n = batch // 2
+            flags = ([False] * (n + 1) + [True] * (batch - n - 1)) * images + [False] * (total - batch * images)
+            t = self._skip_cache[key] = ops.GroupSkip(flags, device)
         return t
 
     def cross_kind(self, step: Optional[int] = None) -> str:
diff --git a/omg_amd/csrc/gemm.hip b/omg_amd/csrc/gemm.hip
--- a/omg_amd/csrc/gemm.hip
+++ b/omg_amd/csrc/gemm.hip
@@ -157,6 +157,7 @@
   const int m_end = (p.tile_groups > 1) ? m_base + p.rows_per_group : p.M;
   const int m0 = m_base + tm * BM;
   const int n0 = tn * BN;
+  if (tile_skipped(p, m0, m_end, n0, BM, BN)) return;
 
   int adapter = 0;
   if (p.group_adapter != nullptr) adapter = p.group_adapter[grp];
@@ -337,6 +338,7 @@
   const int m_end = (p.tile_groups > 1) ? m_base + p.rows_per_group : p.M;
   const int m0 = m_base + tm * BM_;
   const int n0 = tn * BN_;
+  if (tile_skipped(p, m0, m_end, n0, BM_, BN_)) return;
   int adapter = 0;
   if (p.group_adapter != nullptr) adapter = p.group_adapter[grp];
   if (p.w_adapter_stride != 0 && adapter < 0) return;
@@ -565,6 +567,7 @@
   const int m_end = (p.tile_groups > 1) ? m_base + p.rows_per_group : p.M;
   const int m0 = m_base + tm * BM_;
   const int n0 = tn * BN_;
+  if (tile_skipped(p, m0, m_end, n0, BM_, BN_)) return;
   int adapter = 0;
   if (p.group_adapter != nullptr) adapter = p.group_adapter[grp];
   if (p.w_adapter_stride != 0 && adapter < 0) return;
@@ -928,6 +931,7 @@
   if (a->act == OMG_ACT_GEGLU) OMG_REQUIRE(a->N % 64 == 0 && !a->residual && !a->group_bias, "omg_gemm: GEGLU needs N % 64 == 0, no residual");
   if (a->residual) OMG_REQUIRE(a->ldr % 8 == 0, "omg_gemm: ldr");
   if (a->group_bias) OMG_REQUIRE(a->ldgb % 8 == 0, "omg_gemm: ldgb");
+  if (a->group_skip) OMG_REQUIRE(a->skip_n_end >= 0 && a->act != OMG_ACT_GEGLU, "omg_gemm: group_skip needs skip_n_end >= 0 and no GEGLU epilogue");
   ensure_attrs();
   GemmP p{};
   p.M = a->M; p.N = a->N; p.K = a->K;
@@ -942,6 +946,7 @@
   p.bias = (const char*)a->bias; p.group_bias = (const char*)a->group_bias; p.ldgb = a->ldgb;
   p.residual = (const char*)a->residual; p.ldr = a->ldr;
   p.act = a->act; p.out_scale = a->out_scale; p.C = (char*)a->C; p.ldc = a->ldc;
+  if (a->group_skip != nullptr && a->skip_n_end > 0) { p.group_skip = a->group_skip; p.skip_n_end = a->skip_n_end; }
   const int mrows = per_group ? a->rows_per_group : a->M;
   p.tiles_m = (mrows + BM - 1) / BM;
   p.tiles_n = (a->N + BN - 1) / BN;
diff --git a/omg_amd/csrc/gemm_epilogue.h b/omg_amd/csrc/gemm_epilogue.h
--- a/omg_amd/csrc/gemm_epilogue.h
+++ b/omg_amd/csrc/gemm_epilogue.h
@@ -26,11 +26,23 @@
   int sa_ld, sw_ld;
   long sw_adapter_stride;
   char* QS; int qs_ld;
+  const int* group_skip; int skip_n_end;
 };
 
 typedef __attribute__((address_space(3))) void* lds_ptr_t;
 typedef const __attribute__((address_space(1))) void* gbl_ptr_t;
 OMG_DEV bool fold_group_bias(const GemmP& p) { return p.group_bias != nullptr && p.rows_per_group % 256 == 0; }
+
+OMG_DEV bool tile_skipped(const GemmP& p, int m0, int m_end, int n0, int bm, int bn) {
+  if (p.group_skip == nullptr) return false;
+  const int n1 = n0 + bn < p.N ? n0 + bn : p.N;
+  if (n1 > p.skip_n_end) return false;
+  const int m1 = m0 + bm < m_end ? m0 + bm : m_end;
+  const int g1 = (m1 - 1) / p.rows_per_group;
+  for (int g = m0 / p.rows_per_group; g <= g1; ++g)
+    if (p.group_skip[g] == 0) return false;
+  return true;
+}
 
 template <int N> OMG_DEV void wait_vmcnt() {
   static_assert(N >= 0 && N <= 63, "vmcnt range");
diff --git a/omg_amd/csrc/gemm_v12.h b/omg_amd/csrc/gemm_v12.h
--- a/omg_amd/csrc/gemm_v12.h
+++ b/omg_amd/csrc/gemm_v12.h
@@ -63,18 +63,25 @@
   t.grp = grp;
   return t;
 }
+template <bool SKIP>
 OMG_DEV int next_tile_v12(const GemmP& p, int vb, int step, int ntiles) {
-  if (p.w_adapter_stride == 0 || p.group_adapter == nullptr) return vb;
+  const bool slots = p.w_adapter_stride != 0 && p.group_adapter != nullptr;
+  if (!SKIP && !slots) return vb;
   while (vb < ntiles) {
     const TileV12 t = decode_tile_v12(p, vb, ntiles);
-    if (p.group_adapter[t.grp] >= 0) break;
+    bool dead = slots && p.group_adapter[t.grp] < 0;
+    if constexpr (SKIP) dead = dead || tile_skipped(p, t.m0, t.m_end, t.n0, 256, 256);
+    if (!dead) break;
     vb += step;
   }
   return vb;
 }
 
-template <typename T, bool CONV, int EF>
+template <typename T, bool CONV, int EF_>
 __global__ __launch_bounds__(256, 1) void gemm_kernel_v12(GemmP p) {
+  constexpr bool SKIP = EF_ > 4;
+  constexpr int EF = SKIP ? EF_ - 4 : EF_;
+  static_assert(!SKIP || (!CONV && (EF == 1 || EF == 2)), "table forms: the Linear layers' bias-only and residual epilogues");
   constexpr int MT = 4, NT = 4;
   constexpr bool XE = true;
   constexpr int BM_ = MT * 64, BN_ = NT * 64, BKc = 64;
@@ -113,7 +120,7 @@
   f32x16 acc[MT][NT];
   using V8 = typename Vec<T>::v8;
 
-  int vb = next_tile_v12(p, (int)blockIdx.x, step, ntiles);
+  int vb = next_tile_v12<SKIP>(p, (int)blockIdx.x, step, ntiles);
   if (vb >= ntiles) return;
   int m0, n0, m_end;
 #define OMG_TILE_SCALARS(t_)                                                                               \
@@ -289,7 +296,7 @@
     sa_cur = 0; sw_cur = HALF; sa_nxt = 2 * HALF; sw_nxt = 3 * HALF; s_sp = 4 * HALF;
     { const unsigned tnxt = 1u; (void)tnxt; OMG_KS_PROLOGUE_5(); }
     e_m0 = m0; e_n0 = n0; e_mend = m_end;
-    if constexpr (PERSIST) { vbn = next_tile_v12(p, vb + step, step, ntiles); has_next = vbn < ntiles; }
+    if constexpr (PERSIST) { vbn = next_tile_v12<SKIP>(p, vb + step, step, ntiles); has_next = vbn < ntiles; }
 
     int kt = 0;
 #define OMG_KS_VARS const unsigned tcur = 0u; const unsigned tnxt = 1u; (void)tnxt; (void)tcur
@@ -355,7 +362,7 @@
   const int ntiles = p.tile_groups * p.tiles_m * p.tiles_n;
   if (ntiles <= 0) return OMG_OK;
   int grid = ntiles;
-  if (EF != 2) {
+  if (EF != 2 && EF != 6) {
     int cus = num_cus() & ~7;
     if (g_dbg & 0x10000) cus = 8;
     if (grid > cus && cus > 0) grid = cus;
@@ -367,6 +374,12 @@
 int launch_v12_form(const GemmP& p, hipStream_t s, int mrows) {
   const bool gb_rows = p.group_bias != nullptr && p.rows_per_group % 256 != 0;
   if (p.act == OMG_ACT_GEGLU) return launch_v12<T, CONV, 3>(p, s, mrows);
+  if constexpr (!CONV) {
+    if (p.group_skip != nullptr) {
+      if (gb_rows || p.act == OMG_ACT_SILU) return launch_v7<T, CONV>(p, s, mrows);
+      return p.residual != nullptr ? launch_v12<T, CONV, 6>(p, s, mrows) : launch_v12<T, CONV, 5>(p, s, mrows);
+    }
+  }
   if (gb_rows || p.act == OMG_ACT_SILU) return launch_v12<T, CONV, 4>(p, s, mrows);
   if (p.residual != nullptr) return launch_v12<T, CONV, 2>(p, s, mrows);
   return launch_v12<T, CONV, 1>(p, s, mrows);
diff --git a/omg_amd/csrc/gemm_v13.h b/omg_amd/csrc/gemm_v13.h
--- a/omg_amd/csrc/gemm_v13.h
+++ b/omg_amd/csrc/gemm_v13.h
@@ -185,6 +185,7 @@
   const int m_end = (p.tile_groups > 1) ? m_base + p.rows_per_group : p.M;
   const int m0 = m_base + tm * BM_;
   const int n0 = tn * BN_;
+  if (tile_skipped(p, m0, m_end, n0, BM_, BN_)) return;
   int adapter = 0;
   if (p.group_adapter != nullptr) adapter = p.group_adapter[grp];
   if (p.w_adapter_stride != 0 && adapter < 0) return;
diff --git a/omg_amd/modules.py b/omg_amd/modules.py
--- a/omg_amd/modules.py
+++ b/omg_amd/modules.py
@@ -99,7 +99,8 @@
         return ops.LoraSpec(t, self.lora_up, st.group_adapter)
 
     def forward(self, x: torch.Tensor, scale=None, *, residual: Optional[torch.Tensor] = None, act: int = L.ACT_NONE,
-                group_bias: Optional[torch.Tensor] = None, groups: int = 1) -> torch.Tensor:
+                group_bias: Optional[torch.Tensor] = None, groups: int = 1,
+                group_skip: Optional[ops.GroupSkip] = None, skip_n_end: int = 0) -> torch.Tensor:
         if isinstance(x, ops.Mx8Tensor) or (self.mx8 and group_bias is None and self._mx8_ok()):
             if group_bias is not None or not self._mx8_ok():
                 raise L.OmgHipError("an MX-fp8 activation reached a Linear layer that cannot run in MX-fp8")
@@ -109,14 +110,16 @@
         r2 = residual.reshape(-1, self.out_features) if residual is not None else None
         st = self.lora_state
         if st is not None and st.merged and self.w_slots is not None:
-            y = ops.gemm(x2, self.w_slots, bias=self.bias, residual=r2, act=act, groups=st.groups, w_group_adapter=st.group_adapter)
+            y = ops.gemm(x2, self.w_slots, bias=self.bias, residual=r2, act=act, groups=st.groups, w_group_adapter=st.group_adapter,
+                         group_skip=group_skip, skip_n_end=skip_n_end)
             return y.view(*shp[:-1], y.shape[-1])
         lora = self._lora(x2)
         if lora is not None:
             groups = self.lora_state.groups
             if x2.shape[0] % groups != 0:
                 raise L.OmgHipError("LoRA groups do not divide the row count")
-        y = ops.gemm(x2, self.weight, bias=self.bias, residual=r2, act=act, group_bias=group_bias, groups=groups, lora=lora)
+        y = ops.gemm(x2, self.weight, bias=self.bias, residual=r2, act=act, group_bias=group_bias, groups=groups, lora=lora,
+                     group_skip=group_skip, skip_n_end=skip_n_end)
         return y.view(*shp[:-1], y.shape[-1])
 
 
diff --git a/omg_amd/ops.py b/omg_amd/ops.py
--- a/omg_amd/ops.py
+++ b/omg_amd/ops.py
@@ -84,10 +84,43 @@
         self.a2, self.w2, self.group_adapter, self.a2_col_block = a2, w2, group_adapter, a2_col_block
 
 
+class GroupSkip:
+
+    __slots__ = ("flags", "table")
+
+    def __init__(self, flags: Sequence[bool], device):
+        self.flags = tuple(bool(f) for f in flags)
+        self.table = torch.tensor([int(f) for f in self.flags], dtype=torch.int32, device=device)
+
+
+_TILE_OF_VARIANT = {1: (128, 128), 14: (256, 128), 13: (256, 256), 15: (256, 256), 25: (256, 256), 24: (128, 320), 28: (256, 320)}
+
+
+def executed_fraction(M: int, N: int, K: int, K2: int, groups: int, per_group_tiles: bool, skip: GroupSkip, skip_n_end: int) -> float:
+    rpg = M // groups
+    tg = groups if per_group_tiles and groups > 1 else 1
+    mrows = rpg if tg > 1 else M
+    v = L.lib().omg_debug_choose_variant(mrows, tg, N, 0)
+    if K2 > 0 or K % 64 != 0:
+        v = 1
+    bm, bn = _TILE_OF_VARIANT.get(v, (128, 128))
+    total = dead = 0
+    for g in range(tg):
+        base, end = (g * rpg, (g + 1) * rpg) if tg > 1 else (0, M)
+        for m0 in range(base, end, bm):
+            m1 = min(m0 + bm, end)
+            rows_dead = all(skip.flags[q] for q in range(m0 // rpg, (m1 - 1) // rpg + 1))
+            for n0 in range(0, N, bn):
+                total += 1
+                dead += rows_dead and min(n0 + bn, N) <= skip_n_end
+    return (total - dead) / total
+
+
 def gemm(a: torch.Tensor, w: torch.Tensor, *, bias: Optional[torch.Tensor] = None,
          residual: Optional[torch.Tensor] = None, act: int = L.ACT_NONE, out: Optional[torch.Tensor] = None,
          out_scale: float = 1.0, group_bias: Optional[torch.Tensor] = None, groups: int = 1,
-         lora: Optional[LoraSpec] = None, w_group_adapter: Optional[torch.Tensor] = None) -> torch.Tensor:
+         lora: Optional[LoraSpec] = None, w_group_adapter: Optional[torch.Tensor] = None,
+         group_skip: Optional[GroupSkip] = None, skip_n_end: int = 0) -> torch.Tensor:
     _dev(a)
     M, K = a.shape
     assert a.stride(1) == 1
@@ -109,6 +142,16 @@
     args.M, args.N, args.K = M, N, K
     args.A, args.lda = a.data_ptr(), a.stride(0)
     args.W, args.ldw = w.data_ptr(), ldw
+    if group_skip is not None:
+        if groups == 1:
+            groups = len(group_skip.flags)
+        if groups != len(group_skip.flags) or M % groups != 0:
+            raise L.OmgHipError(f"group_skip has {len(group_skip.flags)} entries for {groups} groups of {M} rows")
+        if act == L.ACT_GEGLU:
+            raise L.OmgHipError("group_skip does not combine with the GEGLU epilogue")
+        if all(group_skip.flags) and skip_n_end >= N:
+            return out
+        args.group_skip, args.skip_n_end = group_skip.table.data_ptr(), min(skip_n_end, N)
     args.groups = groups
     args.rows_per_group = M // groups
     adapter = w_group_adapter
@@ -138,7 +181,8 @@
     if _PROF is not None:
         t0 = _PROF.begin()
         L.check(L.lib().omg_gemm(C.byref(args), _stream()), "omg_gemm")
-        _PROF.end("gemm", 2.0 * M * N * (K + args.K2), t0, ("lin", M, N, K, args.K2, groups if adapter is not None else 1, act))
+        done = 1.0 if group_skip is None else executed_fraction(M, N, K, args.K2, groups, adapter is not None, group_skip, args.skip_n_end)
+        _PROF.end("gemm", 2.0 * M * N * (K + args.K2) * done, t0, ("lin", M, N, K, args.K2, groups if adapter is not None else 1, act))
         return out
     L.check(L.lib().omg_gemm(C.byref(args), _stream()), "omg_gemm")
     return out
@@ -178,7 +222,9 @@
 def gemm_mx8(a: Mx8Tensor, w: Mx8Tensor, *, out_dtype: torch.dtype = torch.float16, bias: Optional[torch.Tensor] = None,
              residual: Optional[torch.Tensor] = None, act: int = L.ACT_NONE, out: Optional[torch.Tensor] = None,
              out_scale: float = 1.0, groups: int = 1, w_group_adapter: Optional[torch.Tensor] = None,
-             n_per_adapter: Optional[int] = None, out_mx8: bool = False):
+             n_per_adapter: Optional[int] = None, out_mx8: bool = False, group_skip=None):
+    if group_skip is not None:
+        raise L.OmgHipError("omg_gemm_mx8 takes no group_skip table (16-bit omg_gemm only)")
     M, K = a.rows, a.K
     assert w.K == K
     N = n_per_adapter if w_group_adapter is not None else w.rows
```

Result: no change. 0.4197, median of 6 (+0.5%).
